# BoMingZhao/GaussianPrediction

Hardware: AMD Instinct MI355X
Metric: rendered views/s (full train step) @1M Gaussians 1352x1014 (higher is better)
Workload: dtype f32; 1 GPU; configs[2]: HyperNeRF-like 1M Gaussians, 1352x1014, stage-3 full train step (deform, raster, L1+SSIM loss, Adam: all HIP kernels); gaussians=1000000, width=1352, height=1014, keypoints=250, nearest_num=6, parallelism=view-parallel x1, ranks_seen_by_rccl=1, self_launched=False

## Files before the change

### gaussianprediction_amd/csrc/deform_kernels.h

```cpp
#pragma once
#include "gp_common.h"

struct MlpDev {
    long rows;
    int in_dim, in_pad, out_dim;
    int feature_dim, xyz_freq, time_freq;
    const float* w[5];
    const float* b[5];
    const float* feature;
    const float* xyz;
    const float* t;
    const float* pk;
};

struct MlpPackLayout {
    int q0;
    int tb0;
    long off_f[4], off_b[4], total;
};
static inline __host__ __device__ MlpPackLayout mlp_pack_layout(int in_dim) {
    MlpPackLayout L;
    L.q0 = (in_dim + 15) / 16;
    L.tb0 = 2 * ((in_dim + 31) / 32);
    long o = 0;
    L.off_f[0] = o; o += 16L * L.q0 * 64;
    for (int l = 1; l < 4; ++l) { L.off_f[l] = o; o += 16L * 16 * 64; }
    L.off_b[0] = o; o += (long)L.tb0 * 16 * 64;
    for (int l = 1; l < 4; ++l) { L.off_b[l] = o; o += 16L * 16 * 64; }
    L.total = o;
    return L;
}

struct MlpWeightJobs {
    const float* dZ[5];
    const float* H[5];
    float* dW[5];
    float* db[5];
    int n_out[5], n_in[5], ldh[5];
};

struct BlendDev {
    long N, K;
    int nn, out_dim, norm_rotation;
    const float* delta;
    const float* raw_w;
    const int64_t* knn;
    const float* xyz;
    const float* rot;
    const uint16_t* knn16;
};

__global__ __launch_bounds__(256) void gp_mlp_pack_kernel(MlpDev p, float4* __restrict__ out);
__global__ __launch_bounds__(512) void gp_mlp_fwd_kernel(MlpDev p, float* __restrict__ out, float* __restrict__ saved_x,
                                                         float* __restrict__ saved_h);
__global__ __launch_bounds__(512) void gp_mlp_bwd_data_kernel(MlpDev p, const float* __restrict__ saved_h,
                                                              const float* __restrict__ dL_dout, float* __restrict__ dz,
                                                              float* __restrict__ dfeature, float* __restrict__ dxyz);
__global__ __launch_bounds__(512) void gp_mlp_bwd_weight_kernel(const float* __restrict__ dZ, int n_out,
                                                                const float* __restrict__ H, int ldh, int n_in, long rows,
                                                                long rows_per_block, float* __restrict__ dW, int lddw,
                                                                float* __restrict__ db);
__global__ __launch_bounds__(256) void gp_blend_fwd_kernel(BlendDev a, float* __restrict__ xyz_t, float* __restrict__ q_t);
__global__ __launch_bounds__(256) void gp_blend_fwd6_kernel(BlendDev a, float* __restrict__ xyz_t, float* __restrict__ q_t);
__global__ __launch_bounds__(256) void gp_blend_fwd8_kernel(BlendDev a, float* __restrict__ xyz_t, float* __restrict__ q_t);
__global__ __launch_bounds__(256) void gp_blend_fwd6_i16_kernel(BlendDev a, float* __restrict__ xyz_t, float* __restrict__ q_t);
__global__ __launch_bounds__(256) void gp_blend_fwd8_i16_kernel(BlendDev a, float* __restrict__ xyz_t, float* __restrict__ q_t);
__global__ __launch_bounds__(256) void gp_blend_bwd_kernel(BlendDev a, const float* __restrict__ g_xyz_t,
                                                           const float* __restrict__ g_q_t, float* __restrict__ g_delta,
                                                           float* __restrict__ g_raw_w, float* __restrict__ g_xyz,
                                                           float* __restrict__ g_rot, float* __restrict__ partial);
__global__ __launch_bounds__(256) void gp_blend_bwd6_kernel(BlendDev a, const float* __restrict__ g_xyz_t,
                                                           const float* __restrict__ g_q_t, float* __restrict__ g_delta,
                                                           float* __restrict__ g_raw_w, float* __restrict__ g_xyz,
                                                           float* __restrict__ g_rot, float* __restrict__ partial);
__global__ __launch_bounds__(256) void gp_blend_bwd8_kernel(BlendDev a, const float* __restrict__ g_xyz_t,
                                                           const float* __restrict__ g_q_t, float* __restrict__ g_delta,
                                                           float* __restrict__ g_raw_w, float* __restrict__ g_xyz,
                                                           float* __restrict__ g_rot, float* __restrict__ partial);
__global__ __launch_bounds__(256) void gp_blend_bwd6_i16_kernel(BlendDev a, const float* __restrict__ g_xyz_t,
                                                           const float* __restrict__ g_q_t, float* __restrict__ g_delta,
                                                           float* __restrict__ g_raw_w, float* __restrict__ g_xyz,
                                                           float* __restrict__ g_rot, float* __restrict__ partial);
__global__ __launch_bounds__(256) void gp_blend_bwd8_i16_kernel(BlendDev a, const float* __restrict__ g_xyz_t,
                                                           const float* __restrict__ g_q_t, float* __restrict__ g_delta,
                                                           float* __restrict__ g_raw_w, float* __restrict__ g_xyz,
                                                           float* __restrict__ g_rot, float* __restrict__ partial);
__global__ __launch_bounds__(1024) void gp_blend_bwd_reduce_kernel(const float* __restrict__ partial, int nblocks, int KA,
                                                                  int od, float* __restrict__ g_delta);
__global__ __launch_bounds__(256) void gp_act_fwd_kernel(long n, const float* __restrict__ scaling_raw,
                                                         const float* __restrict__ opacity_raw,
                                                         const float* __restrict__ delta_o, int stride, float beta,
                                                         float* __restrict__ scale, float* __restrict__ opacity);
__global__ __launch_bounds__(256) void gp_act_bwd_kernel(long n, const float* __restrict__ scaling_raw,
                                                         const float* __restrict__ opacity_raw,
                                                         const float* __restrict__ delta_o, int stride, float beta,
                                                         const float* __restrict__ g_scale,
                                                         const float* __restrict__ g_opacity,
                                                         float* __restrict__ g_scaling_raw, float* __restrict__ g_opacity_raw,
                                                         float* __restrict__ g_delta_o);

__global__ __launch_bounds__(512) void gp_mlp_bwd_weight5_kernel(MlpWeightJobs t, long rows);
__global__ __launch_bounds__(512) void gp_mlp_fwd_small_kernel(MlpDev p, float* __restrict__ out, float* __restrict__ saved_x,
                                                               float* __restrict__ saved_h);
__global__ __launch_bounds__(512) void gp_mlp_bwd_data_small_kernel(MlpDev p, const float* __restrict__ saved_h,
                                                                    const float* __restrict__ dL_dout, float* __restrict__ dz,
                                                                    float* __restrict__ dfeature, float* __restrict__ dxyz);

__global__ __launch_bounds__(256) void gp_mlp_fwd_split_small_kernel(MlpDev p, float* __restrict__ out, float* __restrict__ saved_x, float* hx,
                                                                     uint32_t* flags, uint32_t* err);
__global__ __launch_bounds__(256) void gp_mlp_fwd_split_small_agent_kernel(MlpDev p, float* __restrict__ out, float* __restrict__ saved_x,
                                                                           float* hx, uint32_t* flags, uint32_t* err);
__global__ __launch_bounds__(256) void gp_mlp_bwd_data_split_small_kernel(MlpDev p, const float* __restrict__ saved_h, const float* __restrict__ dL_dout,
                                                                          float* dz, float* __restrict__ dfeature, float* __restrict__ dxyz, float* gx,
                                                                          uint32_t* flags, uint32_t* err, int form);
struct AdamTable;
__global__ __launch_bounds__(512) void gp_mlp_bwd_data_small_adam_kernel(MlpDev p, const float* __restrict__ saved_h,
                                                                         const float* __restrict__ dL_dout, float* __restrict__ dz,
                                                                         float* __restrict__ dfeature, float* __restrict__ dxyz,
                                                                         unsigned n_mlp, AdamTable t, float b1, float b2, float eps,
                                                                         int zero_grad, const uint32_t* __restrict__ skip_flag);

__global__ __launch_bounds__(256) void gp_mlp_bwd_weight64_kernel(const float* __restrict__ dZ, int n_out, const float* __restrict__ H,
                                                                 int ldh, int n_in, long rows, long rows_per_block,
                                                                 unsigned n_row_blocks, float* __restrict__ dW, int lddw,
                                                                 float* __restrict__ db);
__global__ __launch_bounds__(512) void gp_mlp_fwd2_kernel(MlpDev p, float* __restrict__ out, float* __restrict__ saved_x,
                                                          float* __restrict__ saved_h, uint32_t* __restrict__ masks);
__global__ __launch_bounds__(512) void gp_mlp_bwd_data2_kernel(MlpDev p, const uint32_t* __restrict__ masks,
                                                               const float* __restrict__ dL_dout, float* __restrict__ dz,
                                                               float* __restrict__ dfeature, float* __restrict__ dxyz);
```

### gaussianprediction_amd/csrc/deform_kernels.hip

```cpp
#include "gp_common.h"
#include "deform_kernels.h"

typedef float f32x16 __attribute__((ext_vector_type(16)));

#define MLP_ROWS 32
#define MLP_THREADS 512
#define MLP_W 256

__device__ __forceinline__ int act_idx(int f, int j) { return f * MLP_ROWS + (j ^ (f & 31)); }
__device__ __forceinline__ int cd_row(int r, int half) { return (r & 3) + 8 * (r >> 2) + 4 * half; }

__device__ __forceinline__ void build_input(float* buf, const MlpDev& p, long row0, int tid) {
    const int fd = p.feature_dim, xf = p.xyz_freq, tf = p.time_freq;
    for (int e = tid; e < fd * MLP_ROWS; e += MLP_THREADS) {
        const int jj = e / fd, f = e - jj * fd;
        const long row = row0 + jj;
        buf[act_idx(f, jj)] = row < p.rows ? p.feature[row * fd + f] : 0.f;
    }
    for (int e = tid; e < 3 * xf * MLP_ROWS; e += MLP_THREADS) {
        const int jj = e % MLP_ROWS, cf = e / MLP_ROWS;
        const int c = cf / xf, fr = cf - c * xf;
        const long row = row0 + jj;
        float sv = 0.f, cv = 0.f;
        if (row < p.rows) {
// ... 403 lines not shown
                    const long row = trow0 + jj;
                    if (row < p.rows) {
                        const float x = p.xyz[row * 3 + c];
                        float g = 0.f;
                        for (int fr = 0; fr < p.xyz_freq; ++fr) {
                            const float sc = (float)(1u << fr);
                            float sv, cv;
                            sincosf(x * sc, &sv, &cv);
                            const int f = p.feature_dim + 2 * (c * p.xyz_freq + fr);
                            g += sc * (cv * buf[act_idx(f, jj)] - sv * buf[act_idx(f + 1, jj)]);
                        }
                        dxyz[row * 3 + c] = g;
                    }
                }
            }
        }
    }
}

__device__ __forceinline__ void mlp_bwd_weight_body(const float* __restrict__ dZ, int n_out, const float* __restrict__ H, int ldh,
                                                    int n_in, long rows, long rows_per_block, float* __restrict__ dW, int lddw,
                                                    float* __restrict__ db, int row_block, int n_row_blocks, int bz, int by) {
    __shared__ float s_red[8][16][64];
    __shared__ float s_b[8][32];
    const int tid = threadIdx.x, lane = tid & 63, wave = tid >> 6, half = lane >> 5, j = lane & 31;
    const int o = 32 * bz + j;
    const int i = 32 * by + j;
    const long b_begin = (long)row_block * rows_per_block;
    long b_end = b_begin + rows_per_block;
    if (b_end > rows) b_end = rows;
    long per_wave = ((b_end - b_begin + 7) / 8 + 1) & ~1L;
    const long r_begin = b_begin + wave * per_wave;
    long r_end = r_begin + per_wave;
    if (r_end > b_end) r_end = b_end;
    f32x16 acc;
#pragma unroll
    for (int r = 0; r < 16; ++r) acc[r] = 0.f;
    float bsum = 0.f;
    const bool o_ok = o < n_out, i_ok = i < n_in;
    for (long rb = r_begin; rb < r_end; rb += 8) {
        float a[4], b[4];
#pragma unroll
        for (int u = 0; u < 4; ++u) {
            const long r = rb + 2 * u + half;
            a[u] = (r < r_end && o_ok) ? dZ[r * n_out + o] : 0.f;
            b[u] = (r < r_end && i_ok) ? H[r * (long)ldh + i] : 0.f;
            bsum += a[u];
        }
#pragma unroll
        for (int u = 0; u < 4; ++u) acc = __builtin_amdgcn_mfma_f32_32x32x2f32(a[u], b[u], acc, 0, 0, 0);
    }
#pragma unroll
    for (int r = 0; r < 16; ++r) s_red[wave][r][lane] = acc[r];
    bsum += __shfl_xor(bsum, 32);
    if (half == 0) s_b[wave][j] = bsum;
    __syncthreads();
    const bool single = n_row_blocks == 1;
    for (int e = tid; e < 16 * 64; e += MLP_THREADS) {
        const int r = e >> 6, l = e & 63;
        float v = 0.f;
#pragma unroll
        for (int w = 0; w < 8; ++w) v += s_red[w][r][l];
        const int oo = 32 * bz + cd_row(r, l >> 5), ii = 32 * by + (l & 31);
        if (oo < n_out && ii < n_in) {
            float* dst = &dW[(size_t)oo * lddw + ii];
            if (single) *dst += v; else atomicAdd(dst, v);
        }
    }
    if (db && by == 0 && tid < 32) {
        float v = 0.f;
#pragma unroll
        for (int w = 0; w < 8; ++w) v += s_b[w][tid];
        const int oo = 32 * bz + tid;
        if (oo < n_out) { if (single) db[oo] += v; else atomicAdd(&db[oo], v); }
    }
}

__global__ __launch_bounds__(MLP_THREADS) void gp_mlp_bwd_weight_kernel(const float* __restrict__ dZ, int n_out,
                                                                        const float* __restrict__ H, int ldh, int n_in,
                                                                        long rows, long rows_per_block,
                                                                        float* __restrict__ dW, int lddw,
                                                                        float* __restrict__ db) {
    mlp_bwd_weight_body(dZ, n_out, H, ldh, n_in, rows, rows_per_block, dW, lddw, db, blockIdx.x, gridDim.x, blockIdx.z, blockIdx.y);
}
__global__ __launch_bounds__(MLP_THREADS) void gp_mlp_bwd_weight5_kernel(MlpWeightJobs t, long rows) {
    const int l = blockIdx.x;
    if ((int)blockIdx.y * 32 >= t.n_in[l] || (int)blockIdx.z * 32 >= t.n_out[l]) return;
    mlp_bwd_weight_body(t.dZ[l], t.n_out[l], t.H[l], t.ldh[l], t.n_in[l], rows, rows, t.dW[l], t.n_in[l], t.db[l], 0, 1, blockIdx.z,
                        blockIdx.y);
}

__global__ __launch_bounds__(256) void gp_mlp_bwd_weight64_kernel(const float* __restrict__ dZ, int n_out, const float* __restrict__ H,
                                                                 int ldh, int n_in, long rows, long rows_per_block,
                                                                 unsigned n_row_blocks, float* __restrict__ dW, int lddw,
                                                                 float* __restrict__ db) {
    __shared__ float s_red[4][4][16][64];
    const int tid = threadIdx.x, lane = tid & 63, wave = tid >> 6, half = lane >> 5, j = lane & 31;
    const int n_ib = (n_in + 63) / 64;
    const int ntp = n_ib * ((n_out + 63) / 64);
    const unsigned flat = blockIdx.x, xcd = flat & 7u, seq = flat >> 3;
    const unsigned slab = (seq / ntp) * 8u + xcd, tp = seq % ntp;
    if (slab >= n_row_blocks) return;
    const int o0 = 64 * (tp / n_ib), i0 = 64 * (tp % n_ib);
    const long b_begin = (long)slab * rows_per_block;
    long b_end = b_begin + rows_per_block;
    if (b_end > rows) b_end = rows;
    const long per_wave = ((b_end - b_begin + 3) / 4 + 7) & ~7L;
    const long r_begin = b_begin + wave * per_wave;
    long r_end = r_begin + per_wave;
    if (r_end > b_end) r_end = b_end;
    f32x16 acc[2][2];
#pragma unroll
    for (int a = 0; a < 2; ++a)
#pragma unroll
        for (int b = 0; b < 2; ++b)
#pragma unroll
            for (int r = 0; r < 16; ++r) acc[a][b][r] = 0.f;
    float bsum[2] = {0.f, 0.f};
    const int oa = o0 + j, ob = o0 + 32 + j, ia = i0 + j, ib = i0 + 32 + j;
    const bool oka = oa < n_out, okb = ob < n_out, ika = ia < n_in, ikb = ib < n_in;
    for (long rb = r_begin; rb < r_end; rb += 8) {
        float a0[4], a1[4], b0[4], b1[4];
#pragma unroll
        for (int u = 0; u < 4; ++u) {
            const long r = rb + 2 * u + half;
            const bool rk = r < r_end;
            a0[u] = (rk && oka) ? dZ[r * n_out + oa] : 0.f;
            a1[u] = (rk && okb) ? dZ[r * n_out + ob] : 0.f;
            b0[u] = (rk && ika) ? H[r * (long)ldh + ia] : 0.f;
            b1[u] = (rk && ikb) ? H[r * (long)ldh + ib] : 0.f;
            bsum[0] += a0[u]; bsum[1] += a1[u];
        }
#pragma unroll
        for (int u = 0; u < 4; ++u) {
            acc[0][0] = __builtin_amdgcn_mfma_f32_32x32x2f32(a0[u], b0[u], acc[0][0], 0, 0, 0);
            acc[0][1] = __builtin_amdgcn_mfma_f32_32x32x2f32(a0[u], b1[u], acc[0][1], 0, 0, 0);
            acc[1][0] = __builtin_amdgcn_mfma_f32_32x32x2f32(a1[u], b0[u], acc[1][0], 0, 0, 0);
            acc[1][1] = __builtin_amdgcn_mfma_f32_32x32x2f32(a1[u], b1[u], acc[1][1], 0, 0, 0);
        }
    }
#pragma unroll
    for (int a = 0; a < 2; ++a)
#pragma unroll
        for (int b = 0; b < 2; ++b)
#pragma unroll
            for (int r = 0; r < 16; ++r) s_red[wave][2 * a + b][r][lane] = acc[a][b][r];
    __syncthreads();
    const bool single = n_row_blocks == 1;
    for (int e = tid; e < 4 * 16 * 64; e += 256) {
        const int tl = e >> 10, r = (e >> 6) & 15, l = e & 63;
        const float v = (s_red[0][tl][r][l] + s_red[1][tl][r][l]) + (s_red[2][tl][r][l] + s_red[3][tl][r][l]);
        const int oo = o0 + 32 * (tl >> 1) + cd_row(r, l >> 5), ii = i0 + 32 * (tl & 1) + (l & 31);
        if (oo < n_out && ii < n_in) {
            float* dst = &dW[(size_t)oo * lddw + ii];
            if (single) *dst += v; else atomicAdd(dst, v);
        }
    }
    if (db && i0 == 0) {
        __syncthreads();
        float* sb = &s_red[0][0][0][0];
#pragma unroll
        for (int u = 0; u < 2; ++u) {
            const float v = bsum[u] + __shfl_xor(bsum[u], 32);
            if (half == 0) sb[(wave * 2 + u) * 32 + j] = v;
        }
        __syncthreads();
        if (tid < 64) {
            const int u = tid >> 5, jj = tid & 31;
            const float v = (sb[(0 * 2 + u) * 32 + jj] + sb[(1 * 2 + u) * 32 + jj]) + (sb[(2 * 2 + u) * 32 + jj] + sb[(3 * 2 + u) * 32 + jj]);
            const int oo = o0 + 32 * u + jj;
            if (oo < n_out) { if (single) db[oo] += v; else atomicAdd(&db[oo], v); }
        }
    }
}

#define GP_MAX_NN 16

__device__ __forceinline__ void quat_mul(const float* q, const float* r, float* p) {
    p[0] = r[0] * q[0] - r[1] * q[1] - r[2] * q[2] - r[3] * q[3];
    p[1] = r[1] * q[0] + r[0] * q[1] + r[3] * q[2] - r[2] * q[3];
    p[2] = r[2] * q[0] - r[3] * q[1] + r[0] * q[2] + r[1] * q[3];
    p[3] = r[3] * q[0] + r[2] * q[1] - r[1] * q[2] + r[0] * q[3];
}
__device__ __forceinline__ float norm4(const float* v) {
    return fmaxf(sqrtf(v[0] * v[0] + v[1] * v[1] + v[2] * v[2] + v[3] * v[3]), 1e-12f);
}
__device__ __forceinline__ void softmax_n(const float* __restrict__ raw, int n, float* w) {
    float m = raw[0];
#pragma unroll
    for (int k = 1; k < n; ++k) m = fmaxf(m, raw[k]);
    float s = 0.f;
#pragma unroll
    for (int k = 0; k < n; ++k) { w[k] = expf(raw[k] - m); s += w[k]; }
    const float inv = 1.f / s;
#pragma unroll
    for (int k = 0; k < n; ++k) w[k] *= inv;
}

template <int NN, bool I16>
__device__ __forceinline__ void load_row_nn(const BlendDev& a, long i, float (&raw)[2 * NN], int (&kps)[NN]) {
    const float4* r4 = (const float4*)(a.raw_w + i * 2 * NN);
#pragma unroll
    for (int u = 0; u < 2 * NN / 4; ++u) { const float4 t = r4[u]; raw[4 * u] = t.x; raw[4 * u + 1] = t.y; raw[4 * u + 2] = t.z; raw[4 * u + 3] = t.w; }
    if (I16) {
        const uint32_t* k1 = (const uint32_t*)(a.knn16 + i * NN);
#pragma unroll
        for (int u = 0; u < NN / 2; ++u) { const uint32_t t = k1[u]; kps[2 * u] = (int)(t & 0xFFFFu); kps[2 * u + 1] = (int)(t >> 16); }
    } else {
        typedef long long ll2 __attribute__((ext_vector_type(2)));
        const ll2* k2 = (const ll2*)(a.knn + i * NN);
#pragma unroll
        for (int u = 0; u < NN / 2; ++u) { const ll2 t = k2[u]; kps[2 * u] = (int)t.x; kps[2 * u + 1] = (int)t.y; }
    }
}

template <int NN, bool I16 = false>
__device__ __forceinline__ void blend_fwd_body(BlendDev a, float* __restrict__ xyz_t, float* __restrict__ q_t) {
    const long i = (long)blockIdx.x * 256 + threadIdx.x;
    if (i >= a.N) return;
    float dxyz[3] = {0.f, 0.f, 0.f}, dq[4] = {0.f, 0.f, 0.f, 0.f};
    const int od = a.out_dim;
    const int nn = NN > 0 ? NN : a.nn;
    const float x0[3] = {a.xyz[3 * i], a.xyz[3 * i + 1], a.xyz[3 * i + 2]};
    const float r[4] = {a.rot[4 * i], a.rot[4 * i + 1], a.rot[4 * i + 2], a.rot[4 * i + 3]};
    if (nn > 0) {
        float wx[NN > 0 ? NN : GP_MAX_NN], wr[NN > 0 ? NN : GP_MAX_NN];
        int kpv[NN > 0 ? NN : 1];
        if constexpr (NN > 0) {
            float raw[2 * (NN > 0 ? NN : 1)];
            load_row_nn<NN, I16>(a, i, raw, kpv);
            softmax_n(raw, NN, wx);
            softmax_n(raw + NN, NN, wr);
        } else {
            softmax_n(a.raw_w + i * 2 * nn, nn, wx);
            softmax_n(a.raw_w + i * 2 * nn + nn, nn, wr);
        }
        if constexpr (NN > 0) {
            float dlr[NN > 0 ? NN : 1][7];
#pragma unroll
            for (int k = 0; k < NN; ++k) {
                const float* dl = a.delta + (long)kpv[k] * od;
#pragma unroll
                for (int c = 0; c < 7; ++c) dlr[k][c] = dl[c];
            }
#pragma unroll
            for (int k = 0; k < NN; ++k) {
                dxyz[0] = fmaf(wx[k], dlr[k][0], dxyz[0]);
                dxyz[1] = fmaf(wx[k], dlr[k][1], dxyz[1]);
                dxyz[2] = fmaf(wx[k], dlr[k][2], dxyz[2]);
                float v[4] = {dlr[k][3], dlr[k][4], dlr[k][5], dlr[k][6]};
                if (a.norm_rotation) { const float inv = 1.f / norm4(v); v[0] *= inv; v[1] *= inv; v[2] *= inv; v[3] *= inv; }
                dq[0] = fmaf(wr[k], v[0], dq[0]); dq[1] = fmaf(wr[k], v[1], dq[1]);
                dq[2] = fmaf(wr[k], v[2], dq[2]); dq[3] = fmaf(wr[k], v[3], dq[3]);
            }
        } else {
            for (int k = 0; k < nn; ++k) {
                const long kp = a.knn16 ? (long)a.knn16[i * nn + k] : a.knn[i * nn + k];
                const float* dl = a.delta + kp * od;
                dxyz[0] = fmaf(wx[k], dl[0], dxyz[0]);
                dxyz[1] = fmaf(wx[k], dl[1], dxyz[1]);
                dxyz[2] = fmaf(wx[k], dl[2], dxyz[2]);
                float v[4] = {dl[3], dl[4], dl[5], dl[6]};
                if (a.norm_rotation) { const float inv = 1.f / norm4(v); v[0] *= inv; v[1] *= inv; v[2] *= inv; v[3] *= inv; }
                dq[0] = fmaf(wr[k], v[0], dq[0]); dq[1] = fmaf(wr[k], v[1], dq[1]);
                dq[2] = fmaf(wr[k], v[2], dq[2]); dq[3] = fmaf(wr[k], v[3], dq[3]);
            }
        }
    } else {
        const float* dl = a.delta + i * od;
        dxyz[0] = dl[0]; dxyz[1] = dl[1]; dxyz[2] = dl[2];
        dq[0] = dl[3]; dq[1] = dl[4]; dq[2] = dl[5]; dq[3] = dl[6];
        if (a.norm_rotation) { const float inv = 1.f / norm4(dq); dq[0] *= inv; dq[1] *= inv; dq[2] *= inv; dq[3] *= inv; }
    }
    xyz_t[3 * i] = x0[0] + dxyz[0];
    xyz_t[3 * i + 1] = x0[1] + dxyz[1];
    xyz_t[3 * i + 2] = x0[2] + dxyz[2];
    const float invq = 1.f / norm4(dq);
    const float q[4] = {dq[0] * invq, dq[1] * invq, dq[2] * invq, dq[3] * invq};
    float pq[4];
    quat_mul(q, r, pq);
    const float invp = 1.f / norm4(pq);
    q_t[4 * i] = pq[0] * invp; q_t[4 * i + 1] = pq[1] * invp; q_t[4 * i + 2] = pq[2] * invp; q_t[4 * i + 3] = pq[3] * invp;
}
__global__ __launch_bounds__(256) void gp_blend_fwd_kernel(BlendDev a, float* __restrict__ xyz_t, float* __restrict__ q_t) { blend_fwd_body<0>(a, xyz_t, q_t); }
__global__ __launch_bounds__(256) void gp_blend_fwd6_kernel(BlendDev a, float* __restrict__ xyz_t, float* __restrict__ q_t) { blend_fwd_body<6>(a, xyz_t, q_t); }
__global__ __launch_bounds__(256) void gp_blend_fwd8_kernel(BlendDev a, float* __restrict__ xyz_t, float* __restrict__ q_t) { blend_fwd_body<8>(a, xyz_t, q_t); }
__global__ __launch_bounds__(256) void gp_blend_fwd6_i16_kernel(BlendDev a, float* __restrict__ xyz_t, float* __restrict__ q_t) { blend_fwd_body<6, true>(a, xyz_t, q_t); }
__global__ __launch_bounds__(256) void gp_blend_fwd8_i16_kernel(BlendDev a, float* __restrict__ xyz_t, float* __restrict__ q_t) { blend_fwd_body<8, true>(a, xyz_t, q_t); }

__device__ __forceinline__ void normalize_bwd(const float* v, const float* g, float* dv) {
    const float n = norm4(v), inv = 1.f / n;
    const float y[4] = {v[0] * inv, v[1] * inv, v[2] * inv, v[3] * inv};
    const float dot = y[0] * g[0] + y[1] * g[1] + y[2] * g[2] + y[3] * g[3];
#pragma unroll
    for (int k = 0; k < 4; ++k) dv[k] = (g[k] - y[k] * dot) * inv;
}

#define BB_LONG 20
#define BB_LONG_CAP 320
template <int NN, bool I16 = false>
__device__ __forceinline__ void blend_bwd_body(BlendDev a, const float* __restrict__ g_xyz_t,
                                               const float* __restrict__ g_q_t, float* __restrict__ g_delta,
                                               float* __restrict__ g_raw_w, float* __restrict__ g_xyz,
                                               float* __restrict__ g_rot, float* __restrict__ partial) {
    extern __shared__ float s_dyn[];
    const int od = a.out_dim;
    const int nn = NN > 0 ? NN : a.nn;
    const int K = (int)a.K;
    const int tid = threadIdx.x;
    float* s_acc = s_dyn;
    float* s_delta = s_acc + (nn > 0 ? K * 7 : 0);
    int* s_cnt = (int*)(s_delta + (nn > 0 ? K * od : 0));
    int* s_base = s_cnt + (nn > 0 ? K : 0);
    float* s_g = (float*)(s_base + (nn > 0 ? K + 1 : 0));
    float* s_inv = s_g + 256 * 7;
    float* s_w = s_inv + (nn > 0 ? K : 0);
    unsigned short* s_sorted = (unsigned short*)(s_w + 256 * 2 * nn);
    __shared__ int s_wsum[4];
    __shared__ int s_nlong, s_long[BB_LONG_CAP];
    if (nn > 0) {
        for (int e = tid; e < K * 7; e += 256) s_acc[e] = 0.f;
        for (int e = tid; e < K * od; e += 256) s_delta[e] = a.delta[e];
        if (a.norm_rotation) {
            __syncthreads();
            for (int kp = tid; kp < K; kp += 256) {
                float* dl = s_delta + kp * od;
                const float v[4] = {dl[3], dl[4], dl[5], dl[6]};
                const float inv = 1.f / norm4(v);
                s_inv[kp] = inv;
                dl[3] = v[0] * inv; dl[4] = v[1] * inv; dl[5] = v[2] * inv; dl[6] = v[3] * inv;
            }
        }
    }
    const long chunks = (a.N + 255) / 256;
    for (long c = blockIdx.x; c < chunks; c += gridDim.x) {
        const long i = c * 256 + tid;
        const bool live = i < a.N;
        if (nn > 0) {
            for (int e = tid; e < K; e += 256) s_cnt[e] = 0;
            if (tid == 0) s_nlong = 0;
            __syncthreads();
        }
        int kps[NN > 0 ? NN : GP_MAX_NN], rk[NN > 0 ? NN : GP_MAX_NN];
        if (live) {
            const float gx[3] = {g_xyz_t[3 * i], g_xyz_t[3 * i + 1], g_xyz_t[3 * i + 2]};
            const float gq[4] = {g_q_t[4 * i], g_q_t[4 * i + 1], g_q_t[4 * i + 2], g_q_t[4 * i + 3]};
            const float r[4] = {a.rot[4 * i], a.rot[4 * i + 1], a.rot[4 * i + 2], a.rot[4 * i + 3]};
            float wx[NN > 0 ? NN : GP_MAX_NN], wr[NN > 0 ? NN : GP_MAX_NN];
            float dq[4] = {0.f, 0.f, 0.f, 0.f};
            if (nn > 0) {
                if constexpr (NN > 0) {
                    float raw[2 * (NN > 0 ? NN : 1)];
                    load_row_nn<NN, I16>(a, i, raw, kps);
                    softmax_n(raw, NN, wx);
                    softmax_n(raw + NN, NN, wr);
                } else {
                    softmax_n(a.raw_w + i * 2 * nn, nn, wx);
                    softmax_n(a.raw_w + i * 2 * nn + nn, nn, wr);
                }
#pragma unroll
                for (int k = 0; k < nn; ++k) {
                    if (NN == 0) kps[k] = a.knn16 ? (int)a.knn16[i * nn + k] : (int)a.knn[i * nn + k];
                    const float* dl = s_delta + kps[k] * od;
                    const float v[4] = {dl[3], dl[4], dl[5], dl[6]};
                    dq[0] = fmaf(wr[k], v[0], dq[0]); dq[1] = fmaf(wr[k], v[1], dq[1]);
                    dq[2] = fmaf(wr[k], v[2], dq[2]); dq[3] = fmaf(wr[k], v[3], dq[3]);
                }
            } else {
                const float* dl = a.delta + i * od;
                dq[0] = dl[3]; dq[1] = dl[4]; dq[2] = dl[5]; dq[3] = dl[6];
                if (a.norm_rotation) { const float inv = 1.f / norm4(dq); dq[0] *= inv; dq[1] *= inv; dq[2] *= inv; dq[3] *= inv; }
            }
            const float invq = 1.f / norm4(dq);
            const float q[4] = {dq[0] * invq, dq[1] * invq, dq[2] * invq, dq[3] * invq};
            g_xyz[3 * i] = gx[0]; g_xyz[3 * i + 1] = gx[1]; g_xyz[3 * i + 2] = gx[2];
            float pq[4];
            quat_mul(q, r, pq);
            float gp[4];
            normalize_bwd(pq, gq, gp);
            const float gqn[4] = {gp[0] * r[0] + gp[1] * r[1] + gp[2] * r[2] + gp[3] * r[3],
                                  -gp[0] * r[1] + gp[1] * r[0] - gp[2] * r[3] + gp[3] * r[2],
                                  -gp[0] * r[2] + gp[1] * r[3] + gp[2] * r[0] - gp[3] * r[1],
                                  -gp[0] * r[3] - gp[1] * r[2] + gp[2] * r[1] + gp[3] * r[0]};
            g_rot[4 * i + 0] = gp[0] * q[0] + gp[1] * q[1] + gp[2] * q[2] + gp[3] * q[3];
            g_rot[4 * i + 1] = -gp[0] * q[1] + gp[1] * q[0] + gp[2] * q[3] - gp[3] * q[2];
            g_rot[4 * i + 2] = -gp[0] * q[2] - gp[1] * q[3] + gp[2] * q[0] + gp[3] * q[1];
            g_rot[4 * i + 3] = -gp[0] * q[3] + gp[1] * q[2] - gp[2] * q[1] + gp[3] * q[0];
            float gdq[4];
            normalize_bwd(dq, gqn, gdq);
            if (nn > 0) {
                float gwx[NN > 0 ? NN : GP_MAX_NN], gwr[NN > 0 ? NN : GP_MAX_NN];
                float sx = 0.f, sr = 0.f;
#pragma unroll
                for (int k = 0; k < nn; ++k) {
                    const float* dl = s_delta + kps[k] * od;
                    gwx[k] = dl[0] * gx[0] + dl[1] * gx[1] + dl[2] * gx[2];
                    const float vn[4] = {dl[3], dl[4], dl[5], dl[6]};
                    gwr[k] = vn[0] * gdq[0] + vn[1] * gdq[1] + vn[2] * gdq[2] + vn[3] * gdq[3];
                    sx += wx[k] * gwx[k];
                    sr += wr[k] * gwr[k];
                    s_w[k * 256 + tid] = wx[k];
                    s_w[(nn + k) * 256 + tid] = wr[k];
                    rk[k] = atomicAdd(&s_cnt[kps[k]], 1);
                }
                if (g_raw_w) {
                    if constexpr (NN > 0) {
                        float go[2 * (NN > 0 ? NN : 1)];
#pragma unroll
                        for (int k = 0; k < NN; ++k) { go[k] = wx[k] * (gwx[k] - sx); go[NN + k] = wr[k] * (gwr[k] - sr); }
                        float4* o4 = (float4*)(g_raw_w + i * 2 * NN);
#pragma unroll
                        for (int u = 0; u < 2 * NN / 4; ++u) o4[u] = make_float4(go[4 * u], go[4 * u + 1], go[4 * u + 2], go[4 * u + 3]);
                    } else {
                        for (int k = 0; k < nn; ++k) {
                            g_raw_w[i * 2 * nn + k] = wx[k] * (gwx[k] - sx);
                            g_raw_w[i * 2 * nn + nn + k] = wr[k] * (gwr[k] - sr);
                        }
                    }
                }
                s_g[0 * 256 + tid] = gx[0]; s_g[1 * 256 + tid] = gx[1]; s_g[2 * 256 + tid] = gx[2];
                s_g[3 * 256 + tid] = gdq[0]; s_g[4 * 256 + tid] = gdq[1]; s_g[5 * 256 + tid] = gdq[2]; s_g[6 * 256 + tid] = gdq[3];
            } else {
                const float* dl = a.delta + i * od;
                float gv[4] = {gdq[0], gdq[1], gdq[2], gdq[3]};
                if (a.norm_rotation) { const float v[4] = {dl[3], dl[4], dl[5], dl[6]}; normalize_bwd(v, gdq, gv); }
                float* gd = g_delta + i * od;
                gd[0] = gx[0]; gd[1] = gx[1]; gd[2] = gx[2];
                gd[3] = gv[0]; gd[4] = gv[1]; gd[5] = gv[2]; gd[6] = gv[3];
                for (int k = 7; k < od; ++k) gd[k] = 0.f;
            }
        }
        if (nn > 0) {
            __syncthreads();
            {
                const int per = (K + 255) / 256;
                const int b0 = tid * per;
                int loc = 0;
                for (int e = 0; e < per; ++e) if (b0 + e < K) loc += s_cnt[b0 + e];
                int inc = loc;
                inc = gp_wave_scan_add(inc);
                if ((tid & 63) == 63) s_wsum[tid >> 6] = inc;
                __syncthreads();
                int woff = 0;
                for (int w = 0; w < (tid >> 6); ++w) woff += s_wsum[w];
                int run = woff + inc - loc;
                for (int e = 0; e < per; ++e) if (b0 + e < K) { s_base[b0 + e] = run; run += s_cnt[b0 + e]; }
                if (tid == 255) s_base[K] = run;
            }
            __syncthreads();
            if (live) {
#pragma unroll
                for (int k = 0; k < nn; ++k) s_sorted[s_base[kps[k]] + rk[k]] = (unsigned short)((k << 8) | tid);
            }
            __syncthreads();
            for (int kp = tid; kp < K; kp += 256) {
                float sacc[7] = {0.f, 0.f, 0.f, 0.f, 0.f, 0.f, 0.f};
                const int pe = s_base[kp + 1];
                if (pe - s_base[kp] > BB_LONG) { s_long[atomicAdd(&s_nlong, 1)] = kp; continue; }
                for (int pp = s_base[kp]; pp < pe; pp += 2) {
                    const int e0 = s_sorted[pp], e1 = pp + 1 < pe ? s_sorted[pp + 1] : -1;
                    const int t0 = e0 & 255, k0 = e0 >> 8, t1 = e1 & 255, k1 = (e1 >> 8) & 15;
                    const float wx0 = s_w[k0 * 256 + t0], wr0 = s_w[(nn + k0) * 256 + t0];
                    const float wx1 = e1 >= 0 ? s_w[k1 * 256 + t1] : 0.f, wr1 = e1 >= 0 ? s_w[(nn + k1) * 256 + t1] : 0.f;
                    float g0[7], g1[7];
#pragma unroll
                    for (int cc = 0; cc < 7; ++cc) { g0[cc] = s_g[cc * 256 + t0]; g1[cc] = s_g[cc * 256 + t1]; }
                    sacc[0] = fmaf(wx0, g0[0], sacc[0]); sacc[1] = fmaf(wx0, g0[1], sacc[1]); sacc[2] = fmaf(wx0, g0[2], sacc[2]);
                    sacc[3] = fmaf(wr0, g0[3], sacc[3]); sacc[4] = fmaf(wr0, g0[4], sacc[4]);
                    sacc[5] = fmaf(wr0, g0[5], sacc[5]); sacc[6] = fmaf(wr0, g0[6], sacc[6]);
                    if (e1 >= 0) {
                        sacc[0] = fmaf(wx1, g1[0], sacc[0]); sacc[1] = fmaf(wx1, g1[1], sacc[1]); sacc[2] = fmaf(wx1, g1[2], sacc[2]);
                        sacc[3] = fmaf(wr1, g1[3], sacc[3]); sacc[4] = fmaf(wr1, g1[4], sacc[4]);
                        sacc[5] = fmaf(wr1, g1[5], sacc[5]); sacc[6] = fmaf(wr1, g1[6], sacc[6]);
                    }
                }
                float* acc = s_acc + kp * 7;
#pragma unroll
                for (int cc = 0; cc < 7; ++cc) acc[cc] += sacc[cc];
            }
            __syncthreads();
            const int nlong = s_nlong;
            for (int q = tid >> 6; q < nlong; q += 4) {
                const int kp = s_long[q], pe = s_base[kp + 1];
                float sacc[7] = {0.f, 0.f, 0.f, 0.f, 0.f, 0.f, 0.f};
                for (int pp = s_base[kp] + (tid & 63); pp < pe; pp += 64) {
                    const int e = s_sorted[pp], t = e & 255, k = e >> 8;
                    const float wxk = s_w[k * 256 + t], wrk = s_w[(nn + k) * 256 + t];
                    sacc[0] = fmaf(wxk, s_g[0 * 256 + t], sacc[0]); sacc[1] = fmaf(wxk, s_g[1 * 256 + t], sacc[1]);
                    sacc[2] = fmaf(wxk, s_g[2 * 256 + t], sacc[2]); sacc[3] = fmaf(wrk, s_g[3 * 256 + t], sacc[3]);
                    sacc[4] = fmaf(wrk, s_g[4 * 256 + t], sacc[4]); sacc[5] = fmaf(wrk, s_g[5 * 256 + t], sacc[5]);
                    sacc[6] = fmaf(wrk, s_g[6 * 256 + t], sacc[6]);
                }
#pragma unroll
                for (int off = 32; off > 0; off >>= 1)
#pragma unroll
                    for (int cc = 0; cc < 7; ++cc) sacc[cc] += __shfl_xor(sacc[cc], off);
                if ((tid & 63) == 0) {
                    float* acc = s_acc + kp * 7;
#pragma unroll
                    for (int cc = 0; cc < 7; ++cc) acc[cc] += sacc[cc];
                }
            }
            if (nlong > 0) __syncthreads();
        }
    }
    if (nn > 0) {
        const int KA = K * 7;
        for (int kp = tid; kp < K; kp += 256) {
            float* acc = s_acc + kp * 7;
            if (a.norm_rotation) {
                const float* y = s_delta + kp * od + 3;
                const float inv = s_inv[kp];
                const float cq[4] = {acc[3], acc[4], acc[5], acc[6]};
                const float dot = y[0] * cq[0] + y[1] * cq[1] + y[2] * cq[2] + y[3] * cq[3];
#pragma unroll
                for (int k = 0; k < 4; ++k) acc[3 + k] = (cq[k] - y[k] * dot) * inv;
            }
        }
        __syncthreads();
        for (int e = tid; e < KA; e += 256) partial[(size_t)blockIdx.x * KA + e] = s_acc[e];
    }
}

#define BB_ARGS BlendDev a, const float* __restrict__ g_xyz_t, const float* __restrict__ g_q_t, float* __restrict__ g_delta, \
    float* __restrict__ g_raw_w, float* __restrict__ g_xyz, float* __restrict__ g_rot, float* __restrict__ partial
__global__ __launch_bounds__(256) void gp_blend_bwd_kernel(BB_ARGS) { blend_bwd_body<0>(a, g_xyz_t, g_q_t, g_delta, g_raw_w, g_xyz, g_rot, partial); }
__global__ __launch_bounds__(256) void gp_blend_bwd6_kernel(BB_ARGS) { blend_bwd_body<6>(a, g_xyz_t, g_q_t, g_delta, g_raw_w, g_xyz, g_rot, partial); }
__global__ __launch_bounds__(256) void gp_blend_bwd8_kernel(BB_ARGS) { blend_bwd_body<8>(a, g_xyz_t, g_q_t, g_delta, g_raw_w, g_xyz, g_rot, partial); }
__global__ __launch_bounds__(256) void gp_blend_bwd6_i16_kernel(BB_ARGS) { blend_bwd_body<6, true>(a, g_xyz_t, g_q_t, g_delta, g_raw_w, g_xyz, g_rot, partial); }
__global__ __launch_bounds__(256) void gp_blend_bwd8_i16_kernel(BB_ARGS) { blend_bwd_body<8, true>(a, g_xyz_t, g_q_t, g_delta, g_raw_w, g_xyz, g_rot, partial); }

__global__ __launch_bounds__(1024) void gp_blend_bwd_reduce_kernel(const float* __restrict__ partial, int nblocks, int KA,
                                                                  int od, float* __restrict__ g_delta) {
    __shared__ float s_r[16][64];
    const int lane = threadIdx.x & 63, wave = threadIdx.x >> 6;
    const int e = blockIdx.x * 64 + lane;
    float v0 = 0.f, v1 = 0.f, v2 = 0.f, v3 = 0.f;
    if (e < KA) {
        int b = wave;
        for (; b + 240 < nblocks; b += 256) {
            float t[16];
#pragma unroll
            for (int u = 0; u < 16; ++u) t[u] = partial[(size_t)(b + 16 * u) * KA + e];
#pragma unroll
            for (int u = 0; u < 16; u += 4) { v0 += t[u]; v1 += t[u + 1]; v2 += t[u + 2]; v3 += t[u + 3]; }
        }
        for (; b + 48 < nblocks; b += 64) {
            v0 += partial[(size_t)b * KA + e]; v1 += partial[(size_t)(b + 16) * KA + e];
            v2 += partial[(size_t)(b + 32) * KA + e]; v3 += partial[(size_t)(b + 48) * KA + e];
        }
        for (; b < nblocks; b += 16) v0 += partial[(size_t)b * KA + e];
    }
    s_r[wave][lane] = (v0 + v1) + (v2 + v3);
    __syncthreads();
    if (wave == 0 && e < KA) {
        float t = 0.f;
#pragma unroll
        for (int w = 0; w < 16; ++w) t += s_r[w][lane];
        g_delta[(size_t)(e / 7) * od + (e % 7)] = t;
        if (e % 7 == 6) for (int c = 7; c < od; ++c) g_delta[(size_t)(e / 7) * od + c] = 0.f;
    }
}

__device__ __forceinline__ float sigmoidf(float x) { return 1.f / (1.f + expf(-x)); }

__global__ __launch_bounds__(256) void gp_act_fwd_kernel(long n, const float* __restrict__ scaling_raw,
                                                        const float* __restrict__ opacity_raw,
                                                        const float* __restrict__ delta_o, int stride, float beta,
                                                        float* __restrict__ scale, float* __restrict__ opacity) {
    const long i = (long)blockIdx.x * 256 + threadIdx.x;
    if (i >= n) return;
    const float s0 = scaling_raw[3 * i], s1 = scaling_raw[3 * i + 1], s2 = scaling_raw[3 * i + 2];
    const float op_raw = opacity_raw[i];
    const float dlt = delta_o ? delta_o[i * stride] : 0.f;
    scale[3 * i] = expf(s0);
    scale[3 * i + 1] = expf(s1);
    scale[3 * i + 2] = expf(s2);
    float o = sigmoidf(op_raw);
    if (delta_o) o *= 1.f / (1.f + expf(-dlt / beta));
    opacity[i] = o;
}
__global__ __launch_bounds__(256) void gp_act_bwd_kernel(long n, const float* __restrict__ scaling_raw,
                                                        const float* __restrict__ opacity_raw,
                                                        const float* __restrict__ delta_o, int stride, float beta,
                                                        const float* __restrict__ g_scale, const float* __restrict__ g_opacity,
                                                        float* __restrict__ g_scaling_raw, float* __restrict__ g_opacity_raw,
                                                        float* __restrict__ g_delta_o) {
    const long i = (long)blockIdx.x * 256 + threadIdx.x;
    if (i >= n) return;
    float gs[3] = {0.f, 0.f, 0.f}, sr[3] = {0.f, 0.f, 0.f};
    if (g_scaling_raw && g_scale) {
#pragma unroll
        for (int k = 0; k < 3; ++k) { gs[k] = g_scale[3 * i + k]; sr[k] = scaling_raw[3 * i + k]; }
    }
    const float op_raw = opacity_raw[i];
    const float go = g_opacity ? g_opacity[i] : 0.f;
    const float dlt = delta_o ? delta_o[i * stride] : 0.f;
    if (g_scaling_raw) {
#pragma unroll
        for (int k = 0; k < 3; ++k) g_scaling_raw[3 * i + k] = g_scale ? gs[k] * expf(sr[k]) : 0.f;
    }
    const float so = sigmoidf(op_raw);
    float life = 1.f;
    if (delta_o) life = 1.f / (1.f + expf(-dlt / beta));
    if (g_opacity_raw) g_opacity_raw[i] = go * life * so * (1.f - so);
    if (delta_o && g_delta_o) g_delta_o[i * stride] = go * so * life * (1.f - life) / beta;
}
```

### gaussianprediction_amd/csrc/gp_capi_deform.hip

```cpp
#include "gp_common.h"
#include "deform_kernels.h"
#include "loss_adam_kernels.h"
#include <stdlib.h>

static int make_mlp(const gp_mlp_params* p, const gp_mlp_input* x, MlpDev& m) {
    if (!p || !x) GP_FAIL("null mlp params/input");
    if (p->width != 256 || p->depth != 4) GP_FAIL("Deformable_Field: only d=4, w=256 is implemented (got d=%d w=%d)", p->depth, p->width);
    if (p->out_dim < 7 || p->out_dim > 8) GP_FAIL("out_dim must be 7 or 8 (got %d)", p->out_dim);
    if (x->feature_dim <= 0 || x->feature_dim % 4 || x->xyz_freq < 0 || x->xyz_freq > 16 || x->time_freq < 0 || x->time_freq > 16)
        GP_FAIL("bad input encoding dims");
    const int in_dim = x->feature_dim + 6 * x->xyz_freq + 2 * x->time_freq;
    if (in_dim != p->in_dim) GP_FAIL("in_dim %d != feature_dim + 6*xyz_freq + 2*time_freq = %d", p->in_dim, in_dim);
    if (in_dim % 4 || in_dim > 256) GP_FAIL("in_dim %d must be a multiple of 4 and <= 256", in_dim);
    if (x->rows < 0) GP_FAIL("negative rows");
    for (int l = 0; l < 5; ++l)
        if (!p->w[l] || !p->b[l]) GP_FAIL("null weight pointer (layer %d)", l);
    if (x->rows > 0 && (!x->feature || (x->xyz_freq > 0 && !x->xyz) || (x->time_freq > 0 && !x->t))) GP_FAIL("null input pointer");
    m.rows = x->rows; m.in_dim = in_dim; m.in_pad = (in_dim + 7) / 8 * 8; m.out_dim = p->out_dim;
    m.feature_dim = x->feature_dim; m.xyz_freq = x->xyz_freq; m.time_freq = x->time_freq;
    for (int l = 0; l < 5; ++l) { m.w[l] = p->w[l]; m.b[l] = p->b[l]; }
    m.feature = x->feature; m.xyz = x->xyz; m.t = x->t;
    m.pk = p->packed;
    if (m.pk && ((uintptr_t)m.pk & 15) != 0) GP_FAIL("gp_mlp_params.packed must be 16-byte aligned");
    if (p->scratch && ((uintptr_t)p->scratch & 15) != 0) GP_FAIL("gp_mlp_params.scratch must be 16-byte aligned");
    return 0;
}

extern "C" int64_t gp_mlp_packed_floats(int32_t in_dim) {
    if (in_dim <= 0 || in_dim > 256) return -1;
    return 4 * (int64_t)mlp_pack_layout(in_dim).total;
}

extern "C" int gp_mlp_pack(const gp_mlp_params* p, float* packed, gp_stream_t stream_) {
    if (!p || !packed) GP_FAIL("null argument");
    if (p->width != 256 || p->depth != 4) GP_FAIL("Deformable_Field: only d=4, w=256 is implemented");
    if (p->in_dim <= 0 || p->in_dim % 4 || p->in_dim > 256) GP_FAIL("in_dim %d must be a multiple of 4 and <= 256", p->in_dim);
    if (((uintptr_t)packed & 15) != 0) GP_FAIL("packed must be 16-byte aligned");
    MlpDev m;
    memset(&m, 0, sizeof(m));
    m.in_dim = p->in_dim;
    for (int l = 0; l < 4; ++l) { if (!p->w[l]) GP_FAIL("null weight pointer (layer %d)", l); m.w[l] = p->w[l]; }
    const long total = mlp_pack_layout(p->in_dim).total;
    GpProfScope _p("mlp_pack", (hipStream_t)stream_);
    hipLaunchKernelGGL(gp_mlp_pack_kernel, dim3(gp_blocks((size_t)total, 256)), dim3(256), 0, (hipStream_t)stream_, m, (float4*)packed);
    GP_LAUNCH_CHECK();
    return 0;
}

static inline size_t acts_x_floats(const MlpDev& m) { return (size_t)m.rows * m.in_pad; }

#define GP_MLP_SMALL_ROWS 2048
#define GP_MLP_LARGE_ROWS 32768
#define GP_MLP_SPLIT_ROWS 512
#define GP_MLP_SCRATCH_FLAG_BYTES 8192
#define GP_MLP_SCRATCH_ERR_WORD 1024

extern "C" int64_t gp_mlp_scratch_bytes(int64_t rows) {
    if (rows <= 0 || rows > GP_MLP_SPLIT_ROWS) return 0;
    return GP_MLP_SCRATCH_FLAG_BYTES + (int64_t)4 * rows * 256 * (int64_t)sizeof(float);
}

static unsigned mlp_split_grid(const MlpDev& m, const void* scratch, int& mode, int*& state_out) {
    mode = 0; state_out = nullptr;
    if (!scratch || m.rows > GP_MLP_SPLIT_ROWS || gp_debug_get(13) == 1) return 0;
    const unsigned rt = (unsigned)((m.rows + 15) / 16), grid = 8u * 16u * ((rt + 7u) / 8u);
    static int resident[32] = {0}, state[32] = {0};
    int dev = 0;
    if (hipGetDevice(&dev) != hipSuccess || dev < 0 || dev >= 32) return 0;
    if (__atomic_load_n(&resident[dev], __ATOMIC_RELAXED) == 0) {
        int per_cu = 0, r = -1;
        hipDeviceProp_t prop;
        if (hipOccupancyMaxActiveBlocksPerMultiprocessor(&per_cu, gp_mlp_fwd_split_small_kernel, 256, 0) == hipSuccess &&
            hipGetDeviceProperties(&prop, dev) == hipSuccess && per_cu * prop.multiProcessorCount > 0)
            r = per_cu * prop.multiProcessorCount;
        else (void)hipGetLastError();
        __atomic_store_n(&resident[dev], r, __ATOMIC_RELAXED);
    }
    if (__atomic_load_n(&resident[dev], __ATOMIC_RELAXED) < (int)grid) return 0;
    if (gp_debug_get(13) == 2) { mode = 3; return grid; }
    const int st = __atomic_load_n(&state[dev], __ATOMIC_ACQUIRE);
    if (st < 0) return 0;
    mode = st > 0 ? 1 : 2;
    state_out = &state[dev];
    return grid;
}

extern "C" int gp_mlp_forward(const gp_mlp_params* p, const gp_mlp_input* x, float* out, float* acts, gp_stream_t stream_) {
    MlpDev m;
    if (make_mlp(p, x, m)) return 1;
    if (m.rows == 0) return 0;
    if (!out) GP_FAIL("null output");
    float* sx = acts;
    float* sh = acts ? acts + gp_align_up(acts_x_floats(m), 64) : nullptr;
    { GpProfScope _p("mlp_fwd", (hipStream_t)stream_);
        int mode = 0;
        int* state = nullptr;
        const unsigned split = mlp_split_grid(m, p->scratch, mode, state);
        if (split) {
            float* hx = sh ? sh : (float*)((char*)p->scratch + GP_MLP_SCRATCH_FLAG_BYTES);
            uint32_t* flags = (uint32_t*)p->scratch;
            hipLaunchKernelGGL(mode == 3 ? gp_mlp_fwd_split_small_agent_kernel : gp_mlp_fwd_split_small_kernel, dim3(split), dim3(256), 0,
                               (hipStream_t)stream_, m, out, sx, hx, flags, flags + GP_MLP_SCRATCH_ERR_WORD);
            if (mode == 2) {
                uint32_t e = 1;
                if (hipGetLastError() != hipSuccess || hipStreamSynchronize((hipStream_t)stream_) != hipSuccess ||
                    hipMemcpy(&e, flags + GP_MLP_SCRATCH_ERR_WORD, sizeof(e), hipMemcpyDeviceToHost) != hipSuccess) e = 1;
                if (e != 0) {
                    (void)hipGetLastError();
                    __atomic_store_n(state, -1, __ATOMIC_RELEASE);
                    GP_HIP_CHECK(hipMemsetAsync(flags, 0, GP_MLP_SCRATCH_FLAG_BYTES, (hipStream_t)stream_));
                    hipLaunchKernelGGL(gp_mlp_fwd_small_kernel, dim3(gp_blocks((size_t)m.rows, 16)), dim3(512), 0, (hipStream_t)stream_, m, out, sx, sh);
                } else __atomic_store_n(state, 1, __ATOMIC_RELEASE);
            }
        }
        else if (m.rows <= GP_MLP_SMALL_ROWS)
            hipLaunchKernelGGL(gp_mlp_fwd_small_kernel, dim3(gp_blocks((size_t)m.rows, 16)), dim3(512), 0, (hipStream_t)stream_, m, out, sx, sh);
        else if (m.rows >= GP_MLP_LARGE_ROWS)
            hipLaunchKernelGGL(gp_mlp_fwd2_kernel, dim3(gp_blocks((size_t)m.rows, 64)), dim3(512), 0, (hipStream_t)stream_, m, out, sx, sh,
                               acts ? (uint32_t*)(sh + (size_t)4 * m.rows * 256) : (uint32_t*)nullptr);
        else
            hipLaunchKernelGGL(gp_mlp_fwd_kernel, dim3(gp_blocks((size_t)m.rows, 32)), dim3(512), 0, (hipStream_t)stream_, m, out, sx, sh);
    GP_LAUNCH_CHECK(); }
    return 0;
}

static thread_local int g_dfeature_accumulate = 0;
bool gp_mlp_backward_splits(const gp_mlp_params* p, int64_t rows) {
    if (!p) return false;
    MlpDev m;
    memset(&m, 0, sizeof(m));
    m.rows = rows;
    int mode = 0;
    int* st = nullptr;
    return mlp_split_grid(m, p->scratch, mode, st) != 0 && (mode == 1 || mode == 3);
}
void gp_mlp_backward_accumulate_dfeature_once() { g_dfeature_accumulate = 1; }

extern "C" int gp_mlp_backward(const gp_mlp_params* p, const gp_mlp_input* x, const float* acts, const float* dL_dout,
                               gp_mlp_grads* g, float* dL_dfeature, float* dL_dxyz, gp_alloc_fn alloc, void* alloc_ctx,
                               gp_stream_t stream_) {
    hipStream_t s = (hipStream_t)stream_;
    struct ClearAcc { ~ClearAcc() { g_dfeature_accumulate = 0; } } clear_acc;
    MlpDev m;
    if (make_mlp(p, x, m)) return 1;
    if (m.rows == 0) return 0;
    if (!acts || !dL_dout || !g || !alloc) GP_FAIL("null argument");
    for (int l = 0; l < 5; ++l)
        if (!g->dw[l] || !g->db[l]) GP_FAIL("null weight-grad pointer (layer %d)", l);
    const float* sx = acts;
    const float* sh = acts + gp_align_up(acts_x_floats(m), 64);
    const size_t dz_bytes = gp_align_up((size_t)4 * m.rows * 256 * sizeof(float), 256);
    float* dz = (float*)alloc(alloc_ctx, GP_BUF_TEMP, dz_bytes);
    if (!dz) GP_FAIL("allocator returned NULL for TEMP (%zu B)", dz_bytes);
    GpAdamRider* rider = gp_adam_rider_slot();
    int split_mode = 0;
    int* split_state = nullptr;
    const unsigned split = mlp_split_grid(m, p->scratch, split_mode, split_state);
    if (split && (split_mode == 1 || split_mode == 3)) {
        float* gx = (float*)((char*)p->scratch + GP_MLP_SCRATCH_FLAG_BYTES);
        uint32_t* flags = (uint32_t*)p->scratch;
        GpProfScope _p("mlp_bwd_data", s);
        const int acc = g_dfeature_accumulate;
        g_dfeature_accumulate = 0;
        hipLaunchKernelGGL(gp_mlp_bwd_data_split_small_kernel, dim3(split), dim3(256), 0, s, m, sh, dL_dout, dz, dL_dfeature, dL_dxyz, gx, flags,
                           flags + GP_MLP_SCRATCH_ERR_WORD, (split_mode == 3 ? 1 : 0) | (acc ? 2 : 0));
        GP_LAUNCH_CHECK();
    } else if (m.rows <= GP_MLP_SMALL_ROWS && rider->armed) {
        rider->armed = false;
        const unsigned n_mlp = gp_blocks((size_t)m.rows, 16);
        GpProfScope _p("adam", s);
        hipLaunchKernelGGL(gp_mlp_bwd_data_small_adam_kernel, dim3(n_mlp + rider->chunks), dim3(512), 0, s, m, sh, dL_dout, dz, dL_dfeature,
                           dL_dxyz, n_mlp, rider->t, rider->b1, rider->b2, rider->eps, rider->zero_grad, rider->skip_flag);
        GP_LAUNCH_CHECK();
    } else { GpProfScope _p("mlp_bwd_data", s);
        if (m.rows <= GP_MLP_SMALL_ROWS)
            hipLaunchKernelGGL(gp_mlp_bwd_data_small_kernel, dim3(gp_blocks((size_t)m.rows, 16)), dim3(512), 0, s, m, sh, dL_dout, dz,
                               dL_dfeature, dL_dxyz);
        else if (m.rows >= GP_MLP_LARGE_ROWS)
            hipLaunchKernelGGL(gp_mlp_bwd_data2_kernel, dim3(gp_blocks((size_t)m.rows, 64)), dim3(512), 0, s, m,
                               (const uint32_t*)(sh + (size_t)4 * m.rows * 256), dL_dout, dz,
                               dL_dfeature, dL_dxyz);
        else
            hipLaunchKernelGGL(gp_mlp_bwd_data_kernel, dim3(gp_blocks((size_t)m.rows, 32)), dim3(512), 0, s, m, sh, dL_dout, dz,
                       dL_dfeature, dL_dxyz);
    GP_LAUNCH_CHECK(); }
    long nrb_l = (m.rows + 4095) / 4096;
    if (nrb_l > 16) nrb_l = 16;
    if (nrb_l < 1) nrb_l = 1;
    long rpb = ((m.rows + nrb_l - 1) / nrb_l + 15) & ~15L;
    const unsigned nrb = (unsigned)((m.rows + rpb - 1) / rpb);
    GpProfScope _pw("mlp_bwd_weight", s);
    if (nrb == 1) {
        MlpWeightJobs jobs;
        for (int l = 0; l < 5; ++l) {
            jobs.dZ[l] = l < 4 ? dz + (size_t)l * m.rows * 256 : dL_dout;
            jobs.n_out[l] = l < 4 ? 256 : m.out_dim;
            jobs.H[l] = l == 0 ? sx : sh + (size_t)(l - 1) * m.rows * 256;
            jobs.ldh[l] = l == 0 ? m.in_pad : 256;
            jobs.n_in[l] = l == 0 ? m.in_dim : 256;
            jobs.dW[l] = g->dw[l]; jobs.db[l] = g->db[l];
        }
        hipLaunchKernelGGL(gp_mlp_bwd_weight5_kernel, dim3(5, 8, 8), dim3(512), 0, s, jobs, m.rows);
        GP_LAUNCH_CHECK();
        return 0;
    }
    if (m.rows >= 16384) {
        long nb = (m.rows + 4095) / 4096;
        if (nb < 64) nb = 64;
        const long brpb = ((m.rows + nb - 1) / nb + 7) & ~7L;
        const unsigned bnrb = (unsigned)((m.rows + brpb - 1) / brpb);
        for (int l = 0; l < 5; ++l) {
            const float* dZl = l < 4 ? dz + (size_t)l * m.rows * 256 : dL_dout;
            const int n_out = l < 4 ? 256 : m.out_dim;
            const float* H = l == 0 ? sx : sh + (size_t)(l - 1) * m.rows * 256;
            const int ldh = l == 0 ? m.in_pad : 256;
            const int n_in = l == 0 ? m.in_dim : 256;
            const unsigned ntp = (unsigned)((n_in + 63) / 64) * (unsigned)((n_out + 63) / 64);
            hipLaunchKernelGGL(gp_mlp_bwd_weight64_kernel, dim3(ntp * ((bnrb + 7u) & ~7u)), dim3(256), 0, s, dZl, n_out, H, ldh, n_in,
                               m.rows, brpb, bnrb, g->dw[l], n_in, g->db[l]);
            GP_LAUNCH_CHECK();
        }
        return 0;
    }
    for (int l = 0; l < 5; ++l) {
        const float* dZl = l < 4 ? dz + (size_t)l * m.rows * 256 : dL_dout;
        const int n_out = l < 4 ? 256 : m.out_dim;
        const float* H = l == 0 ? sx : sh + (size_t)(l - 1) * m.rows * 256;
        const int ldh = l == 0 ? m.in_pad : 256;
        const int n_in = l == 0 ? m.in_dim : 256;
        {
        hipLaunchKernelGGL(gp_mlp_bwd_weight_kernel, dim3(nrb, (unsigned)((n_in + 31) / 32), (unsigned)((n_out + 31) / 32)),
                           dim3(512), 0, s, dZl, n_out, H, ldh, n_in, m.rows, rpb, g->dw[l], n_in, g->db[l]);
        GP_LAUNCH_CHECK(); }
    }
    return 0;
}

static int make_blend(const gp_blend_args* a, BlendDev& b) {
    if (!a) GP_FAIL("null blend args");
    if (a->num_gaussians < 0) GP_FAIL("negative num_gaussians");
    if (a->out_dim < 7 || a->out_dim > 8) GP_FAIL("out_dim must be 7 or 8");
    if (a->nearest_num < 0 || a->nearest_num > 16) GP_FAIL("nearest_num %d unsupported (0..16)", a->nearest_num);
    if (a->nearest_num > 0 && (a->num_keypoints <= 0 || !a->raw_w || !a->knn_idx)) GP_FAIL("stage-2 blend needs keypoints, raw_w and knn_idx");
    if (a->nearest_num > 0 && a->num_keypoints * 7 * sizeof(float) > 60000) GP_FAIL("too many keypoints (%ld) for the LDS accumulator", (long)a->num_keypoints);
    if (a->num_gaussians > 0 && (!a->delta || !a->xyz || !a->rot)) GP_FAIL("null blend input");
    if (a->knn_idx16 && (a->num_keypoints > 65535 || ((uintptr_t)a->knn_idx16 & 3) != 0)) GP_FAIL("knn_idx16 needs K < 65536 and 4-byte alignment");
    b.N = a->num_gaussians; b.K = a->num_keypoints; b.nn = a->nearest_num; b.out_dim = a->out_dim;
    b.norm_rotation = a->norm_rotation; b.delta = a->delta; b.raw_w = a->raw_w; b.knn = a->knn_idx; b.xyz = a->xyz; b.rot = a->rot; b.knn16 = a->knn_idx16;
    return 0;
}

extern "C" int gp_blend_forward(const gp_blend_args* a, float* xyz_t, float* q_t, gp_stream_t stream_) {
    BlendDev b;
    if (make_blend(a, b)) return 1;
    if (b.N == 0) return 0;
    if (!xyz_t || !q_t) GP_FAIL("null output");
    { GpProfScope _p("blend_fwd", (hipStream_t)stream_);
        const bool al = (((uintptr_t)b.raw_w | (uintptr_t)b.knn) & 15) == 0;
        const bool i16 = b.knn16 != nullptr;
        hipLaunchKernelGGL(b.nn == 6 && al ? (i16 ? gp_blend_fwd6_i16_kernel : gp_blend_fwd6_kernel)
                           : b.nn == 8 && al ? (i16 ? gp_blend_fwd8_i16_kernel : gp_blend_fwd8_kernel) : gp_blend_fwd_kernel,
                       dim3(gp_blocks((size_t)b.N, 256)), dim3(256), 0, (hipStream_t)stream_, b, xyz_t, q_t);
    GP_LAUNCH_CHECK(); }
    return 0;
}

extern "C" int gp_blend_backward(const gp_blend_args* a, const float* dL_dxyz_t, const float* dL_dq_t, float* dL_ddelta,
                                 float* dL_draw_w, float* dL_dxyz, float* dL_drot, gp_alloc_fn alloc, void* alloc_ctx,
                                 gp_stream_t stream_) {
    BlendDev b;
    if (make_blend(a, b)) return 1;
    if (b.N == 0) return 0;
    if (!dL_dxyz_t || !dL_dq_t || !dL_ddelta || !dL_dxyz || !dL_drot) GP_FAIL("null argument");
    unsigned blocks = gp_blocks((size_t)b.N, 256);
    if (b.nn > 0 && blocks > 1024) blocks = 1024;
    const size_t lds = b.nn > 0 ? ((size_t)b.K * (7 + b.out_dim + 3) + 1 + 256 * 7 + 256 * 2 * (size_t)b.nn) * 4 + 256 * (size_t)b.nn * 2 + 16 : 256 * 8 * 4;
    if (lds > 64 * 1024) GP_FAIL("keypoint blend backward: K = %ld, nn = %d needs %zu B of LDS (> 64 KiB)", (long)b.K, b.nn, lds);
    float* partial = nullptr;
    const int KA = (int)b.K * 7;
    if (b.nn > 0) {
        if (!alloc) GP_FAIL("null allocator");
        partial = (float*)alloc(alloc_ctx, GP_BUF_TEMP, gp_align_up((size_t)blocks * KA * sizeof(float), 256));
        if (!partial) GP_FAIL("allocator returned NULL for TEMP");
    }
    { GpProfScope _p("blend_bwd", (hipStream_t)stream_);
    const bool al = (((uintptr_t)b.raw_w | (uintptr_t)b.knn | (uintptr_t)dL_draw_w) & 15) == 0;
    const bool i16 = b.knn16 != nullptr;
    hipLaunchKernelGGL(b.nn == 6 && al ? (i16 ? gp_blend_bwd6_i16_kernel : gp_blend_bwd6_kernel)
                       : b.nn == 8 && al ? (i16 ? gp_blend_bwd8_i16_kernel : gp_blend_bwd8_kernel) : gp_blend_bwd_kernel,
                       dim3(blocks), dim3(256), lds, (hipStream_t)stream_, b, dL_dxyz_t, dL_dq_t, dL_ddelta,
                       dL_draw_w, dL_dxyz, dL_drot, partial);
    GP_LAUNCH_CHECK();
    if (b.nn > 0) {
        hipLaunchKernelGGL(gp_blend_bwd_reduce_kernel, dim3(gp_blocks((size_t)KA, 64)), dim3(1024), 0, (hipStream_t)stream_, partial,
                           (int)blocks, KA, b.out_dim, dL_ddelta);
        GP_LAUNCH_CHECK();
    } }
    return 0;
}

extern "C" int gp_activations_forward(int64_t n, const float* scaling_raw, const float* opacity_raw, const float* delta_o,
                                      int32_t stride, float beta, float* scale, float* opacity, gp_stream_t stream_) {
    if (n < 0) GP_FAIL("negative n");
    if (n == 0) return 0;
    if (!scaling_raw || !opacity_raw || !scale || !opacity) GP_FAIL("null argument");
    if (delta_o && (stride <= 0 || !(beta > 0.f))) GP_FAIL("bad delta_o stride/beta");
    hipLaunchKernelGGL(gp_act_fwd_kernel, dim3(gp_blocks((size_t)n, 256)), dim3(256), 0, (hipStream_t)stream_, (long)n, scaling_raw,
                       opacity_raw, delta_o, stride, beta, scale, opacity);
    GP_LAUNCH_CHECK();
    return 0;
}

extern "C" int gp_activations_backward(int64_t n, const float* scaling_raw, const float* opacity_raw, const float* delta_o,
                                       int32_t stride, float beta, const float* dL_dscale, const float* dL_dopacity,
                                       float* dL_dscaling_raw, float* dL_dopacity_raw, float* dL_ddelta_o, gp_stream_t stream_) {
    if (n < 0) GP_FAIL("negative n");
    if (n == 0) return 0;
    if (!scaling_raw || !opacity_raw) GP_FAIL("null argument");
    hipLaunchKernelGGL(gp_act_bwd_kernel, dim3(gp_blocks((size_t)n, 256)), dim3(256), 0, (hipStream_t)stream_, (long)n, scaling_raw,
                       opacity_raw, delta_o, stride, beta, dL_dscale, dL_dopacity, dL_dscaling_raw, dL_dopacity_raw, dL_ddelta_o);
    GP_LAUNCH_CHECK();
    return 0;
}
```

### gaussianprediction_amd/csrc/gp_capi_raster.hip

```cpp
#include "gp_common.h"
#include "raster_kernels.h"
#include <stdlib.h>
#include <atomic>

thread_local char gp_err_buf[512] = "";
static std::atomic<uint32_t> g_key_tag{0};

extern "C" const char* gp_last_error(void) { return gp_err_buf; }
extern "C" const char* gp_version(void) { return "gaussianprediction_amd 0.4 (gfx950)"; }
extern "C" int gp_abi_version(void) { return GP_ABI_VERSION; }

static int tile_bits_for(int T) {
    int b = 1;
    while ((1 << b) < T) ++b;
    return b;
}

static int make_dims(const gp_raster_settings* st, const gp_raster_inputs* in, RasterDims& d) {
    if (!st || !in) GP_FAIL("null settings/inputs");
    if (st->image_width <= 0 || st->image_height <= 0) GP_FAIL("bad image size %dx%d", st->image_width, st->image_height);
    if (in->num_gaussians < 0 || in->num_gaussians > 0x7FFFFFF0LL) GP_FAIL("num_gaussians out of range");
    if (st->sh_degree < 0 || st->sh_degree > 3) GP_FAIL("sh_degree %d unsupported (0..3)", st->sh_degree);
    const bool has_sr = in->scales != nullptr || in->rotations != nullptr;
    if (in->num_gaussians > 0) {
        if ((in->shs == nullptr) == (in->colors_precomp == nullptr)) GP_FAIL("Please provide exactly one of either SHs or precomputed colors!");
        if (has_sr == (in->cov3D_precomp != nullptr) || (has_sr && (!in->scales || !in->rotations)))
            GP_FAIL("Please provide exactly one of either scale/rotation pair or precomputed 3D covariance!");
    }
    if (in->shs && st->sh_coeffs < (st->sh_degree + 1) * (st->sh_degree + 1)) GP_FAIL("shs has %d coeffs, degree %d needs more", st->sh_coeffs, st->sh_degree);
    if (in->shs && st->sh_coeffs > 16) GP_FAIL("sh_coeffs %d > 16 unsupported", st->sh_coeffs);
    if (in->shs_rest && (!in->shs || st->sh_coeffs != 16)) GP_FAIL("shs_rest needs shs (= features_dc) and sh_coeffs == 16");
    if (!st->bg || !st->viewmatrix || !st->projmatrix || !st->campos) GP_FAIL("null camera pointers");
    if (in->num_gaussians > 0 && (!in->means3D || !in->opacities)) GP_FAIL("null means3D/opacities");
    d.N = (int)in->num_gaussians;
    d.M = in->shs ? st->sh_coeffs : 0;
    d.D = st->sh_degree;
    d.W = st->image_width;
    d.H = st->image_height;
    d.gx = (d.W + GP_TILE - 1) / GP_TILE;
    d.gy = (d.H + GP_TILE - 1) / GP_TILE;
    d.tanfovx = st->tanfovx;
    d.tanfovy = st->tanfovy;
    d.fx = (float)d.W / (2.f * st->tanfovx);
    d.fy = (float)d.H / (2.f * st->tanfovy);
    d.scale_mod = st->scale_modifier;
    d.late_color = (st->sh_ready_event && in->shs) ? 1 : 0;
    d.visible = nullptr; d.zero_words = nullptr; d.n_zero = 0;
    d.key_hi = 0u; d.key_base = 0u; d.key_culled = 0xFFFFFFFFu; d.key_flag = nullptr; d.key_tag = 0u;
    d.sb_side = nullptr;
    d.raw_opacity = nullptr;
    if (st->raw_activations) {
        if (in->cov3D_precomp || !in->scales) GP_FAIL("raw_activations needs scales + rotations (not cov3D_precomp)");
        d.raw_opacity = in->opacities;
    }
    if (st->depth_key_bits != 0 && st->depth_key_bits != 32) {
        if (st->depth_key_bits < 8 || st->depth_key_bits > 31) GP_FAIL("depth_key_bits must be 0, 32 or 8 .. 31 (got %d)", st->depth_key_bits);
        if (!st->binning_status) GP_FAIL("depth_key_bits needs binning_status (the word a broken promise raises)");
        const uint32_t low = (1u << st->depth_key_bits) - 1u;
        d.key_hi = ~low;
        d.key_base = st->depth_key_base;
        d.key_culled = low;
        d.key_flag = st->binning_status + 2;
        do { d.key_tag = ++g_key_tag; } while (d.key_tag == 0u);
    }
    return 0;
}

struct GeomLayout {
    float4* rec;
    uint8_t* clamped;
    float2* sb_side;
    size_t bytes;
    GeomLayout(void* base, size_t N) {
        GpCarver c(base);
        rec = c.take<float4>(3 * N + 1);
        clamped = c.take<uint8_t>(N + 1);
        sb_side = c.take<float2>(GP_SB_HOIST == 1 ? N + 1 : 0);
        bytes = c.bytes();
    }
};
struct ImageLayout {
    int2* ranges;
    float* final_T;
    int32_t* n_contrib;
    int32_t* tile_work;
    uint32_t* order;
    size_t bytes;
    uint32_t* total;
    ImageLayout(void* base, size_t T, size_t P) {
        GpCarver c(base);
        ranges = c.take<int2>(T + GP_TOTAL_SLOTS / 2);
        total = (uint32_t*)(ranges + T);
        final_T = c.take<float>(P);
        n_contrib = c.take<int32_t>(P);
        tile_work = c.take<int32_t>(T);
        order = c.take<uint32_t>(T);
        bytes = c.bytes();
    }
};

extern "C" int gp_raster_forward(const gp_raster_settings* st, const gp_raster_inputs* in, gp_raster_outputs* out,
                                 gp_raster_saved* saved, gp_alloc_fn alloc, void* alloc_ctx, gp_stream_t stream_) {
    hipStream_t s = (hipStream_t)stream_;
    RasterDims d;
    if (make_dims(st, in, d)) return 1;
    if (!out || !out->color || !out->depth || !out->tidx || (d.N > 0 && !out->radii)) GP_FAIL("null output pointers");
    if (!saved || !alloc) GP_FAIL("null saved/alloc");
    const size_t N = (size_t)d.N, T = (size_t)d.gx * d.gy, P = (size_t)d.W * d.H;

    ImageLayout il0(nullptr, T, P);
    void* img = alloc(alloc_ctx, GP_BUF_IMAGE, il0.bytes);
    if (!img) GP_FAIL("allocator returned NULL for IMAGE (%zu B)", il0.bytes);
    ImageLayout il(img, T, P);
    GeomLayout gl0(nullptr, N);
    void* geom = alloc(alloc_ctx, GP_BUF_GEOM, gl0.bytes);
    if (!geom) GP_FAIL("allocator returned NULL for GEOM (%zu B)", gl0.bytes);
    GeomLayout gl(geom, N);
    d.sb_side = gl.sb_side;
    saved->geom = geom; saved->geom_bytes = gl.bytes;
    saved->image = img; saved->image_bytes = il.bytes;
    saved->binning = nullptr; saved->binning_bytes = 0; saved->num_rendered = 0;

    {
        const size_t words = (T + GP_TOTAL_SLOTS / 2) * 2;
        if ((size_t)N >= words) { d.zero_words = (uint32_t*)il.ranges; d.n_zero = (int)words; }
        else GP_HIP_CHECK(hipMemsetAsync(il.ranges, 0, words * sizeof(uint32_t), s));
    }
    d.visible = out->visible;
    uint32_t R = 0;
    uint32_t* point_list = nullptr;
    bool order_done = false;
    if (N > 0) {
        GpCarver tc0(nullptr);
        const size_t hist_elems = gp_sort_hist_elems(N);
        const size_t scan_elems = gp_scan_tmp_elems(256 * ((N + 4095) / 4096) > N + 1 ? 256 * ((N + 4095) / 4096) : N + 1) + (N + GP_SCAN_TILE - 1) / GP_SCAN_TILE + 64;
        const bool counting = gp_bin_supported(N, T);
        GpBinPlan bp = {0, 0, 0};
        if (counting) bp = gp_bin_plan(N, T);
        const bool dsort3 = gp_dsort_supported(N);
        auto carve_tmp = [&](GpCarver& c, uint32_t*& k0, uint32_t*& k1, uint32_t*& v0, uint32_t*& v1, uint2*& tiles,
                             uint2*& rects, uint32_t*& tt, uint32_t*& hist, uint32_t*& scan_tmp, uint32_t*& binhist, uint32_t*& dshist) {
            k0 = c.take<uint32_t>(N); k1 = c.take<uint32_t>(N); v0 = c.take<uint32_t>(N); v1 = c.take<uint32_t>(N);
            tiles = c.take<uint2>(N); rects = c.take<uint2>(N); tt = c.take<uint32_t>(N + 1);
            hist = c.take<uint32_t>(hist_elems); scan_tmp = c.take<uint32_t>(scan_elems);
            binhist = c.take<uint32_t>(bp.hist_elems);
            dshist = c.take<uint32_t>(dsort3 ? gp_dsort_hist_elems(N) : 0);
        };
        uint32_t *k0, *k1, *v0, *v1, *tt, *hist, *scan_tmp, *binhist, *dshist;
        uint2 *tiles, *rects;
        carve_tmp(tc0, k0, k1, v0, v1, tiles, rects, tt, hist, scan_tmp, binhist, dshist);
        void* tmp = alloc(alloc_ctx, GP_BUF_TEMP, tc0.bytes());
        if (!tmp) GP_FAIL("allocator returned NULL for TEMP (%zu B)", tc0.bytes());
        GpCarver tc(tmp);
        carve_tmp(tc, k0, k1, v0, v1, tiles, rects, tt, hist, scan_tmp, binhist, dshist);

        {
            GpProfScope _p("preprocess_fwd", s);
            const bool al16 = (((uintptr_t)in->shs | (uintptr_t)in->shs_rest) & 15) == 0;
            auto kern = gp_preprocess_fwd_kernel;
            if (in->shs && in->shs_rest) {
                if (!al16) GP_FAIL("shs/shs_rest must be 16-byte aligned");
                kern = gp_preprocess_fwd_split_kernel;
            } else if (in->shs && d.M == 16 && al16) {
                kern = gp_preprocess_fwd_sh16_kernel;
            }
            hipLaunchKernelGGL(kern, dim3(gp_blocks(N, 256)), dim3(256), 0, s, d, in->means3D, in->scales, in->rotations,
                               in->opacities, in->shs, in->shs_rest, in->colors_precomp, in->cov3D_precomp, st->viewmatrix,
                               st->projmatrix, st->campos, out->radii, gl.rec, k0, tiles, gl.clamped);
            GP_LAUNCH_CHECK();
        }
        GpSortBufs sb;
        sb.k[0] = k0; sb.k[1] = k1; sb.v[0] = v0; sb.v[1] = v1; sb.hist = hist; sb.scan_tmp = scan_tmp; sb.scan_tmp_elems = scan_elems;
        int r1;
        const GpSortEpilogue ep = {tiles, rects, tt};
        const int key_bits = d.key_hi ? st->depth_key_bits : 32;
        if (st->depth_key_range) {
            GP_HIP_CHECK(hipMemsetAsync(st->depth_key_range, 0xFF, 4, s));
            GP_HIP_CHECK(hipMemsetAsync(st->depth_key_range + 1, 0, 4, s));
            hipLaunchKernelGGL(gp_key_range_kernel, dim3(gp_blocks(N, 1024)), dim3(256), 0, s, (const uint32_t*)k0, (const int32_t*)out->radii, (int)N,
                               d.key_base, st->depth_key_range);
            GP_LAUNCH_CHECK();
        }
        { GpProfScope _p("depth_sort", s); r1 = (dsort3 && key_bits == 32) ? gp_depth_sort3(sb, N, dshist, s, &ep) : gp_radix_sort_pairs(sb, N, key_bits, s, true, &ep); }
        if (r1 < 0) return 1;
        const uint32_t* sorted_ids = sb.v[r1];
        uint32_t* block_sums = scan_tmp;
        if (counting) {
            GpProfScope _p("bin_count", s);
            if (gp_bin_count(bp, N, d.gx, T, rects, binhist, il.total, s)) return 1;
        } else if (gp_scan_blocks_u32(tt, N, block_sums, il.total, s)) return 1;
        const bool capacity_mode = st->binning_capacity > 0;
        if (capacity_mode) {
            if (!st->binning_status) GP_FAIL("binning_capacity needs binning_status (device, 2 words)");
            if (st->binning_capacity > 0x7FFFFF00ll) GP_FAIL("binning_capacity too large");
            R = (uint32_t)st->binning_capacity;
        } else {
            uint32_t slots[GP_TOTAL_SLOTS];
            GP_HIP_CHECK(hipMemcpyAsync(slots, il.total, sizeof(slots), hipMemcpyDeviceToHost, s));
            GP_HIP_CHECK(hipStreamSynchronize(s));
            uint64_t Rsum = 0;
            for (int k = 0; k < GP_TOTAL_SLOTS; ++k) Rsum += slots[k];
            if (Rsum > 0x7FFFFF00ull) GP_FAIL("too many tile-splat instances (%llu)", (unsigned long long)Rsum);
            R = (uint32_t)Rsum;
            if (R > 0x7FFFFF00u) GP_FAIL("too many tile-splat instances (%u)", R);
            if (st->binning_status && (!counting || R == 0)) {
                hipLaunchKernelGGL(gp_binning_status_kernel, dim3(1), dim3(1), 0, s, il.total, 0xFFFFFFFFu, st->binning_status, d.key_tag);
                GP_LAUNCH_CHECK();
            }
        }

        if (R > 0 && counting) {
            const size_t bin_bytes = gp_align_up((size_t)R * 4, 256) + gp_align_up(2 * (size_t)R + 8, 256);
            void* bin = alloc(alloc_ctx, GP_BUF_BINNING, bin_bytes);
            if (!bin) GP_FAIL("allocator returned NULL for BINNING");
            point_list = (uint32_t*)bin;
            saved->binning = bin; saved->binning_bytes = bin_bytes;
            if (gp_bin_scatter(bp, N, d.gx, T, sorted_ids, rects, binhist, point_list, R, il.ranges, st->binning_status, il.order, d.key_tag, s)) return 1;
            order_done = true;
        } else if (R > 0) {
            const int tbits = tile_bits_for((int)T + (capacity_mode ? 1 : 0));
            const int passes = (tbits + 7) / 8;
            const int res = passes & 1;
            const size_t bin_bytes = gp_align_up((size_t)R * 4, 256) + gp_align_up(2 * (size_t)R + 8, 256);
            void* bin = alloc(alloc_ctx, GP_BUF_BINNING, bin_bytes);
            if (!bin) GP_FAIL("allocator returned NULL for BINNING");
            point_list = (uint32_t*)bin;
            saved->binning = bin; saved->binning_bytes = bin_bytes;
            const size_t bh = gp_sort_hist_elems(R), bs = gp_scan_tmp_elems(256 * (((size_t)R + 4095) / 4096));
            auto carve_bin = [&](GpCarver& c, uint32_t*& bk0, uint32_t*& bk1, uint32_t*& bvo, uint32_t*& bhist, uint32_t*& bscan) {
                bk0 = c.take<uint32_t>(R); bk1 = c.take<uint32_t>(R); bvo = c.take<uint32_t>(R);
                bhist = c.take<uint32_t>(bh); bscan = c.take<uint32_t>(bs);
            };
            uint32_t *bk0, *bk1, *bvo, *bhist, *bscan;
            GpCarver bc0(nullptr);
            carve_bin(bc0, bk0, bk1, bvo, bhist, bscan);
            void* btmp = alloc(alloc_ctx, GP_BUF_TEMP, bc0.bytes());
            if (!btmp) GP_FAIL("allocator returned NULL for TEMP (%zu B)", bc0.bytes());
            GpCarver bc(btmp);
            carve_bin(bc, bk0, bk1, bvo, bhist, bscan);
            GpSortBufs tb;
            tb.k[0] = bk0; tb.k[1] = bk1;
            tb.v[res] = point_list; tb.v[res ^ 1] = bvo;
            tb.hist = bhist; tb.scan_tmp = bscan; tb.scan_tmp_elems = bs;
            { GpProfScope _p("duplicate", s);
            const unsigned ndup = gp_blocks(N, 256);
            hipLaunchKernelGGL(gp_duplicate_kernel, dim3(ndup + (capacity_mode ? gp_blocks(R, 4096) : 0u)), dim3(256), 0, s, d, sorted_ids, tt,
                               (const uint32_t*)block_sums, (const uint32_t*)il.total, rects, tb.k[0], tb.v[0], R, st->binning_status, ndup, d.key_tag);
            GP_LAUNCH_CHECK(); }
            int r2;
            { GpProfScope _p("tile_sort", s); r2 = gp_radix_sort_pairs(tb, R, tbits, s); }
            if (r2 < 0) return 1;
            if (r2 != res) GP_FAIL("internal: sort parity mismatch");
            { GpProfScope _p("tile_ranges", s);
        hipLaunchKernelGGL(gp_tile_ranges_kernel, dim3(gp_blocks(R, 256)), dim3(256), 0, s, tb.k[r2], R, (uint32_t)T, il.ranges);
            GP_LAUNCH_CHECK(); }
        }
    }
    if (N == 0 && st->binning_status)
        GP_HIP_CHECK(hipMemsetAsync(st->binning_status, 0, 2 * sizeof(uint32_t), s));
    saved->num_rendered = (int64_t)R;
    if (!order_done) {
        hipLaunchKernelGGL(gp_tile_order_kernel, dim3(1), dim3(1024), 0, s, il.ranges, (const int32_t*)nullptr, (int)T, il.order);
        GP_LAUNCH_CHECK();
    }
    if (d.late_color && N > 0) {
        GP_HIP_CHECK(hipStreamWaitEvent(s, (hipEvent_t)st->sh_ready_event, 0));
        GpProfScope _p("sh_color", s);
        const bool al16 = (((uintptr_t)in->shs | (uintptr_t)in->shs_rest) & 15) == 0;
        auto kern = gp_sh_color_kernel;
        if (in->shs_rest) kern = gp_sh_color_split_kernel;
        else if (d.M == 16 && al16) kern = gp_sh_color_sh16_kernel;
        GeomLayout glc(saved->geom, N);
        hipLaunchKernelGGL(kern, dim3(gp_blocks(N, 256)), dim3(256), 0, s, d, in->means3D, in->shs, in->shs_rest, st->campos,
                           (const int32_t*)out->radii, glc.rec, glc.clamped);
        GP_LAUNCH_CHECK();
    }
    { GpProfScope _p("composite_fwd", s, 1);
        hipLaunchKernelGGL((gp_debug_get(0) == 3 ? gp_composite_fwd_count_kernel : gp_debug_get(0) == 2 ? gp_composite_fwd_sbc_kernel : gp_composite_fwd_sb_kernel), dim3((unsigned)T), dim3(256), 0, s, d, il.ranges, point_list, gl.rec, st->bg,
                       out->color, out->depth, out->tidx, il.final_T, il.n_contrib, il.order, il.tile_work,
                       point_list ? (uint16_t*)((uint8_t*)point_list + gp_align_up((size_t)R * 4, 256)) : (uint16_t*)nullptr);
    GP_LAUNCH_CHECK(); }
    return 0;
}

extern "C" int gp_raster_backward(const gp_raster_settings* st, const gp_raster_inputs* in, const gp_raster_outputs* fwd,
                                  const gp_raster_saved* saved, const float* dL_dcolor, const float* dL_ddepth,
                                  gp_raster_grads* g, gp_alloc_fn alloc, void* alloc_ctx, gp_stream_t stream_) {
    hipStream_t s = (hipStream_t)stream_;
    RasterDims d;
    if (make_dims(st, in, d)) return 1;
    if (!fwd || !saved || !g || !alloc || !dL_dcolor) GP_FAIL("null argument");
    const size_t N = (size_t)d.N, T = (size_t)d.gx * d.gy, P = (size_t)d.W * d.H;
    if (N == 0) return 0;
    if (!g->dL_dmeans3D || !g->dL_dmeans2D || !g->dL_dopacities) GP_FAIL("null gradient outputs");
    if (in->shs ? (!g->dL_dshs && !g->adam_shs) : !g->dL_dcolors_precomp) GP_FAIL("missing colour gradient output");
    if (in->cov3D_precomp ? !g->dL_dcov3D_precomp : (!g->dL_dscales || !g->dL_drotations)) GP_FAIL("missing covariance gradient output");
    if (!saved->geom || !saved->image) GP_FAIL("saved state missing");
    AdamFuseDev af;
    memset(&af, 0, sizeof(af));
    if (g->adam_shs) {
        const gp_adam_fuse* a = g->adam_shs;
        if (!(in->shs && in->shs_rest) || d.M != 16) GP_FAIL("adam_shs needs the split SH layout (shs [N,1,3] + shs_rest [N,15,3])");
        if (!a->exp_avg_dc || !a->exp_avg_sq_dc || !a->exp_avg_rest || !a->exp_avg_sq_rest) GP_FAIL("adam_shs: null moment pointer");
        if ((((uintptr_t)in->shs_rest | (uintptr_t)a->exp_avg_rest | (uintptr_t)a->exp_avg_sq_rest) & 15) != 0)
            GP_FAIL("adam_shs: shs_rest and its moments must be 16-byte aligned");
        if (a->step < 1) GP_FAIL("adam_shs: bad step");
        const float bc1 = 1.f - powf(a->beta1, (float)a->step);
        af.p_dc = (float*)in->shs; af.m_dc = a->exp_avg_dc; af.v_dc = a->exp_avg_sq_dc;
        af.p_rest = (float*)in->shs_rest; af.m_rest = a->exp_avg_rest; af.v_rest = a->exp_avg_sq_rest;
        af.step_dc = a->lr_dc / bc1; af.step_rest = a->lr_rest / bc1;
        af.b1 = a->beta1; af.b2 = a->beta2; af.eps = a->eps;
        af.bc2_sqrt = sqrtf(1.f - powf(a->beta2, (float)a->step));
        af.skip = a->skip_flag; af.on = 1;
    }
    GeomLayout gl(saved->geom, N);
    ImageLayout il(saved->image, T, P);
    const uint32_t R = (uint32_t)saved->num_rendered;
    const uint32_t* point_list = (const uint32_t*)saved->binning;
    if (R > 0 && !point_list) GP_FAIL("saved binning state missing");

    const size_t acc_floats = (size_t)GP_ACC_STRIDE * N;
    float* acc = (float*)alloc(alloc_ctx, GP_BUF_TEMP, gp_align_up(acc_floats * 4, 256) + gp_align_up(T * 4, 256));
    if (!acc) GP_FAIL("allocator returned NULL for TEMP");
    uint32_t* order_bwd = (uint32_t*)((char*)acc + gp_align_up(acc_floats * 4, 256));
    if (R > 0) {
        const unsigned zb = (unsigned)std::min<size_t>(2048, std::max<size_t>(1, (acc_floats / 4 + 1023) / 1024));
        hipLaunchKernelGGL(gp_bwd_prologue_kernel, dim3(1 + zb), dim3(1024), 0, s, il.ranges, il.tile_work, (int)T, order_bwd, acc, acc_floats);
        GP_LAUNCH_CHECK();
    } else {
        GP_HIP_CHECK(hipMemsetAsync(acc, 0, acc_floats * 4, s));
    }
    float* g_mean2D = acc;
    float* g_conic = acc + 2;
    float* g_opacity = acc + 5;
    float* g_color = acc + 6;
    float* g_depth = acc + 9;
    if (R > 0) {
        static thread_local int ablate_set = 0;
        if (gp_debug_get(1) != ablate_set) { ablate_set = gp_debug_get(1); if (gp_bwd_set_ablate(ablate_set)) GP_FAIL("bwd ablate flag"); }
        GpProfScope _p("composite_bwd", s);
        const int variant = gp_debug_get(7);
        auto kern = dL_ddepth ? gp_composite_bwd_depth_kernel : gp_composite_bwd_kernel;
        if (variant == 3 && N < (size_t)GP_BWD_SB_MAX_N) kern = dL_ddepth ? gp_composite_bwd_sb_depth_kernel : gp_composite_bwd_sb_kernel;
        else if (variant == 2 && !dL_ddepth && N < (size_t)GP_BWD_SB_MAX_N) kern = gp_composite_bwd_sb_count_kernel;
        hipLaunchKernelGGL(kern, dim3((unsigned)((T + 7) / 8 * 8) * GP_BWD_PARTS),
                           dim3(64), 0, s, d, il.ranges, point_list, (const uint16_t*)((const uint8_t*)point_list + gp_align_up((size_t)R * 4, 256)), gl.rec,
                           st->bg, (const float*)fwd->color, (const float*)fwd->depth, (const float*)il.final_T,
                           (const int32_t*)il.n_contrib, dL_dcolor, dL_ddepth, g_mean2D, g_conic, g_opacity, g_color, g_depth, order_bwd);
        GP_LAUNCH_CHECK();
    }
    {
        GpProfScope _p("preprocess_bwd", s);
        const bool al16 = (((uintptr_t)in->shs | (uintptr_t)in->shs_rest | (uintptr_t)g->dL_dshs | (uintptr_t)g->dL_dshs_rest) & 15) == 0;
        auto kern = gp_preprocess_bwd_kernel;
        if (in->shs && in->shs_rest) {
            if (!al16 || (!g->dL_dshs_rest && !af.on)) GP_FAIL("split SH mode needs 16-byte aligned tensors and dL_dshs_rest");
            kern = gp_preprocess_bwd_split_kernel;
        } else if (in->shs && d.M == 16 && al16) {
            kern = gp_preprocess_bwd_sh16_kernel;
        }
        if (g->accumulate_shs && kern == gp_preprocess_bwd_kernel)
            GP_FAIL("accumulate_shs needs the staged SH kernels (16 coeffs, 16-byte aligned)");
        hipLaunchKernelGGL(kern, dim3(gp_blocks(N, 256)), dim3(256), 0, s, d, in->means3D, in->scales, in->rotations, in->shs,
                           in->shs_rest, in->cov3D_precomp, st->viewmatrix, st->projmatrix, st->campos, fwd->radii, gl.clamped,
                           g_mean2D, g_conic, g_opacity, g_color, g_depth, g->dL_dmeans3D, g->dL_dmeans2D, g->dL_dshs,
                           g->dL_dshs_rest, in->shs ? nullptr : g->dL_dcolors_precomp, g->dL_dopacities, g->dL_dscales,
                           g->dL_drotations, g->dL_dcov3D_precomp, (kern != gp_preprocess_bwd_kernel) ? g->accumulate_shs : 0, af);
        GP_LAUNCH_CHECK();
    }
    return 0;
}

extern "C" int gp_debug_counters(uint64_t* out4) {
    if (!out4) GP_FAIL("null argument");
    unsigned long long v[4];
    if (gp_pair_counters_read(v)) GP_FAIL("gp_debug_counters: device read failed");
    for (int k = 0; k < 4; ++k) out4[k] = v[k];
    return 0;
}

extern "C" int gp_raster_mark_visible(int64_t n, const float* means3D, const float* viewmatrix, uint8_t* present,
                                      gp_stream_t stream_) {
    if (n < 0 || n > 0x7FFFFFF0LL) GP_FAIL("n out of range");
    if (n == 0) return 0;
    if (!means3D || !viewmatrix || !present) GP_FAIL("null argument");
    hipLaunchKernelGGL(gp_mark_visible_kernel, dim3(gp_blocks((size_t)n, 256)), dim3(256), 0, (hipStream_t)stream_, (int)n,
                       means3D, viewmatrix, present);
    GP_LAUNCH_CHECK();
    return 0;
}

extern "C" int gp_raster_debug_binning(const gp_raster_settings* st, const gp_raster_saved* saved, uint32_t* point_list,
                                       int32_t* ranges, gp_stream_t stream_) {
    hipStream_t s = (hipStream_t)stream_;
    if (!st || !saved || !ranges) GP_FAIL("null argument");
    const int gx = (st->image_width + GP_TILE - 1) / GP_TILE, gy = (st->image_height + GP_TILE - 1) / GP_TILE;
    const size_t T = (size_t)gx * gy, P = (size_t)st->image_width * st->image_height;
    ImageLayout il(saved->image, T, P);
    GP_HIP_CHECK(hipMemcpyAsync(ranges, il.ranges, T * sizeof(int2), hipMemcpyDeviceToDevice, s));
    if (saved->num_rendered > 0) {
        if (!point_list) GP_FAIL("null point_list");
        GP_HIP_CHECK(hipMemcpyAsync(point_list, saved->binning, (size_t)saved->num_rendered * 4, hipMemcpyDeviceToDevice, s));
    }
    return 0;
}
```

### gaussianprediction_amd/csrc/gp_train_step.hip

```cpp
#include "gp_common.h"
#include "loss_adam_kernels.h"

bool gp_mlp_backward_splits(const gp_mlp_params* p, int64_t rows);
void gp_mlp_backward_accumulate_dfeature_once();

__global__ __launch_bounds__(256) void gp_step_accumulate_kernel(float* __restrict__ dst, const float* __restrict__ src, int64_t n) {
    const int64_t i = (int64_t)blockIdx.x * 256 + threadIdx.x;
    if (i < n) dst[i] += src[i];
}

static int step_adam(const gp_step_update* u, uint32_t sel, gp_stream_t stream, bool ride = false) {
    float *P[32], *G[32], *M[32], *V[32];
    int64_t NUM[32], ST[32];
    float LR[32];
    int n = 0;
    uint32_t keep = 0;
    for (int k = 0; k < u->adam_count && k < 32; ++k) {
        if (!((sel >> k) & 1u)) continue;
        P[n] = u->adam_params[k]; G[n] = u->adam_grads[k]; M[n] = u->adam_exp_avgs[k]; V[n] = u->adam_exp_avg_sqs[k];
        NUM[n] = u->adam_numels[k]; LR[n] = u->adam_lrs[k];
        ST[n] = u->adam_steps ? u->adam_steps[k] : u->step;
        if ((u->keep_grad_mask >> k) & 1u) keep |= 1u << n;
        ++n;
    }
    if (n == 0) return 0;
    if (ride) return gp_adam_rider_arm(n, P, G, M, V, NUM, LR, ST, u->beta1, u->beta2, u->eps, 1, keep, u->skip_flag);
    return gp_adam_step_multi_steps(n, P, G, M, V, NUM, LR, ST, u->beta1, u->beta2, u->eps, 1, keep, u->skip_flag, stream);
}

extern "C" int gp_train_step_run(const gp_step_plan* p, const gp_step_view* v, const gp_step_update* u, gp_alloc_fn alloc,
                                 void* alloc_ctx, gp_stream_t stream) {
    if (!p || !v || !u || !alloc) GP_FAIL("gp_train_step_run: null argument");
    const int64_t N = p->num_gaussians, K = p->num_keypoints;
    if (N <= 0 || K <= 0 || p->nearest_num <= 0) GP_FAIL("gp_train_step_run: needs Gaussians, keypoints and neighbours (the stage-3 form)");
    if (u->binning_capacity <= 0 || !u->binning_status) GP_FAIL("gp_train_step_run: capacity mode only (binning_capacity > 0 with a status word)");
    if (!p->xyz || !p->scaling || !p->rotation || !p->opacity || !p->features_dc || !p->features_rest || !p->keypoints ||
        !p->keypoint_features || !p->raw_w || !p->knn_idx)
        GP_FAIL("gp_train_step_run: null parameter pointer");
    if (!p->g_xyz || !p->g_scaling || !p->g_rotation || !p->g_opacity || !p->g_keypoints || !p->g_keypoint_features)
        GP_FAIL("gp_train_step_run: null gradient pointer");
    if (!u->adam_shs && (!p->g_features_dc || !p->g_features_rest)) GP_FAIL("gp_train_step_run: SH gradient buffers or adam_shs needed");
    if (!p->delta || !p->acts || !p->xyz_t || !p->q_t || !p->scale || !p->opacity_t || !p->loss_sums || !p->loss || !p->g_xyz_t || !p->g_q_t || !p->g_scale || !p->g_opacity_t || !p->g_means2D || !p->g_delta || !p->g_feature_tmp)
        GP_FAIL("gp_train_step_run: null intermediate buffer");
    if (!v->bg || !v->viewmatrix || !v->projmatrix || !v->campos || !v->gt_image || !v->time) GP_FAIL("gp_train_step_run: null view pointer");
    if (u->adam_count < 0 || u->adam_count > 32) GP_FAIL("gp_train_step_run: 0..32 optimizer tensors (got %d)", u->adam_count);
    if (u->adam_count > 0 && (!u->adam_params || !u->adam_grads || !u->adam_exp_avgs || !u->adam_exp_avg_sqs || !u->adam_numels || !u->adam_lrs))
        GP_FAIL("gp_train_step_run: null optimizer table");
    const int H = p->image_height, W = p->image_width, od = p->mlp.out_dim;
    const bool reg = p->reg_scale != 0.f;
    const int64_t nfeat = K * (int64_t)p->feature_dim;
    if (reg && nfeat > 65536) GP_FAIL("gp_train_step_run: the folded regulariser takes at most 65536 feature elements");

    gp_mlp_input mi;
    mi.rows = K; mi.feature_dim = p->feature_dim; mi.xyz_freq = p->xyz_freq; mi.time_freq = p->time_freq;
    mi.feature = p->keypoint_features; mi.xyz = p->keypoints; mi.t = v->time;
    if (gp_mlp_forward(&p->mlp, &mi, p->delta, p->acts, stream)) return 1;
    gp_blend_args ba;
    ba.num_gaussians = N; ba.num_keypoints = K; ba.nearest_num = p->nearest_num; ba.out_dim = od; ba.norm_rotation = p->norm_rotation;
    ba.delta = p->delta; ba.raw_w = p->raw_w; ba.knn_idx = p->knn_idx; ba.xyz = p->xyz; ba.rot = p->rotation; ba.knn_idx16 = p->knn_idx16;
    if (gp_blend_forward(&ba, p->xyz_t, p->q_t, stream)) return 1;
    const bool raw_act = gp_debug_get(14) == 0;
    if (!raw_act && gp_activations_forward(N, p->scaling, p->opacity, nullptr, 0, 1.f, p->scale, p->opacity_t, stream)) return 1;

    gp_raster_settings st;
    memset(&st, 0, sizeof(st));
    st.image_height = H; st.image_width = W; st.tanfovx = v->tanfovx; st.tanfovy = v->tanfovy; st.scale_modifier = 1.f;
    st.sh_degree = p->sh_degree; st.sh_coeffs = 16;
    st.bg = v->bg; st.viewmatrix = v->viewmatrix; st.projmatrix = v->projmatrix; st.campos = v->campos;
    st.binning_capacity = u->binning_capacity; st.binning_status = u->binning_status; st.sh_ready_event = u->sh_ready_event;
    st.depth_key_bits = u->depth_key_bits; st.depth_key_base = u->depth_key_base;
    st.raw_activations = raw_act ? 1 : 0;
    gp_raster_inputs in;
    memset(&in, 0, sizeof(in));
    in.num_gaussians = N; in.means3D = p->xyz_t; in.shs = p->features_dc; in.shs_rest = p->features_rest;
    in.opacities = raw_act ? p->opacity : p->opacity_t;
    in.scales = raw_act ? p->scaling : p->scale; in.rotations = p->q_t;
    gp_raster_outputs out = p->out;
    gp_raster_saved saved;
    memset(&saved, 0, sizeof(saved));
    if (gp_raster_forward(&st, &in, &out, &saved, alloc, alloc_ctx, stream)) return 1;
    alloc(alloc_ctx, GP_BUF_TEMP_DONE, 0);
    if (u->hook) u->hook(u->hook_ctx, GP_STEP_AFTER_FORWARD);

    float* dimg = p->dL_dimage;
    if (!dimg) GP_FAIL("gp_train_step_run: null intermediate buffer");
    if (gp_debug_get(11) == 0) {
        if (gp_loss_l1_ssim_fused(out.color, v->gt_image, 3, H, W, p->lambda_dssim, nullptr, p->loss_sums, dimg, reg ? p->keypoint_features : nullptr,
                                  nfeat, p->reg_scale, reg ? p->g_keypoint_features : nullptr, stream)) return 1;
        if (reg) { if (gp_loss_l1_ssim_finalize_reg(p->loss_sums, 3, H, W, p->lambda_dssim, p->keypoint_features, nfeat, p->reg_scale, p->loss, stream)) return 1; }
        else if (gp_loss_l1_ssim_finalize(p->loss_sums, 3, H, W, p->lambda_dssim, p->loss, stream)) return 1;
    } else {
        float* dmaps = p->dmaps;
        if (!dmaps) {
            dmaps = (float*)alloc(alloc_ctx, GP_BUF_TEMP, gp_align_up((size_t)9 * H * W * 4, 256));
            if (!dmaps) GP_FAIL("gp_train_step_run: allocator returned NULL for the SSIM derivative maps");
        }
        if (gp_loss_l1_ssim_forward(out.color, v->gt_image, 3, H, W, p->loss_sums, dmaps, stream)) return 1;
        if (reg) {
            if (gp_loss_l1_ssim_finalize_reg(p->loss_sums, 3, H, W, p->lambda_dssim, p->keypoint_features, nfeat, p->reg_scale, p->loss, stream)) return 1;
            if (gp_loss_l1_ssim_backward_reg(out.color, v->gt_image, dmaps, 3, H, W, p->lambda_dssim, nullptr, dimg,
                                             p->keypoint_features, nfeat, p->reg_scale, p->g_keypoint_features, stream)) return 1;
        } else {
            if (gp_loss_l1_ssim_finalize(p->loss_sums, 3, H, W, p->lambda_dssim, p->loss, stream)) return 1;
            if (gp_loss_l1_ssim_backward(out.color, v->gt_image, dmaps, 3, H, W, p->lambda_dssim, nullptr, dimg, stream)) return 1;
        }
        if (!p->dmaps) alloc(alloc_ctx, GP_BUF_TEMP_DONE, 0);
    }

    gp_raster_grads g;
    memset(&g, 0, sizeof(g));
    g.dL_dmeans3D = p->g_xyz_t; g.dL_dmeans2D = p->g_means2D; g.dL_dshs = p->g_features_dc; g.dL_dshs_rest = p->g_features_rest;
    g.dL_dopacities = raw_act ? p->g_opacity : p->g_opacity_t; g.dL_dscales = raw_act ? p->g_scaling : p->g_scale; g.dL_drotations = p->g_q_t; g.accumulate_shs = 0; g.adam_shs = u->adam_shs;
    if (gp_raster_backward(&st, &in, &out, &saved, dimg, nullptr, &g, alloc, alloc_ctx, stream)) return 1;
    alloc(alloc_ctx, GP_BUF_TEMP_DONE, 0);
    if (u->hook) u->hook(u->hook_ctx, GP_STEP_AFTER_RASTER_BACKWARD);
    if (!raw_act && gp_activations_backward(N, p->scaling, p->opacity, nullptr, 0, 1.f, p->g_scale, p->g_opacity_t, p->g_scaling, p->g_opacity, nullptr, stream))
        return 1;
    if (gp_blend_backward(&ba, p->g_xyz_t, p->g_q_t, p->g_delta, nullptr, p->g_xyz, p->g_rotation, alloc, alloc_ctx, stream)) return 1;
    alloc(alloc_ctx, GP_BUF_TEMP_DONE, 0);
    const uint32_t all = u->adam_count >= 32 ? 0xFFFFFFFFu : ((1u << u->adam_count) - 1u);
    const uint32_t early = (u->hook || u->adam_count <= 0) ? 0u : (u->adam_early_mask & all);
    if (early && step_adam(u, early, stream, true)) return 1;
    gp_mlp_grads mg = p->g_mlp;
    const bool add_in_place = reg && gp_mlp_backward_splits(&p->mlp, K);
    if (add_in_place) gp_mlp_backward_accumulate_dfeature_once();
    const int rc_mlp = gp_mlp_backward(&p->mlp, &mi, p->acts, p->g_delta, &mg, (reg && !add_in_place) ? p->g_feature_tmp : p->g_keypoint_features,
                                       p->g_keypoints, alloc, alloc_ctx, stream);
    if (rc_mlp) { gp_adam_rider_slot()->armed = false; return 1; }
    if (gp_adam_rider_flush((hipStream_t)stream)) return 1;
    if (reg && !add_in_place) {
        hipLaunchKernelGGL(gp_step_accumulate_kernel, dim3(gp_blocks((size_t)nfeat, 256)), dim3(256), 0, (hipStream_t)stream,
                           p->g_keypoint_features, (const float*)p->g_feature_tmp, nfeat);
        GP_LAUNCH_CHECK();
    }
    if (u->hook) u->hook(u->hook_ctx, GP_STEP_AFTER_BACKWARD);

    if (u->adam_count > 0 && step_adam(u, all & ~early, stream)) return 1;
    return 0;
}
```

### gaussianprediction_amd/csrc/loss_adam_kernels.h

```cpp
#pragma once
#include "gp_common.h"

#define ADAM_MAX_TENSORS 32
#define ADAM_CHUNK 16384
struct AdamTable {
    float* p[ADAM_MAX_TENSORS];
    float* g[ADAM_MAX_TENSORS];
    float* m[ADAM_MAX_TENSORS];
    float* v[ADAM_MAX_TENSORS];
    unsigned long long n[ADAM_MAX_TENSORS];
    float step_size[ADAM_MAX_TENSORS];
    float bc2_sqrt[ADAM_MAX_TENSORS];
    unsigned keep_grad_mask;
    unsigned chunk_begin[ADAM_MAX_TENSORS + 1];
    int count;
};

template <int THREADS>
__device__ __forceinline__ void adam_chunk_body(const AdamTable& t, unsigned chunk, int tid, float b1, float b2, float eps, int zero_grad,
                                                const uint32_t* __restrict__ skip_flag) {
    const bool skip = skip_flag && *skip_flag != 0;
    int k = 0;
    while (k + 1 < t.count && chunk >= t.chunk_begin[k + 1]) ++k;
    const size_t base = (size_t)(chunk - t.chunk_begin[k]) * ADAM_CHUNK;
    const size_t n = t.n[k];
    float* __restrict__ p = t.p[k]; float* __restrict__ g = t.g[k]; float* __restrict__ m = t.m[k]; float* __restrict__ v = t.v[k];
    const float step_size = t.step_size[k], bc2_sqrt = t.bc2_sqrt[k];
    if ((t.keep_grad_mask >> k) & 1u) zero_grad = 0;
    const size_t end = base + ADAM_CHUNK < n ? base + ADAM_CHUNK : n;
    auto upd = [&](float4& pv, const float4& gv, float4& mv, float4& vv) {
        float* pp = (float*)&pv; const float* gg = (const float*)&gv; float* mm = (float*)&mv; float* vq = (float*)&vv;
#pragma unroll
        for (int u = 0; u < 4; ++u) gp_adam_update(pp[u], gg[u], mm[u], vq[u], b1, b2, eps, step_size, bc2_sqrt);
    };
    const float4 zero4 = make_float4(0.f, 0.f, 0.f, 0.f);
    size_t i = base + (size_t)tid * 4;
    if (skip) {
        if (zero_grad)
            for (size_t j = base + tid; j < end; j += THREADS) g[j] = 0.f;
        return;
    }
    constexpr size_t S = (size_t)THREADS * 4;
    for (; i + S + 3 < end; i += 2 * S) {
        const size_t j = i + S;
        float4 pa = *(float4*)(p + i), ga = *(float4*)(g + i), ma = *(float4*)(m + i), va = *(float4*)(v + i);
        float4 pb = *(float4*)(p + j), gb = *(float4*)(g + j), mb = *(float4*)(m + j), vb = *(float4*)(v + j);
        upd(pa, ga, ma, va);
        upd(pb, gb, mb, vb);
        *(float4*)(p + i) = pa; *(float4*)(m + i) = ma; *(float4*)(v + i) = va;
        *(float4*)(p + j) = pb; *(float4*)(m + j) = mb; *(float4*)(v + j) = vb;
        if (zero_grad) { *(float4*)(g + i) = zero4; *(float4*)(g + j) = zero4; }
    }
    for (; i < end; i += S) {
        if (i + 3 < n) {
            float4 pv = *(float4*)(p + i), gv = *(float4*)(g + i), mv = *(float4*)(m + i), vv = *(float4*)(v + i);
            upd(pv, gv, mv, vv);
            *(float4*)(p + i) = pv; *(float4*)(m + i) = mv; *(float4*)(v + i) = vv;
            if (zero_grad) *(float4*)(g + i) = zero4;
        } else {
            for (size_t j = i; j < n; ++j) {
                gp_adam_update(p[j], g[j], m[j], v[j], b1, b2, eps, step_size, bc2_sqrt);
                if (zero_grad) g[j] = 0.f;
            }
        }
    }
}

struct GpAdamRider {
    AdamTable t;
    float b1, b2, eps;
    int zero_grad;
    const uint32_t* skip_flag;
    unsigned chunks;
    bool armed;
};
GpAdamRider* gp_adam_rider_slot();
int gp_adam_rider_arm(int count, float* const* params, float* const* grads, float* const* exp_avgs, float* const* exp_avg_sqs,
                      const int64_t* numels, const float* lrs, const int64_t* steps, float beta1, float beta2, float eps, int zero_grad,
                      uint32_t keep_grad_mask, const uint32_t* skip_flag);
int gp_adam_rider_flush(hipStream_t s);
```

### gaussianprediction_amd/csrc/loss_adam_kernels.hip

```cpp
#include "gp_common.h"
#include "loss_adam_kernels.h"

#define LT 32
#define LH 5
#define LE (LT + 2 * LH)
#define LP (LE + 1)
#define LHP (LT + 1)

struct Win11 { float w[11]; };

__device__ __forceinline__ float block_sum_256(float v, float* s_red) {
#pragma unroll
    for (int d = 32; d >= 1; d >>= 1) v += __shfl_xor(v, d);
    const int lane = threadIdx.x & 63, wave = threadIdx.x >> 6;
    if (lane == 0) s_red[wave] = v;
    __syncthreads();
    return s_red[0] + s_red[1] + s_red[2] + s_red[3];
}

__global__ __launch_bounds__(256) void gp_l1_ssim_fwd_kernel(const float* __restrict__ img, const float* __restrict__ gt,
                                                            int H, int W, Win11 win, double* __restrict__ sums,
                                                            float* __restrict__ dmap) {
    __shared__ float s_a[LE][LP], s_b[LE][LP];
    __shared__ float s_h[4][LE][LHP];
    __shared__ float s_red[4];
    const int tid = threadIdx.x;
    const int tx0 = blockIdx.x * LT, ty0 = blockIdx.y * LT, ch = blockIdx.z;
    const size_t HW = (size_t)H * W;
    const float* a_img = img + ch * HW;
    const float* b_img = gt + ch * HW;
    {
        constexpr int NST = (LE * LE + 255) / 256;
        float va[NST], vb[NST];
#pragma unroll
        for (int u = 0; u < NST; ++u) {
            const int i = tid + 256 * u, y = i / LE, x = i - y * LE;
            const int gy = ty0 - LH + y, gx = tx0 - LH + x;
            const bool in = i < LE * LE && gy >= 0 && gy < H && gx >= 0 && gx < W;
            const size_t o = in ? (size_t)gy * W + gx : 0;
            va[u] = a_img[o]; vb[u] = b_img[o];
        }
#pragma unroll
        for (int u = 0; u < NST; ++u) {
            const int i = tid + 256 * u, y = i / LE, x = i - y * LE;
            const int gy = ty0 - LH + y, gx = tx0 - LH + x;
            const bool in = gy >= 0 && gy < H && gx >= 0 && gx < W;
            if (i < LE * LE) { s_a[y][x] = in ? va[u] : 0.f; s_b[y][x] = in ? vb[u] : 0.f; }
        }
    }
    __syncthreads();
    if (tid < LE * 4) {
        const int y = tid >> 2, x0 = (tid & 3) * 8;
        float a[18], b[18], s2[18], ab[18];
#pragma unroll
        for (int j = 0; j < 18; ++j) {
            a[j] = s_a[y][x0 + j]; b[j] = s_b[y][x0 + j];
            s2[j] = a[j] * a[j] + b[j] * b[j]; ab[j] = a[j] * b[j];
        }
#pragma unroll
        for (int e = 0; e < 8; ++e) {
            float m1 = 0.f, m2 = 0.f, ss2 = 0.f, sab = 0.f;
#pragma unroll
            for (int k = 0; k < 11; ++k) {
                const float w = win.w[k];
                m1 = fmaf(w, a[e + k], m1); m2 = fmaf(w, b[e + k], m2);
                ss2 = fmaf(w, s2[e + k], ss2); sab = fmaf(w, ab[e + k], sab);
            }
            s_h[0][y][x0 + e] = m1; s_h[1][y][x0 + e] = m2; s_h[2][y][x0 + e] = ss2; s_h[3][y][x0 + e] = sab;
        }
    }
    __syncthreads();
    float l1 = 0.f, ss = 0.f;
    const float C1 = 0.01f * 0.01f, C2 = 0.03f * 0.03f;
    {
        const int x = tid & 31, y0 = (tid >> 5) * 4;
        float o[4][4];
#pragma unroll
        for (int q = 0; q < 4; ++q) {
            float v[14];
#pragma unroll
            for (int j = 0; j < 14; ++j) v[j] = s_h[q][y0 + j][x];
#pragma unroll
            for (int e = 0; e < 4; ++e) {
                float acc = 0.f;
#pragma unroll
                for (int k = 0; k < 11; ++k) acc = fmaf(win.w[k], v[e + k], acc);
                o[q][e] = acc;
            }
        }
        const int gx = tx0 + x;
#pragma unroll
        for (int e = 0; e < 4; ++e) {
            const int y = y0 + e, gy = ty0 + y;
            if (gy >= H || gx >= W) continue;
            const float mu1 = o[0][e], mu2 = o[1][e], s2f = o[2][e], ab = o[3][e];
            const float mu1s = mu1 * mu1, mu2s = mu2 * mu2, mu12 = mu1 * mu2;
            const float s12 = ab - mu12;
            const float N1 = 2.f * mu12 + C1, N2 = 2.f * s12 + C2, D1 = mu1s + mu2s + C1, D2 = ((s2f - mu1s) - mu2s) + C2;
            const float inv = 1.f / (D1 * D2);
            const float ssim = N1 * N2 * inv;
            ss += ssim;
            l1 += fabsf(s_a[y + LH][x + LH] - s_b[y + LH][x + LH]);
            if (dmap) {
                const size_t oo = ch * HW + (size_t)gy * W + gx;
                const float dmu1 = (2.f * mu2 * N2 - 2.f * mu2 * N1) * inv - ssim * (2.f * mu1 * D2 - 2.f * mu1 * D1) * inv;
                dmap[oo] = dmu1;
                dmap[3 * HW + oo] = -ssim / D2;
                dmap[6 * HW + oo] = 2.f * N1 * inv;
            }
        }
    }
    const float l1_tot = block_sum_256(l1, s_red);
    __syncthreads();
    const float ss_tot = block_sum_256(ss, s_red);
    if (tid == 0) {
        const unsigned slot = blockIdx.x + gridDim.x * (blockIdx.y + gridDim.y * blockIdx.z);
        sums[2 * slot] = (double)l1_tot;
        sums[2 * slot + 1] = (double)ss_tot;
    }
}

__global__ __launch_bounds__(256) void gp_l1_ssim_bwd_kernel(const float* __restrict__ img, const float* __restrict__ gt,
                                                            const float* __restrict__ dmap, int H, int W, Win11 win,
                                                            float lambda, const float* __restrict__ upstream,
                                                            float* __restrict__ dimg, const float* __restrict__ reg_x, long reg_n,
                                                            float reg_scale_over_n, float* __restrict__ reg_g) {
    __shared__ float s_m[3][LE][LP];
    __shared__ float s_h[3][LE][LHP];
    const int tid = threadIdx.x;
    const int tx0 = blockIdx.x * LT, ty0 = blockIdx.y * LT, ch = blockIdx.z;
    if (reg_g && blockIdx.x == 0 && blockIdx.y == 0 && blockIdx.z == 0) {
        const float c = (upstream ? upstream[0] : 1.f) * reg_scale_over_n;
        for (long i = tid; i < reg_n; i += 256) { const float v = reg_x[i]; reg_g[i] = v > 0.f ? c : (v < 0.f ? -c : 0.f); }
    }
    const size_t HW = (size_t)H * W;
    float pa[4], pb[4];
    {
        const int x = tid & 31, y0 = (tid >> 5) * 4, gx = min(tx0 + x, W - 1);
#pragma unroll
        for (int e = 0; e < 4; ++e) {
            const size_t oo = ch * HW + (size_t)min(ty0 + y0 + e, H - 1) * W + gx;
            pa[e] = img[oo]; pb[e] = gt[oo];
        }
    }
    {
        constexpr int NST = (LE * LE + 255) / 256;
        float v0[NST], v1[NST], v2[NST];
#pragma unroll
        for (int u = 0; u < NST; ++u) {
            const int i = tid + 256 * u, y = i / LE, x = i - y * LE;
            const int gy = ty0 - LH + y, gx = tx0 - LH + x;
            const bool in = i < LE * LE && gy >= 0 && gy < H && gx >= 0 && gx < W;
            const size_t o = ch * HW + (in ? (size_t)gy * W + gx : 0);
            v0[u] = dmap[o]; v1[u] = dmap[3 * HW + o]; v2[u] = dmap[6 * HW + o];
        }
#pragma unroll
        for (int u = 0; u < NST; ++u) {
            const int i = tid + 256 * u, y = i / LE, x = i - y * LE;
            const int gy = ty0 - LH + y, gx = tx0 - LH + x;
            const bool in = gy >= 0 && gy < H && gx >= 0 && gx < W;
            if (i < LE * LE) { s_m[0][y][x] = in ? v0[u] : 0.f; s_m[1][y][x] = in ? v1[u] : 0.f; s_m[2][y][x] = in ? v2[u] : 0.f; }
        }
    }
    __syncthreads();
    if (tid < LE * 4) {
        const int y = tid >> 2, x0 = (tid & 3) * 8;
#pragma unroll
        for (int q = 0; q < 3; ++q) {
            float v[18];
#pragma unroll
            for (int j = 0; j < 18; ++j) v[j] = s_m[q][y][x0 + j];
#pragma unroll
            for (int e = 0; e < 8; ++e) {
                float acc = 0.f;
#pragma unroll
                for (int k = 0; k < 11; ++k) acc = fmaf(win.w[k], v[e + k], acc);
                s_h[q][y][x0 + e] = acc;
            }
        }
    }
    __syncthreads();
    const float g = upstream ? upstream[0] : 1.f;
    const float inv_n = 1.f / (3.f * (float)HW);
    {
        const int x = tid & 31, y0 = (tid >> 5) * 4;
        float o[3][4];
#pragma unroll
        for (int q = 0; q < 3; ++q) {
            float v[14];
#pragma unroll
            for (int j = 0; j < 14; ++j) v[j] = s_h[q][y0 + j][x];
#pragma unroll
            for (int e = 0; e < 4; ++e) {
                float acc = 0.f;
#pragma unroll
                for (int k = 0; k < 11; ++k) acc = fmaf(win.w[k], v[e + k], acc);
                o[q][e] = acc;
            }
        }
        const int gx = tx0 + x;
#pragma unroll
        for (int e = 0; e < 4; ++e) {
            const int gy = ty0 + y0 + e;
            if (gy >= H || gx >= W) continue;
            const size_t oo = ch * HW + (size_t)gy * W + gx;
            const float a = pa[e], b = pb[e];
            const float d = a - b;
            const float sgn = (d > 0.f) ? 1.f : ((d < 0.f) ? -1.f : 0.f);
            dimg[oo] = g * inv_n * ((1.f - lambda) * sgn - lambda * (o[0][e] + 2.f * a * o[1][e] + b * o[2][e]));
        }
    }
}

#define LF (LT + 4 * LH)
#define LFP (LF + 1)
__global__ __launch_bounds__(256) void gp_l1_ssim_fused_kernel(const float* __restrict__ img, const float* __restrict__ gt, int H, int W,
                                                              Win11 win, float lambda, const float* __restrict__ upstream,
                                                              double* __restrict__ sums, float* __restrict__ dimg,
                                                              const float* __restrict__ reg_x, long reg_n, float reg_scale_over_n,
                                                              float* __restrict__ reg_g) {
    typedef float f2 __attribute__((ext_vector_type(2)));
    __shared__ f2 s_ab[LF][LFP];
    __shared__ f2 s_h[LF][LP];
    __shared__ float s_red[4];
    f2 (*s_m01)[LP] = (f2 (*)[LP]) & s_ab[0][0];
    float (*s_m2)[LP] = (float (*)[LP])((float*)&s_ab[0][0] + 2 * LE * LP);
    f2 (*s_g01)[LHP] = (f2 (*)[LHP]) & s_h[0][0];
    float (*s_g2)[LHP] = (float (*)[LHP])((float*)&s_h[0][0] + 2 * LE * LHP);
    static_assert(3 * LE * LP <= 2 * LF * LFP && 3 * LE * LHP <= 2 * LF * LP, "aliased planes must fit");
    const int tid = threadIdx.x;
    const int tx0 = blockIdx.x * LT, ty0 = blockIdx.y * LT, ch = blockIdx.z;
    if (reg_g && blockIdx.x == 0 && blockIdx.y == 0 && blockIdx.z == 0) {
        const float c = (upstream ? upstream[0] : 1.f) * reg_scale_over_n;
        for (long i = tid; i < reg_n; i += 256) { const float v = reg_x[i]; reg_g[i] = v > 0.f ? c : (v < 0.f ? -c : 0.f); }
    }
    const size_t HW = (size_t)H * W;
    const float* a_img = img + ch * HW;
    const float* b_img = gt + ch * HW;
    {
        constexpr int NST = (LF * LF + 255) / 256;
        float va[NST], vb[NST];
#pragma unroll
        for (int u = 0; u < NST; ++u) {
            const int i = tid + 256 * u, y = i / LF, x = i - y * LF;
            const int gy = ty0 - 2 * LH + y, gx = tx0 - 2 * LH + x;
            const bool in = i < LF * LF && gy >= 0 && gy < H && gx >= 0 && gx < W;
            const size_t o = in ? (size_t)gy * W + gx : 0;
            va[u] = a_img[o]; vb[u] = b_img[o];
        }
#pragma unroll
        for (int u = 0; u < NST; ++u) {
            const int i = tid + 256 * u, y = i / LF, x = i - y * LF;
            const int gy = ty0 - 2 * LH + y, gx = tx0 - 2 * LH + x;
            const bool in = gy >= 0 && gy < H && gx >= 0 && gx < W;
            if (i < LF * LF) s_ab[y][x] = in ? f2{va[u], vb[u]} : f2{0.f, 0.f};
        }
    }
    __syncthreads();
    const int ox = tid & 31, oy0 = (tid >> 5) * 4;
    f2 pab[4];
#pragma unroll
    for (int e = 0; e < 4; ++e) pab[e] = s_ab[oy0 + e + 2 * LH][ox + 2 * LH];
    const int vx = tid % LE, vy0 = (tid / LE) * 7;
    const bool vert = tid < LE * 6;
    float st[4][7];
#pragma unroll
    for (int round = 0; round < 2; ++round) {
        if (tid < LF * 4) {
            const int y = tid >> 2, x0 = (tid & 3) * 11;
            f2 v[21];
#pragma unroll
            for (int j = 0; j < 21; ++j) v[j] = s_ab[y][x0 + j];
            if (round == 1) {
#pragma unroll
                for (int j = 0; j < 21; ++j) {
                    const f2 sq = v[j] * v[j];
                    v[j] = f2{sq[0] + sq[1], v[j][0] * v[j][1]};
                }
            }
#pragma unroll
            for (int e = 0; e < 11; ++e) {
                f2 m = {0.f, 0.f};
#pragma unroll
                for (int k = 0; k < 11; ++k) m = __builtin_elementwise_fma(f2{win.w[k], win.w[k]}, v[e + k], m);
                if (x0 + e < LE) s_h[y][x0 + e] = m;
            }
        }
        __syncthreads();
        if (vert) {
            f2 v[17];
#pragma unroll
            for (int j = 0; j < 17; ++j) v[j] = s_h[vy0 + j][vx];
#pragma unroll
            for (int e = 0; e < 7; ++e) {
                f2 acc = {0.f, 0.f};
#pragma unroll
                for (int k = 0; k < 11; ++k) acc = __builtin_elementwise_fma(f2{win.w[k], win.w[k]}, v[e + k], acc);
                st[2 * round][e] = acc[0];
                st[2 * round + 1][e] = acc[1];
            }
        }
        if (round < 1) __syncthreads();
    }
    float l1 = 0.f, ss = 0.f;
    const float C1 = 0.01f * 0.01f, C2 = 0.03f * 0.03f;
    if (vert) {
        const int gx = tx0 - LH + vx;
#pragma unroll
        for (int e = 0; e < 7; ++e) {
            const int y = vy0 + e, gy = ty0 - LH + y;
            float d0 = 0.f, d1 = 0.f, d2 = 0.f;
            if (gy >= 0 && gy < H && gx >= 0 && gx < W) {
                const float mu1 = st[0][e], mu2 = st[1][e], s2f = st[2][e], ab = st[3][e];
                const float mu1s = mu1 * mu1, mu2s = mu2 * mu2, mu12 = mu1 * mu2;
                const float s12 = ab - mu12;
                const float N1 = 2.f * mu12 + C1, N2 = 2.f * s12 + C2, D1 = mu1s + mu2s + C1, D2 = ((s2f - mu1s) - mu2s) + C2;
                const float inv = 1.f / (D1 * D2);
                const float ssim = N1 * N2 * inv;
                if (vx >= LH && vx < LH + LT && y >= LH && y < LH + LT) ss += ssim;
                d0 = (2.f * mu2 * N2 - 2.f * mu2 * N1) * inv - ssim * (2.f * mu1 * D2 - 2.f * mu1 * D1) * inv;
                d1 = -ssim / D2;
                d2 = 2.f * N1 * inv;
            }
            s_m01[y][vx] = f2{d0, d1};
            s_m2[y][vx] = d2;
        }
    }
    __syncthreads();
    if (tid < LE * 4) {
        const int y = tid >> 2, x0 = (tid & 3) * 8;
        f2 v[18];
        float v2[18];
#pragma unroll
        for (int j = 0; j < 18; ++j) { v[j] = s_m01[y][x0 + j]; v2[j] = s_m2[y][x0 + j]; }
#pragma unroll
        for (int e = 0; e < 8; ++e) {
            f2 acc = {0.f, 0.f};
            float acc2 = 0.f;
#pragma unroll
            for (int k = 0; k < 11; ++k) { acc = __builtin_elementwise_fma(f2{win.w[k], win.w[k]}, v[e + k], acc); acc2 = fmaf(win.w[k], v2[e + k], acc2); }
            s_g01[y][x0 + e] = acc;
            s_g2[y][x0 + e] = acc2;
        }
    }
    __syncthreads();
    const float g = upstream ? upstream[0] : 1.f;
    const float inv_n = 1.f / (3.f * (float)HW);
    {
        float o[3][4];
        {
            f2 v[14];
            float v2[14];
#pragma unroll
            for (int j = 0; j < 14; ++j) { v[j] = s_g01[oy0 + j][ox]; v2[j] = s_g2[oy0 + j][ox]; }
#pragma unroll
            for (int e = 0; e < 4; ++e) {
                f2 acc = {0.f, 0.f};
                float acc2 = 0.f;
#pragma unroll
                for (int k = 0; k < 11; ++k) { acc = __builtin_elementwise_fma(f2{win.w[k], win.w[k]}, v[e + k], acc); acc2 = fmaf(win.w[k], v2[e + k], acc2); }
                o[0][e] = acc[0]; o[1][e] = acc[1]; o[2][e] = acc2;
            }
        }
        const int gx = tx0 + ox;
#pragma unroll
        for (int e = 0; e < 4; ++e) {
            const int gy = ty0 + oy0 + e;
            if (gy >= H || gx >= W) continue;
            const float a = pab[e][0], b = pab[e][1];
            const float d = a - b;
            l1 += fabsf(d);
            const float sgn = (d > 0.f) ? 1.f : ((d < 0.f) ? -1.f : 0.f);
            dimg[ch * HW + (size_t)gy * W + gx] = g * inv_n * ((1.f - lambda) * sgn - lambda * (o[0][e] + 2.f * a * o[1][e] + b * o[2][e]));
        }
    }
    const float l1_tot = block_sum_256(l1, s_red);
    __syncthreads();
    const float ss_tot = block_sum_256(ss, s_red);
    if (tid == 0) {
        const unsigned slot = blockIdx.x + gridDim.x * (blockIdx.y + gridDim.y * blockIdx.z);
        sums[2 * slot] = (double)l1_tot;
        sums[2 * slot + 1] = (double)ss_tot;
    }
}

__global__ __launch_bounds__(256) void gp_adam_kernel(float* __restrict__ p, float* __restrict__ g, float* __restrict__ m,
                                                     float* __restrict__ v, size_t n, float lr, float b1, float b2, float eps,
                                                     float bc1, float bc2_sqrt, int zero_grad) {
    size_t i = ((size_t)blockIdx.x * 256 + threadIdx.x) * 4;
    if (i + 3 < n) {
        float4 pv = *(float4*)(p + i), gv = *(float4*)(g + i), mv = *(float4*)(m + i), vv = *(float4*)(v + i);
        float* pp = (float*)&pv; float* gg = (float*)&gv; float* mm = (float*)&mv; float* vq = (float*)&vv;
#pragma unroll
        for (int k = 0; k < 4; ++k) {
            mm[k] = b1 * mm[k] + (1.f - b1) * gg[k];
            vq[k] = b2 * vq[k] + (1.f - b2) * gg[k] * gg[k];
            const float denom = sqrtf(vq[k]) / bc2_sqrt + eps;
            pp[k] -= (lr / bc1) * (mm[k] / denom);
        }
        *(float4*)(p + i) = pv; *(float4*)(m + i) = mv; *(float4*)(v + i) = vv;
        if (zero_grad) *(float4*)(g + i) = make_float4(0.f, 0.f, 0.f, 0.f);
    } else {
        for (; i < n; ++i) {
            const float gk = g[i];
            const float mk = b1 * m[i] + (1.f - b1) * gk;
            const float vk = b2 * v[i] + (1.f - b2) * gk * gk;
            const float denom = sqrtf(vk) / bc2_sqrt + eps;
            p[i] -= (lr / bc1) * (mk / denom);
            m[i] = mk; v[i] = vk;
            if (zero_grad) g[i] = 0.f;
        }
    }
}

__global__ __launch_bounds__(256) void gp_adam_multi_kernel(AdamTable t, float b1, float b2, float eps, int zero_grad,
                                                           const uint32_t* __restrict__ skip_flag) {
    adam_chunk_body<256>(t, blockIdx.x, threadIdx.x, b1, b2, eps, zero_grad, skip_flag);
}

__device__ __forceinline__ void loss_slot_totals(const double* __restrict__ sums, int nslots, double* s_red , double& s0, double& s1) {
    const int tid = threadIdx.x;
    double a = 0.0, b = 0.0;
    const double2* s2 = reinterpret_cast<const double2*>(sums);
    for (int k0 = tid; k0 < nslots; k0 += 256 * 8) {
        double2 v[8];
#pragma unroll
        for (int u = 0; u < 8; ++u) { const int k = k0 + 256 * u; v[u] = s2[k < nslots ? k : nslots - 1]; }
#pragma unroll
        for (int u = 0; u < 8; ++u) if (k0 + 256 * u < nslots) { a += v[u].x; b += v[u].y; }
    }
#pragma unroll
    for (int d = 32; d >= 1; d >>= 1) {
        a += __shfl_xor(a, d);
        b += __shfl_xor(b, d);
    }
    if ((tid & 63) == 0) { s_red[2 * (tid >> 6)] = a; s_red[2 * (tid >> 6) + 1] = b; }
    __syncthreads();
    s0 = (s_red[0] + s_red[2]) + (s_red[4] + s_red[6]);
    s1 = (s_red[1] + s_red[3]) + (s_red[5] + s_red[7]);
}

__global__ __launch_bounds__(256) void gp_loss_finalize_kernel(const double* __restrict__ sums, int nslots, double n, float lambda, float* __restrict__ loss) {
    __shared__ double s_tot[8];
    double s0, s1;
    loss_slot_totals(sums, nslots, s_tot, s0, s1);
    if (threadIdx.x == 0) loss[0] = (float)((1.0 - (double)lambda) * s0 / n + (double)lambda * (1.0 - s1 / n));
}

__global__ __launch_bounds__(256) void gp_loss_finalize_reg_kernel(const double* __restrict__ sums, int nslots, double n, float lambda,
                                                                  const float* __restrict__ x, long nx, float scale_over_n,
                                                                  float* __restrict__ loss) {
    __shared__ float s_red[4];
    __shared__ double s_tot[8];
    float acc = 0.f;
    if ((nx & 3) == 0 && (((uintptr_t)x) & 15) == 0) {
        const float4* x4 = (const float4*)x;
        const long n4 = nx >> 2;
        for (long i0 = threadIdx.x; i0 < n4; i0 += 256 * 8) {
            float4 v[8];
#pragma unroll
            for (int u = 0; u < 8; ++u) { const long i = i0 + 256 * u; v[u] = x4[i < n4 ? i : n4 - 1]; }
#pragma unroll
            for (int u = 0; u < 8; ++u)
                if (i0 + 256 * u < n4) acc += (fabsf(v[u].x) + fabsf(v[u].y)) + (fabsf(v[u].z) + fabsf(v[u].w));
        }
    } else {
        for (long i = threadIdx.x; i < nx; i += 256) acc += fabsf(x[i]);
    }
    const float tot = block_sum_256(acc, s_red);
    double s0, s1;
    loss_slot_totals(sums, nslots, s_tot, s0, s1);
    if (threadIdx.x == 0)
        loss[0] = (float)((1.0 - (double)lambda) * s0 / n + (double)lambda * (1.0 - s1 / n)) + tot * scale_over_n;
}

__global__ __launch_bounds__(256) void gp_l1_mean_fwd_kernel(const float* __restrict__ x, long n, float scale_over_n,
                                                            const float* __restrict__ base, float* __restrict__ out) {
    __shared__ float s_red[4];
    float acc = 0.f;
    for (long i = (long)blockIdx.x * 256 + threadIdx.x; i < n; i += (long)gridDim.x * 256) acc += fabsf(x[i]);
    const float tot = block_sum_256(acc, s_red);
    if (threadIdx.x == 0) atomicAdd(out, tot * scale_over_n + (blockIdx.x == 0 ? base[0] : 0.f));
}
__global__ __launch_bounds__(256) void gp_l1_mean_bwd_kernel(const float* __restrict__ x, long n, float scale_over_n,
                                                            const float* __restrict__ upstream, float* __restrict__ g) {
    const float c = upstream[0] * scale_over_n;
    for (long i = (long)blockIdx.x * 256 + threadIdx.x; i < n; i += (long)gridDim.x * 256) {
        const float v = x[i];
        g[i] = v > 0.f ? c : (v < 0.f ? -c : 0.f);
    }
}

static Win11 make_window() {
    Win11 w;
    double s = 0.0, t[11];
    for (int x = 0; x < 11; ++x) { t[x] = exp(-(double)((x - 5) * (x - 5)) / (2.0 * 1.5 * 1.5)); s += (float)t[x]; }
    for (int x = 0; x < 11; ++x) w.w[x] = (float)((float)t[x] / (float)s);
    return w;
}

extern "C" int gp_loss_l1_ssim_forward(const float* img, const float* gt, int32_t channels, int32_t H, int32_t W, double* sums,
                                       float* dmaps, gp_stream_t stream_) {
    hipStream_t s = (hipStream_t)stream_;
    if (!img || !gt || !sums) GP_FAIL("null argument");
    if (channels != 3 || H <= 0 || W <= 0) GP_FAIL("expects a [3,H,W] image (got C=%d H=%d W=%d)", channels, H, W);
    GpProfScope _p("l1_ssim_fwd", s);
    hipLaunchKernelGGL(gp_l1_ssim_fwd_kernel, dim3((W + LT - 1) / LT, (H + LT - 1) / LT, 3), dim3(256), 0, s, img, gt, H, W,
                       make_window(), sums, dmaps);
    GP_LAUNCH_CHECK();
    return 0;
}

extern "C" int gp_loss_l1_ssim_finalize(const double* sums, int32_t channels, int32_t H, int32_t W, float lambda_dssim, float* loss,
                                        gp_stream_t stream_) {
    if (!sums || !loss) GP_FAIL("null argument");
    if (((uintptr_t)sums & 15) != 0) GP_FAIL("sums must be 16-byte aligned");
    hipLaunchKernelGGL(gp_loss_finalize_kernel, dim3(1), dim3(256), 0, (hipStream_t)stream_, sums, (int)GP_LOSS_SUM_SLOTS(H, W), (double)channels * H * W, lambda_dssim, loss);
    GP_LAUNCH_CHECK();
    return 0;
}

extern "C" int gp_loss_l1_ssim_backward(const float* img, const float* gt, const float* dmaps, int32_t channels, int32_t H,
                                        int32_t W, float lambda_dssim, const float* upstream, float* dimg, gp_stream_t stream_) {
    hipStream_t s = (hipStream_t)stream_;
    if (!img || !gt || !dmaps || !dimg) GP_FAIL("null argument");
    if (channels != 3 || H <= 0 || W <= 0) GP_FAIL("expects a [3,H,W] image");
    GpProfScope _p("l1_ssim_bwd", s);
    hipLaunchKernelGGL(gp_l1_ssim_bwd_kernel, dim3((W + LT - 1) / LT, (H + LT - 1) / LT, 3), dim3(256), 0, s, img, gt, dmaps, H, W,
                       make_window(), lambda_dssim, upstream, dimg, (const float*)nullptr, 0L, 0.f, (float*)nullptr);
    GP_LAUNCH_CHECK();
    return 0;
}

extern "C" int gp_loss_l1_ssim_fused(const float* img, const float* gt, int32_t channels, int32_t H, int32_t W, float lambda_dssim,
                                     const float* upstream, double* sums, float* dimg, const float* x, int64_t n, float scale, float* gx,
                                     gp_stream_t stream_) {
    hipStream_t s = (hipStream_t)stream_;
    if (!img || !gt || !sums || !dimg) GP_FAIL("null argument");
    if (channels != 3 || H <= 0 || W <= 0) GP_FAIL("expects a [3,H,W] image (got C=%d H=%d W=%d)", channels, H, W);
    if ((x != nullptr) != (gx != nullptr)) GP_FAIL("regulariser input and gradient must be given together");
    if (x && (n <= 0 || n > 65536)) GP_FAIL("regulariser input must have 1..65536 elements");
    GpProfScope _p("l1_ssim_fused", s);
    hipLaunchKernelGGL(gp_l1_ssim_fused_kernel, dim3((W + LT - 1) / LT, (H + LT - 1) / LT, 3), dim3(256), 0, s, img, gt, H, W, make_window(),
                       lambda_dssim, upstream, sums, dimg, x, x ? (long)n : 0L, x ? scale / (float)n : 0.f, gx);
    GP_LAUNCH_CHECK();
    return 0;
}

#define GP_LOSS_REG_MAX 65536
extern "C" int gp_loss_l1_ssim_finalize_reg(const double* sums, int32_t channels, int32_t H, int32_t W, float lambda_dssim,
                                            const float* x, int64_t n, float scale, float* loss, gp_stream_t stream_) {
    if (!sums || !loss || !x) GP_FAIL("null argument");
    if (((uintptr_t)sums & 15) != 0) GP_FAIL("sums must be 16-byte aligned");
    if (n <= 0 || n > GP_LOSS_REG_MAX) GP_FAIL("regulariser input must have 1..%d elements (use gp_l1_mean_forward beyond)", GP_LOSS_REG_MAX);
    hipLaunchKernelGGL(gp_loss_finalize_reg_kernel, dim3(1), dim3(256), 0, (hipStream_t)stream_, sums, (int)GP_LOSS_SUM_SLOTS(H, W), (double)channels * H * W, lambda_dssim,
                       x, (long)n, scale / (float)n, loss);
    GP_LAUNCH_CHECK();
    return 0;
}
extern "C" int gp_loss_l1_ssim_backward_reg(const float* img, const float* gt, const float* dmaps, int32_t channels, int32_t H, int32_t W,
                                            float lambda_dssim, const float* upstream, float* dimg, const float* x, int64_t n,
                                            float scale, float* gx, gp_stream_t stream_) {
    hipStream_t s = (hipStream_t)stream_;
    if (!img || !gt || !dmaps || !dimg || !x || !gx) GP_FAIL("null argument");
    if (channels != 3 || H <= 0 || W <= 0) GP_FAIL("expects a [3,H,W] image");
    if (n <= 0 || n > GP_LOSS_REG_MAX) GP_FAIL("regulariser input must have 1..%d elements", GP_LOSS_REG_MAX);
    GpProfScope _p("l1_ssim_bwd", s);
    hipLaunchKernelGGL(gp_l1_ssim_bwd_kernel, dim3((W + LT - 1) / LT, (H + LT - 1) / LT, 3), dim3(256), 0, s, img, gt, dmaps, H, W,
                       make_window(), lambda_dssim, upstream, dimg, x, (long)n, scale / (float)n, gx);
    GP_LAUNCH_CHECK();
    return 0;
}

extern "C" int gp_adam_step(float* param, float* grad, float* exp_avg, float* exp_avg_sq, int64_t n, float lr, float beta1,
                            float beta2, float eps, int64_t step, int32_t zero_grad, gp_stream_t stream_) {
    hipStream_t s = (hipStream_t)stream_;
    if (n < 0 || step < 1) GP_FAIL("bad n/step");
    if (n == 0) return 0;
    if (!param || !grad || !exp_avg || !exp_avg_sq) GP_FAIL("null argument");
    if ((((uintptr_t)param | (uintptr_t)grad | (uintptr_t)exp_avg | (uintptr_t)exp_avg_sq) & 15) != 0) GP_FAIL("adam: pointers must be 16-byte aligned");
    const float bc1 = 1.f - powf(beta1, (float)step);
    const float bc2_sqrt = sqrtf(1.f - powf(beta2, (float)step));
    GpProfScope _p("adam", s);
    hipLaunchKernelGGL(gp_adam_kernel, dim3(gp_blocks(((size_t)n + 3) / 4, 256)), dim3(256), 0, s, param, grad, exp_avg, exp_avg_sq,
                       (size_t)n, lr, beta1, beta2, eps, bc1, bc2_sqrt, zero_grad);
    GP_LAUNCH_CHECK();
    return 0;
}

static int adam_build_table(AdamTable& t, long& n_chunks, int32_t count, float* const* params, float* const* grads, float* const* exp_avgs,
                            float* const* exp_avg_sqs, const int64_t* numels, const float* lrs, const int64_t* steps, float beta1,
                            float beta2, uint32_t keep_grad_mask) {
    n_chunks = 0;
    if (count < 0 || count > ADAM_MAX_TENSORS) GP_FAIL("adam: at most %d tensors per call (got %d)", ADAM_MAX_TENSORS, count);
    if (count == 0) return 0;
    if (!params || !grads || !exp_avgs || !exp_avg_sqs || !numels || !lrs || !steps) GP_FAIL("null argument");
    t.count = 0;
    t.keep_grad_mask = 0;
    unsigned chunks = 0;
    for (int k = 0; k < count; ++k) {
        if (numels[k] <= 0) continue;
        if (steps[k] < 1) GP_FAIL("adam: bad step %lld (tensor %d)", (long long)steps[k], k);
        if ((((uintptr_t)params[k] | (uintptr_t)grads[k] | (uintptr_t)exp_avgs[k] | (uintptr_t)exp_avg_sqs[k]) & 15) != 0)
            GP_FAIL("adam: pointers must be 16-byte aligned (tensor %d)", k);
        const int j = t.count++;
        if ((keep_grad_mask >> k) & 1u) t.keep_grad_mask |= 1u << j;
        t.p[j] = params[k]; t.g[j] = grads[k]; t.m[j] = exp_avgs[k]; t.v[j] = exp_avg_sqs[k];
        t.n[j] = (unsigned long long)numels[k];
        t.step_size[j] = lrs[k] / (1.f - powf(beta1, (float)steps[k]));
        t.bc2_sqrt[j] = sqrtf(1.f - powf(beta2, (float)steps[k]));
        t.chunk_begin[j] = chunks;
        chunks += (unsigned)((numels[k] + ADAM_CHUNK - 1) / ADAM_CHUNK);
    }
    t.chunk_begin[t.count] = chunks;
    n_chunks = (long)chunks;
    return 0;
}

extern "C" int gp_adam_step_multi_steps(int32_t count, float* const* params, float* const* grads, float* const* exp_avgs,
                                        float* const* exp_avg_sqs, const int64_t* numels, const float* lrs, const int64_t* steps,
                                        float beta1, float beta2, float eps, int32_t zero_grad, uint32_t keep_grad_mask,
                                        const uint32_t* skip_flag, gp_stream_t stream_) {
    hipStream_t s = (hipStream_t)stream_;
    AdamTable t;
    long chunks = 0;
    if (adam_build_table(t, chunks, count, params, grads, exp_avgs, exp_avg_sqs, numels, lrs, steps, beta1, beta2, keep_grad_mask)) return 1;
    if (chunks == 0) return 0;
    GpProfScope _p("adam", s);
    hipLaunchKernelGGL(gp_adam_multi_kernel, dim3((unsigned)chunks), dim3(256), 0, s, t, beta1, beta2, eps, zero_grad, skip_flag);
    GP_LAUNCH_CHECK();
    return 0;
}

GpAdamRider* gp_adam_rider_slot() {
    static thread_local GpAdamRider slot = {};
    return &slot;
}
int gp_adam_rider_arm(int count, float* const* params, float* const* grads, float* const* exp_avgs, float* const* exp_avg_sqs,
                      const int64_t* numels, const float* lrs, const int64_t* steps, float beta1, float beta2, float eps, int zero_grad,
                      uint32_t keep_grad_mask, const uint32_t* skip_flag) {
    GpAdamRider* r = gp_adam_rider_slot();
    r->armed = false;
    long chunks = 0;
    if (adam_build_table(r->t, chunks, count, params, grads, exp_avgs, exp_avg_sqs, numels, lrs, steps, beta1, beta2, keep_grad_mask)) return 1;
    r->b1 = beta1; r->b2 = beta2; r->eps = eps; r->zero_grad = zero_grad; r->skip_flag = skip_flag; r->chunks = (unsigned)chunks;
    r->armed = chunks > 0;
    return 0;
}
int gp_adam_rider_flush(hipStream_t s) {
    GpAdamRider* r = gp_adam_rider_slot();
    if (!r->armed) return 0;
    r->armed = false;
    GpProfScope _p("adam", s);
    hipLaunchKernelGGL(gp_adam_multi_kernel, dim3(r->chunks), dim3(256), 0, s, r->t, r->b1, r->b2, r->eps, r->zero_grad, r->skip_flag);
    GP_LAUNCH_CHECK();
    return 0;
}

extern "C" int gp_adam_step_multi(int32_t count, float* const* params, float* const* grads, float* const* exp_avgs,
                                  float* const* exp_avg_sqs, const int64_t* numels, const float* lrs, float beta1, float beta2,
                                  float eps, int64_t step, int32_t zero_grad, uint32_t keep_grad_mask, const uint32_t* skip_flag,
                                  gp_stream_t stream_) {
    if (count < 0 || count > ADAM_MAX_TENSORS) GP_FAIL("adam: at most %d tensors per call (got %d)", ADAM_MAX_TENSORS, count);
    if (step < 1) GP_FAIL("bad step");
    int64_t steps[ADAM_MAX_TENSORS];
    for (int k = 0; k < count; ++k) steps[k] = step;
    return gp_adam_step_multi_steps(count, params, grads, exp_avgs, exp_avg_sqs, numels, lrs, steps, beta1, beta2, eps, zero_grad,
                                    keep_grad_mask, skip_flag, stream_);
}

extern "C" int gp_l1_mean_forward(const float* x, int64_t n, float scale, const float* base, float* out, gp_stream_t stream_) {
    if (n <= 0) GP_FAIL("l1 mean: empty input");
    if (!x || !base || !out) GP_FAIL("null argument");
    hipStream_t s = (hipStream_t)stream_;
    GP_HIP_CHECK(hipMemsetAsync(out, 0, sizeof(float), s));
    unsigned blocks = gp_blocks((size_t)n, 4096);
    if (blocks > 256) blocks = 256;
    hipLaunchKernelGGL(gp_l1_mean_fwd_kernel, dim3(blocks), dim3(256), 0, s, x, (long)n, scale / (float)n, base, out);
    GP_LAUNCH_CHECK();
    return 0;
}

extern "C" int gp_l1_mean_backward(const float* x, int64_t n, float scale, const float* upstream, float* g, gp_stream_t stream_) {
    if (n <= 0) GP_FAIL("l1 mean: empty input");
    if (!x || !upstream || !g) GP_FAIL("null argument");
    unsigned blocks = gp_blocks((size_t)n, 1024);
    if (blocks > 2048) blocks = 2048;
    hipLaunchKernelGGL(gp_l1_mean_bwd_kernel, dim3(blocks), dim3(256), 0, (hipStream_t)stream_, x, (long)n, scale / (float)n, upstream, g);
    GP_LAUNCH_CHECK();
    return 0;
}
```

### gaussianprediction_amd/csrc/raster_kernels.h

```cpp
#pragma once
#include "gp_common.h"

#define GP_ACC_STRIDE 16
#ifndef GP_BWD_ROWS
#define GP_BWD_ROWS 8
#define GP_BWD_COLS 8
#endif
#define GP_BWD_PARTS ((16 / GP_BWD_ROWS) * (16 / GP_BWD_COLS))
#define GP_BWD_PAIRS (GP_BWD_ROWS * GP_BWD_COLS / 2)

#ifndef GP_SB_HOIST
#define GP_SB_HOIST 0
#endif
struct RasterDims {
    int N, M, D;
    int W, H, gx, gy;
    float tanfovx, tanfovy, fx, fy, scale_mod;
    int late_color;
    uint8_t* visible;
    uint32_t* zero_words;
    int n_zero;
    uint32_t key_hi, key_base, key_culled, key_tag;
    uint32_t* key_flag;
    float2* sb_side;
    const float* raw_opacity;
};
__global__ __launch_bounds__(256) void gp_key_range_kernel(const uint32_t* __restrict__ keys, const int32_t* __restrict__ radii, int n,
                                                          uint32_t base, uint32_t* __restrict__ out2);

__global__ __launch_bounds__(256) void gp_preprocess_fwd_kernel(RasterDims d, const float* __restrict__ means3D, const float* __restrict__ scales,      const float* __restrict__ rotations, const float* __restrict__ opacities, const float* __restrict__ shs,      const float* __restrict__ shs_rest, const float* __restrict__ colors_precomp, const float* __restrict__ cov3D_precomp,      const float* __restrict__ view, const float* __restrict__ proj, const float* __restrict__ campos,      int32_t* __restrict__ radii, float4* __restrict__ rec, uint32_t* __restrict__ depth_key,      uint2* __restrict__ tiles_touched, uint8_t* __restrict__ clamped);

__global__ __launch_bounds__(256) void gp_preprocess_fwd_sh16_kernel(RasterDims d, const float* __restrict__ means3D, const float* __restrict__ scales,      const float* __restrict__ rotations, const float* __restrict__ opacities, const float* __restrict__ shs,      const float* __restrict__ shs_rest, const float* __restrict__ colors_precomp, const float* __restrict__ cov3D_precomp,      const float* __restrict__ view, const float* __restrict__ proj, const float* __restrict__ campos,      int32_t* __restrict__ radii, float4* __restrict__ rec, uint32_t* __restrict__ depth_key,      uint2* __restrict__ tiles_touched, uint8_t* __restrict__ clamped);

__global__ __launch_bounds__(256) void gp_preprocess_fwd_split_kernel(RasterDims d, const float* __restrict__ means3D, const float* __restrict__ scales,      const float* __restrict__ rotations, const float* __restrict__ opacities, const float* __restrict__ shs,      const float* __restrict__ shs_rest, const float* __restrict__ colors_precomp, const float* __restrict__ cov3D_precomp,      const float* __restrict__ view, const float* __restrict__ proj, const float* __restrict__ campos,      int32_t* __restrict__ radii, float4* __restrict__ rec, uint32_t* __restrict__ depth_key,      uint2* __restrict__ tiles_touched, uint8_t* __restrict__ clamped);

#define GP_SC_ARGS RasterDims d, const float* __restrict__ means3D, const float* __restrict__ shs, const float* __restrict__ shs_rest, \
    const float* __restrict__ campos, const int32_t* __restrict__ radii, float4* __restrict__ rec, uint8_t* __restrict__ clamped
__global__ __launch_bounds__(256) void gp_sh_color_kernel(GP_SC_ARGS);
__global__ __launch_bounds__(256) void gp_sh_color_sh16_kernel(GP_SC_ARGS);
__global__ __launch_bounds__(256) void gp_sh_color_split_kernel(GP_SC_ARGS);

__global__ __launch_bounds__(256) void gp_mark_visible_kernel(int n, const float* __restrict__ means3D,
                                                             const float* __restrict__ view, uint8_t* __restrict__ present);


__global__ __launch_bounds__(256) void gp_duplicate_kernel(RasterDims d, const uint32_t* __restrict__ sorted_ids,
                                                          const uint32_t* __restrict__ offsets,
                                                          const uint32_t* __restrict__ block_sums, const uint32_t* __restrict__ total,
                                                          const uint2* __restrict__ rect_sorted,
                                                          uint32_t* __restrict__ keys, uint32_t* __restrict__ vals, uint32_t capacity,
                                                          uint32_t* __restrict__ status, uint32_t n_dup_blocks, uint32_t key_tag);

__global__ __launch_bounds__(256) void gp_tile_ranges_kernel(const uint32_t* __restrict__ keys, uint32_t R, uint32_t n_tiles,
                                                            int2* __restrict__ ranges);
__global__ void gp_binning_status_kernel(const uint32_t* __restrict__ total, uint32_t capacity, uint32_t* __restrict__ status, uint32_t key_tag);

__global__ __launch_bounds__(1024) void gp_tile_order_kernel(const int2* __restrict__ ranges, const int32_t* __restrict__ work_hint, int T, uint32_t* __restrict__ order);
__global__ __launch_bounds__(1024) void gp_bwd_prologue_kernel(const int2* __restrict__ ranges, const int32_t* __restrict__ work_hint, int T,
                                                               uint32_t* __restrict__ order, float* __restrict__ acc, size_t acc_floats);



__global__ __launch_bounds__(256) void gp_preprocess_bwd_kernel(RasterDims d, const float* __restrict__ means3D, const float* __restrict__ scales,      const float* __restrict__ rotations, const float* __restrict__ shs, const float* __restrict__ shs_rest,      const float* __restrict__ cov3D_precomp, const float* __restrict__ view, const float* __restrict__ proj,      const float* __restrict__ campos, const int32_t* __restrict__ radii, const uint8_t* __restrict__ clamped,      const float* __restrict__ g_mean2D, const float* __restrict__ g_conic, const float* __restrict__ g_opacity,      const float* __restrict__ g_color, const float* __restrict__ g_depth, float* __restrict__ dL_dmeans3D,      float* __restrict__ dL_dmeans2D, float* __restrict__ dL_dshs, float* __restrict__ dL_dshs_rest,      float* __restrict__ dL_dcolors, float* __restrict__ dL_dopacities, float* __restrict__ dL_dscales,      float* __restrict__ dL_drots, float* __restrict__ dL_dcov3D, int accumulate_shs, AdamFuseDev af);

__global__ __launch_bounds__(256) void gp_preprocess_bwd_sh16_kernel(RasterDims d, const float* __restrict__ means3D, const float* __restrict__ scales,      const float* __restrict__ rotations, const float* __restrict__ shs, const float* __restrict__ shs_rest,      const float* __restrict__ cov3D_precomp, const float* __restrict__ view, const float* __restrict__ proj,      const float* __restrict__ campos, const int32_t* __restrict__ radii, const uint8_t* __restrict__ clamped,      const float* __restrict__ g_mean2D, const float* __restrict__ g_conic, const float* __restrict__ g_opacity,      const float* __restrict__ g_color, const float* __restrict__ g_depth, float* __restrict__ dL_dmeans3D,      float* __restrict__ dL_dmeans2D, float* __restrict__ dL_dshs, float* __restrict__ dL_dshs_rest,      float* __restrict__ dL_dcolors, float* __restrict__ dL_dopacities, float* __restrict__ dL_dscales,      float* __restrict__ dL_drots, float* __restrict__ dL_dcov3D, int accumulate_shs, AdamFuseDev af);

__global__ __launch_bounds__(256) void gp_preprocess_bwd_split_kernel(RasterDims d, const float* __restrict__ means3D, const float* __restrict__ scales,      const float* __restrict__ rotations, const float* __restrict__ shs, const float* __restrict__ shs_rest,      const float* __restrict__ cov3D_precomp, const float* __restrict__ view, const float* __restrict__ proj,      const float* __restrict__ campos, const int32_t* __restrict__ radii, const uint8_t* __restrict__ clamped,      const float* __restrict__ g_mean2D, const float* __restrict__ g_conic, const float* __restrict__ g_opacity,      const float* __restrict__ g_color, const float* __restrict__ g_depth, float* __restrict__ dL_dmeans3D,      float* __restrict__ dL_dmeans2D, float* __restrict__ dL_dshs, float* __restrict__ dL_dshs_rest,      float* __restrict__ dL_dcolors, float* __restrict__ dL_dopacities, float* __restrict__ dL_dscales,      float* __restrict__ dL_drots, float* __restrict__ dL_dcov3D, int accumulate_shs, AdamFuseDev af);


__global__ __launch_bounds__(256) void gp_composite_fwd_sb_kernel(RasterDims d, const int2* __restrict__ ranges,
                                                                  const uint32_t* __restrict__ point_list,
                                                                  const float4* __restrict__ rec,
                                                                  const float* __restrict__ bg,
                                                                  float* __restrict__ out_color,
                                                                  float* __restrict__ out_depth,
                                                                  int32_t* __restrict__ out_tidx,
                                                                  float* __restrict__ final_T,
                                                                  int32_t* __restrict__ n_contrib, const uint32_t* __restrict__ order, int32_t* __restrict__ tile_work, uint16_t* __restrict__ smask);

__device__ __forceinline__ int gp_tile_bucket(int w) {
    if (w <= 0) return 127;
    const int lg = 31 - __clz(w);
    const int sub = lg >= 2 ? ((w >> (lg - 2)) & 3) : 0;
    const int v = lg * 4 + sub;
    return 126 - (v < 126 ? v : 126);
}
int gp_pair_counters_read(unsigned long long* out4);
int gp_bwd_set_ablate(int v);
__global__ __launch_bounds__(256) void gp_composite_fwd_count_kernel(RasterDims d, const int2* __restrict__ ranges,
                                                                  const uint32_t* __restrict__ point_list,
                                                                  const float4* __restrict__ rec,
                                                                  const float* __restrict__ bg,
                                                                  float* __restrict__ out_color,
                                                                  float* __restrict__ out_depth,
                                                                  int32_t* __restrict__ out_tidx,
                                                                  float* __restrict__ final_T,
                                                                  int32_t* __restrict__ n_contrib, const uint32_t* __restrict__ order, int32_t* __restrict__ tile_work, uint16_t* __restrict__ smask);

__global__ __launch_bounds__(256) void gp_composite_fwd_sbc_kernel(RasterDims d, const int2* __restrict__ ranges,
                                                                  const uint32_t* __restrict__ point_list,
                                                                  const float4* __restrict__ rec,
                                                                  const float* __restrict__ bg,
                                                                  float* __restrict__ out_color,
                                                                  float* __restrict__ out_depth,
                                                                  int32_t* __restrict__ out_tidx,
                                                                  float* __restrict__ final_T,
                                                                  int32_t* __restrict__ n_contrib, const uint32_t* __restrict__ order, int32_t* __restrict__ tile_work, uint16_t* __restrict__ smask);

#define GP_CB_ARGS RasterDims d, const int2* __restrict__ ranges, const uint32_t* __restrict__ point_list, \
    const uint16_t* __restrict__ smask, const float4* __restrict__ rec, const float* __restrict__ bg, const float* __restrict__ out_color, \
    const float* __restrict__ out_depth, const float* __restrict__ final_T, const int32_t* __restrict__ n_contrib, \
    const float* __restrict__ dL_dpix, const float* __restrict__ dL_dpixdepth, float* __restrict__ g_mean2D, float* __restrict__ g_conic, \
    float* __restrict__ g_opacity, float* __restrict__ g_color, float* __restrict__ g_depth, const uint32_t* __restrict__ order
__global__ __launch_bounds__(64) void gp_composite_bwd_kernel(GP_CB_ARGS);
__global__ __launch_bounds__(64) void gp_composite_bwd_depth_kernel(GP_CB_ARGS);
__global__ __launch_bounds__(64) void gp_composite_bwd_sb_kernel(GP_CB_ARGS);
__global__ __launch_bounds__(64) void gp_composite_bwd_sb_depth_kernel(GP_CB_ARGS);
__global__ __launch_bounds__(64) void gp_composite_bwd_sb_count_kernel(GP_CB_ARGS);
#define GP_BWD_SB_MAX_N (1 << 28)
```

Measured before the change: 880.0 views/s.

## Piggyback loss finalize, Adam and raster-bwd prologue onto existing kernels

Adds rider blocks to the keypoint blend-backward kernel so the loss-finalize and the Adam optimizer chunks run as extra blocks of the same launch, and moves the raster-backward prologue (tile ordering and accumulator zeroing) into an extra block of the fused L1+SSIM loss kernel. The aim is to remove several small kernel launches and their serialization gaps in the train step. In exchange, the blend grid is capped lower when Adam rides, state is passed through thread-local slots with arm/disarm logic, and error paths must clean up the armed state.

New measurement: 896.8 views/s (median of 6 runs). 1.02x the previous value.

```diff
diff --git a/gaussianprediction_amd/csrc/deform_kernels.h b/gaussianprediction_amd/csrc/deform_kernels.h
--- a/gaussianprediction_amd/csrc/deform_kernels.h
+++ b/gaussianprediction_amd/csrc/deform_kernels.h
@@ -1,5 +1,6 @@
 #pragma once
 #include "gp_common.h"
+#include "loss_adam_kernels.h"
 
 struct MlpDev {
     long rows;
@@ -85,6 +86,12 @@
                                                            const float* __restrict__ g_q_t, float* __restrict__ g_delta,
                                                            float* __restrict__ g_raw_w, float* __restrict__ g_xyz,
                                                            float* __restrict__ g_rot, float* __restrict__ partial);
+#define GP_BB_RIDE_ARGS BlendRideDev r, BlendDev a, const float* __restrict__ g_xyz_t, const float* __restrict__ g_q_t, \
+    float* __restrict__ g_delta, float* __restrict__ g_raw_w, float* __restrict__ g_xyz, float* __restrict__ g_rot, float* __restrict__ partial
+__global__ __launch_bounds__(256) void gp_blend_bwd6_ride_kernel(GP_BB_RIDE_ARGS);
+__global__ __launch_bounds__(256) void gp_blend_bwd8_ride_kernel(GP_BB_RIDE_ARGS);
+__global__ __launch_bounds__(256) void gp_blend_bwd6_i16_ride_kernel(GP_BB_RIDE_ARGS);
+__global__ __launch_bounds__(256) void gp_blend_bwd8_i16_ride_kernel(GP_BB_RIDE_ARGS);
 __global__ __launch_bounds__(1024) void gp_blend_bwd_reduce_kernel(const float* __restrict__ partial, int nblocks, int KA,
                                                                   int od, float* __restrict__ g_delta);
 __global__ __launch_bounds__(256) void gp_act_fwd_kernel(long n, const float* __restrict__ scaling_raw,
diff --git a/gaussianprediction_amd/csrc/deform_kernels.hip b/gaussianprediction_amd/csrc/deform_kernels.hip
--- a/gaussianprediction_amd/csrc/deform_kernels.hip
+++ b/gaussianprediction_amd/csrc/deform_kernels.hip
@@ -729,7 +729,8 @@
 __device__ __forceinline__ void blend_bwd_body(BlendDev a, const float* __restrict__ g_xyz_t,
                                                const float* __restrict__ g_q_t, float* __restrict__ g_delta,
                                                float* __restrict__ g_raw_w, float* __restrict__ g_xyz,
-                                               float* __restrict__ g_rot, float* __restrict__ partial) {
+                                               float* __restrict__ g_rot, float* __restrict__ partial, const unsigned bid,
+                                               const unsigned nblk) {
     extern __shared__ float s_dyn[];
     const int od = a.out_dim;
     const int nn = NN > 0 ? NN : a.nn;
@@ -760,7 +761,7 @@
         }
     }
     const long chunks = (a.N + 255) / 256;
-    for (long c = blockIdx.x; c < chunks; c += gridDim.x) {
+    for (long c = bid; c < chunks; c += nblk) {
         const long i = c * 256 + tid;
         const bool live = i < a.N;
         if (nn > 0) {
@@ -945,17 +946,37 @@
             }
         }
         __syncthreads();
-        for (int e = tid; e < KA; e += 256) partial[(size_t)blockIdx.x * KA + e] = s_acc[e];
+        for (int e = tid; e < KA; e += 256) partial[(size_t)bid * KA + e] = s_acc[e];
     }
 }
 
 #define BB_ARGS BlendDev a, const float* __restrict__ g_xyz_t, const float* __restrict__ g_q_t, float* __restrict__ g_delta, \
     float* __restrict__ g_raw_w, float* __restrict__ g_xyz, float* __restrict__ g_rot, float* __restrict__ partial
-__global__ __launch_bounds__(256) void gp_blend_bwd_kernel(BB_ARGS) { blend_bwd_body<0>(a, g_xyz_t, g_q_t, g_delta, g_raw_w, g_xyz, g_rot, partial); }
-__global__ __launch_bounds__(256) void gp_blend_bwd6_kernel(BB_ARGS) { blend_bwd_body<6>(a, g_xyz_t, g_q_t, g_delta, g_raw_w, g_xyz, g_rot, partial); }
-__global__ __launch_bounds__(256) void gp_blend_bwd8_kernel(BB_ARGS) { blend_bwd_body<8>(a, g_xyz_t, g_q_t, g_delta, g_raw_w, g_xyz, g_rot, partial); }
-__global__ __launch_bounds__(256) void gp_blend_bwd6_i16_kernel(BB_ARGS) { blend_bwd_body<6, true>(a, g_xyz_t, g_q_t, g_delta, g_raw_w, g_xyz, g_rot, partial); }
-__global__ __launch_bounds__(256) void gp_blend_bwd8_i16_kernel(BB_ARGS) { blend_bwd_body<8, true>(a, g_xyz_t, g_q_t, g_delta, g_raw_w, g_xyz, g_rot, partial); }
+__global__ __launch_bounds__(256) void gp_blend_bwd_kernel(BB_ARGS) { blend_bwd_body<0>(a, g_xyz_t, g_q_t, g_delta, g_raw_w, g_xyz, g_rot, partial, blockIdx.x, gridDim.x); }
+__global__ __launch_bounds__(256) void gp_blend_bwd6_kernel(BB_ARGS) { blend_bwd_body<6>(a, g_xyz_t, g_q_t, g_delta, g_raw_w, g_xyz, g_rot, partial, blockIdx.x, gridDim.x); }
+__global__ __launch_bounds__(256) void gp_blend_bwd8_kernel(BB_ARGS) { blend_bwd_body<8>(a, g_xyz_t, g_q_t, g_delta, g_raw_w, g_xyz, g_rot, partial, blockIdx.x, gridDim.x); }
+__global__ __launch_bounds__(256) void gp_blend_bwd6_i16_kernel(BB_ARGS) { blend_bwd_body<6, true>(a, g_xyz_t, g_q_t, g_delta, g_raw_w, g_xyz, g_rot, partial, blockIdx.x, gridDim.x); }
+__global__ __launch_bounds__(256) void gp_blend_bwd8_i16_kernel(BB_ARGS) { blend_bwd_body<8, true>(a, g_xyz_t, g_q_t, g_delta, g_raw_w, g_xyz, g_rot, partial, blockIdx.x, gridDim.x); }
+
+template <int NN, bool I16>
+__device__ __forceinline__ void blend_bwd_ride_body(const BlendRideDev& r, BB_ARGS) {
+    const unsigned riders = r.fin_blocks + r.adam_chunks;
+    if (blockIdx.x < riders) {
+        if (blockIdx.x < r.fin_blocks) {
+            extern __shared__ float s_dyn[];
+            double* s_tot = (double*)(((uintptr_t)s_dyn + 7) & ~(uintptr_t)7);
+            loss_finalize_body(r.fin, (float*)(s_tot + 8), s_tot);
+        } else {
+            adam_chunk_body<256>(r.t, blockIdx.x - r.fin_blocks, threadIdx.x, r.b1, r.b2, r.eps, r.zero_grad, r.skip_flag);
+        }
+        return;
+    }
+    blend_bwd_body<NN, I16>(a, g_xyz_t, g_q_t, g_delta, g_raw_w, g_xyz, g_rot, partial, blockIdx.x - riders, gridDim.x - riders);
+}
+__global__ __launch_bounds__(256) void gp_blend_bwd6_ride_kernel(BlendRideDev r, BB_ARGS) { blend_bwd_ride_body<6, false>(r, a, g_xyz_t, g_q_t, g_delta, g_raw_w, g_xyz, g_rot, partial); }
+__global__ __launch_bounds__(256) void gp_blend_bwd8_ride_kernel(BlendRideDev r, BB_ARGS) { blend_bwd_ride_body<8, false>(r, a, g_xyz_t, g_q_t, g_delta, g_raw_w, g_xyz, g_rot, partial); }
+__global__ __launch_bounds__(256) void gp_blend_bwd6_i16_ride_kernel(BlendRideDev r, BB_ARGS) { blend_bwd_ride_body<6, true>(r, a, g_xyz_t, g_q_t, g_delta, g_raw_w, g_xyz, g_rot, partial); }
+__global__ __launch_bounds__(256) void gp_blend_bwd8_i16_ride_kernel(BlendRideDev r, BB_ARGS) { blend_bwd_ride_body<8, true>(r, a, g_xyz_t, g_q_t, g_delta, g_raw_w, g_xyz, g_rot, partial); }
 
 __global__ __launch_bounds__(1024) void gp_blend_bwd_reduce_kernel(const float* __restrict__ partial, int nblocks, int KA,
                                                                   int od, float* __restrict__ g_delta) {
diff --git a/gaussianprediction_amd/csrc/gp_capi_deform.hip b/gaussianprediction_amd/csrc/gp_capi_deform.hip
--- a/gaussianprediction_amd/csrc/gp_capi_deform.hip
+++ b/gaussianprediction_amd/csrc/gp_capi_deform.hip
@@ -272,8 +272,14 @@
     if (make_blend(a, b)) return 1;
     if (b.N == 0) return 0;
     if (!dL_dxyz_t || !dL_dq_t || !dL_ddelta || !dL_dxyz || !dL_drot) GP_FAIL("null argument");
+    const bool al = (((uintptr_t)b.raw_w | (uintptr_t)b.knn | (uintptr_t)dL_draw_w) & 15) == 0;
+    const bool i16 = b.knn16 != nullptr;
+    GpBlendRider* rider = gp_blend_rider_slot();
+    const bool ride = (rider->fin_armed || rider->adam.armed) && al && (b.nn == 6 || b.nn == 8);
+    const unsigned adam_chunks = ride && rider->adam.armed ? rider->adam.chunks : 0u;
     unsigned blocks = gp_blocks((size_t)b.N, 256);
-    if (b.nn > 0 && blocks > 1024) blocks = 1024;
+    const unsigned cap = adam_chunks > 0 ? 768u : 1024u;
+    if (b.nn > 0 && blocks > cap) blocks = cap;
     const size_t lds = b.nn > 0 ? ((size_t)b.K * (7 + b.out_dim + 3) + 1 + 256 * 7 + 256 * 2 * (size_t)b.nn) * 4 + 256 * (size_t)b.nn * 2 + 16 : 256 * 8 * 4;
     if (lds > 64 * 1024) GP_FAIL("keypoint blend backward: K = %ld, nn = %d needs %zu B of LDS (> 64 KiB)", (long)b.K, b.nn, lds);
     float* partial = nullptr;
@@ -284,12 +290,25 @@
         if (!partial) GP_FAIL("allocator returned NULL for TEMP");
     }
     { GpProfScope _p("blend_bwd", (hipStream_t)stream_);
-    const bool al = (((uintptr_t)b.raw_w | (uintptr_t)b.knn | (uintptr_t)dL_draw_w) & 15) == 0;
-    const bool i16 = b.knn16 != nullptr;
-    hipLaunchKernelGGL(b.nn == 6 && al ? (i16 ? gp_blend_bwd6_i16_kernel : gp_blend_bwd6_kernel)
-                       : b.nn == 8 && al ? (i16 ? gp_blend_bwd8_i16_kernel : gp_blend_bwd8_kernel) : gp_blend_bwd_kernel,
-                       dim3(blocks), dim3(256), lds, (hipStream_t)stream_, b, dL_dxyz_t, dL_dq_t, dL_ddelta,
-                       dL_draw_w, dL_dxyz, dL_drot, partial);
+    if (ride) {
+        BlendRideDev r;
+        memset(&r, 0, sizeof(r));
+        if (adam_chunks) {
+            r.t = rider->adam.t; r.b1 = rider->adam.b1; r.b2 = rider->adam.b2; r.eps = rider->adam.eps; r.zero_grad = rider->adam.zero_grad;
+            r.skip_flag = rider->adam.skip_flag; r.adam_chunks = adam_chunks;
+        }
+        if (rider->fin_armed) { r.fin = rider->fin; r.fin_blocks = 1; }
+        gp_blend_rider_disarm();
+        hipLaunchKernelGGL(b.nn == 6 ? (i16 ? gp_blend_bwd6_i16_ride_kernel : gp_blend_bwd6_ride_kernel)
+                                     : (i16 ? gp_blend_bwd8_i16_ride_kernel : gp_blend_bwd8_ride_kernel),
+                           dim3(r.fin_blocks + r.adam_chunks + blocks), dim3(256), lds, (hipStream_t)stream_, r, b, dL_dxyz_t, dL_dq_t, dL_ddelta,
+                           dL_draw_w, dL_dxyz, dL_drot, partial);
+    } else {
+        hipLaunchKernelGGL(b.nn == 6 && al ? (i16 ? gp_blend_bwd6_i16_kernel : gp_blend_bwd6_kernel)
+                           : b.nn == 8 && al ? (i16 ? gp_blend_bwd8_i16_kernel : gp_blend_bwd8_kernel) : gp_blend_bwd_kernel,
+                           dim3(blocks), dim3(256), lds, (hipStream_t)stream_, b, dL_dxyz_t, dL_dq_t, dL_ddelta,
+                           dL_draw_w, dL_dxyz, dL_drot, partial);
+    }
     GP_LAUNCH_CHECK();
     if (b.nn > 0) {
         hipLaunchKernelGGL(gp_blend_bwd_reduce_kernel, dim3(gp_blocks((size_t)KA, 64)), dim3(1024), 0, (hipStream_t)stream_, partial,
diff --git a/gaussianprediction_amd/csrc/gp_capi_raster.hip b/gaussianprediction_amd/csrc/gp_capi_raster.hip
--- a/gaussianprediction_amd/csrc/gp_capi_raster.hip
+++ b/gaussianprediction_amd/csrc/gp_capi_raster.hip
@@ -1,5 +1,6 @@
 #include "gp_common.h"
 #include "raster_kernels.h"
+#include "loss_adam_kernels.h"
 #include <stdlib.h>
 #include <atomic>
 
@@ -283,6 +284,36 @@
     return 0;
 }
 
+struct GpBwdPrepared {
+    const void* image;
+    float* acc;
+    size_t acc_floats;
+    bool armed;
+};
+static GpBwdPrepared* bwd_prepared_slot() {
+    static thread_local GpBwdPrepared slot = {};
+    return &slot;
+}
+void gp_raster_backward_unprepare() { bwd_prepared_slot()->armed = false; }
+int gp_raster_backward_prepare(const gp_raster_settings* st, const gp_raster_inputs* in, const gp_raster_saved* saved, gp_alloc_fn alloc,
+                               void* alloc_ctx, GpLossPrologue* pro) {
+    bwd_prepared_slot()->armed = false;
+    pro->armed = false;
+    RasterDims d;
+    if (make_dims(st, in, d)) return 1;
+    const size_t N = (size_t)d.N, T = (size_t)d.gx * d.gy, P = (size_t)d.W * d.H;
+    if (N == 0 || !saved || !saved->image || saved->num_rendered <= 0 || !alloc) return 0;
+    ImageLayout il(saved->image, T, P);
+    const size_t acc_floats = (size_t)GP_ACC_STRIDE * N;
+    float* acc = (float*)alloc(alloc_ctx, GP_BUF_TEMP, gp_align_up(acc_floats * 4, 256) + gp_align_up(T * 4, 256));
+    if (!acc) GP_FAIL("allocator returned NULL for TEMP");
+    pro->ranges = il.ranges; pro->tile_work = il.tile_work; pro->T = (int)T;
+    pro->order = (uint32_t*)((char*)acc + gp_align_up(acc_floats * 4, 256));
+    pro->acc = acc; pro->acc_floats = acc_floats; pro->armed = true;
+    *bwd_prepared_slot() = GpBwdPrepared{saved->image, acc, acc_floats, true};
+    return 0;
+}
+
 extern "C" int gp_raster_backward(const gp_raster_settings* st, const gp_raster_inputs* in, const gp_raster_outputs* fwd,
                                   const gp_raster_saved* saved, const float* dL_dcolor, const float* dL_ddepth,
                                   gp_raster_grads* g, gp_alloc_fn alloc, void* alloc_ctx, gp_stream_t stream_) {
@@ -320,10 +351,14 @@
     if (R > 0 && !point_list) GP_FAIL("saved binning state missing");
 
     const size_t acc_floats = (size_t)GP_ACC_STRIDE * N;
-    float* acc = (float*)alloc(alloc_ctx, GP_BUF_TEMP, gp_align_up(acc_floats * 4, 256) + gp_align_up(T * 4, 256));
+    GpBwdPrepared* pre = bwd_prepared_slot();
+    const bool prepared = pre->armed && pre->image == saved->image && pre->acc_floats == acc_floats && R > 0;
+    pre->armed = false;
+    float* acc = prepared ? pre->acc : (float*)alloc(alloc_ctx, GP_BUF_TEMP, gp_align_up(acc_floats * 4, 256) + gp_align_up(T * 4, 256));
     if (!acc) GP_FAIL("allocator returned NULL for TEMP");
     uint32_t* order_bwd = (uint32_t*)((char*)acc + gp_align_up(acc_floats * 4, 256));
-    if (R > 0) {
+    if (prepared) {
+    } else if (R > 0) {
         const unsigned zb = (unsigned)std::min<size_t>(2048, std::max<size_t>(1, (acc_floats / 4 + 1023) / 1024));
         hipLaunchKernelGGL(gp_bwd_prologue_kernel, dim3(1 + zb), dim3(1024), 0, s, il.ranges, il.tile_work, (int)T, order_bwd, acc, acc_floats);
         GP_LAUNCH_CHECK();
diff --git a/gaussianprediction_amd/csrc/gp_train_step.hip b/gaussianprediction_amd/csrc/gp_train_step.hip
--- a/gaussianprediction_amd/csrc/gp_train_step.hip
+++ b/gaussianprediction_amd/csrc/gp_train_step.hip
@@ -3,13 +3,16 @@
 
 bool gp_mlp_backward_splits(const gp_mlp_params* p, int64_t rows);
 void gp_mlp_backward_accumulate_dfeature_once();
+int gp_raster_backward_prepare(const gp_raster_settings* st, const gp_raster_inputs* in, const gp_raster_saved* saved, gp_alloc_fn alloc,
+                               void* alloc_ctx, GpLossPrologue* pro);
+void gp_raster_backward_unprepare();
 
 __global__ __launch_bounds__(256) void gp_step_accumulate_kernel(float* __restrict__ dst, const float* __restrict__ src, int64_t n) {
     const int64_t i = (int64_t)blockIdx.x * 256 + threadIdx.x;
     if (i < n) dst[i] += src[i];
 }
 
-static int step_adam(const gp_step_update* u, uint32_t sel, gp_stream_t stream, bool ride = false) {
+static int step_adam(const gp_step_update* u, uint32_t sel, gp_stream_t stream, int ride = 0) {
     float *P[32], *G[32], *M[32], *V[32];
     int64_t NUM[32], ST[32];
     float LR[32];
@@ -24,12 +27,28 @@
         ++n;
     }
     if (n == 0) return 0;
+    if (ride == 2) return gp_blend_rider_arm_adam(n, P, G, M, V, NUM, LR, ST, u->beta1, u->beta2, u->eps, 1, keep, u->skip_flag);
     if (ride) return gp_adam_rider_arm(n, P, G, M, V, NUM, LR, ST, u->beta1, u->beta2, u->eps, 1, keep, u->skip_flag);
     return gp_adam_step_multi_steps(n, P, G, M, V, NUM, LR, ST, u->beta1, u->beta2, u->eps, 1, keep, u->skip_flag, stream);
 }
 
+static int train_step_run(const gp_step_plan* p, const gp_step_view* v, const gp_step_update* u, gp_alloc_fn alloc, void* alloc_ctx,
+                          gp_stream_t stream, bool& temp_open);
 extern "C" int gp_train_step_run(const gp_step_plan* p, const gp_step_view* v, const gp_step_update* u, gp_alloc_fn alloc,
                                  void* alloc_ctx, gp_stream_t stream) {
+    bool temp_open = false;
+    const int rc = train_step_run(p, v, u, alloc, alloc_ctx, stream, temp_open);
+    if (rc) {
+        gp_adam_rider_slot()->armed = false;
+        gp_blend_rider_disarm();
+        gp_loss_prologue_slot()->armed = false;
+        gp_raster_backward_unprepare();
+        if (temp_open) alloc(alloc_ctx, GP_BUF_TEMP_DONE, 0);
+    }
+    return rc;
+}
+static int train_step_run(const gp_step_plan* p, const gp_step_view* v, const gp_step_update* u, gp_alloc_fn alloc, void* alloc_ctx,
+                          gp_stream_t stream, bool& temp_open) {
     if (!p || !v || !u || !alloc) GP_FAIL("gp_train_step_run: null argument");
     const int64_t N = p->num_gaussians, K = p->num_keypoints;
     if (N <= 0 || K <= 0 || p->nearest_num <= 0) GP_FAIL("gp_train_step_run: needs Gaussians, keypoints and neighbours (the stage-3 form)");
@@ -84,10 +103,20 @@
 
     float* dimg = p->dL_dimage;
     if (!dimg) GP_FAIL("gp_train_step_run: null intermediate buffer");
+    const int riders_off = gp_debug_get(15);
+    bool finalize_rides = false;
     if (gp_debug_get(11) == 0) {
+        if (!(riders_off & 1)) {
+            GpLossPrologue pro;
+            if (gp_raster_backward_prepare(&st, &in, &saved, alloc, alloc_ctx, &pro)) return 1;
+            if (pro.armed) { temp_open = true; *gp_loss_prologue_slot() = pro; }
+        }
         if (gp_loss_l1_ssim_fused(out.color, v->gt_image, 3, H, W, p->lambda_dssim, nullptr, p->loss_sums, dimg, reg ? p->keypoint_features : nullptr,
                                   nfeat, p->reg_scale, reg ? p->g_keypoint_features : nullptr, stream)) return 1;
-        if (reg) { if (gp_loss_l1_ssim_finalize_reg(p->loss_sums, 3, H, W, p->lambda_dssim, p->keypoint_features, nfeat, p->reg_scale, p->loss, stream)) return 1; }
+        if (!(riders_off & 2)) {
+            if (gp_blend_rider_arm_finalize(p->loss_sums, 3, H, W, p->lambda_dssim, reg ? p->keypoint_features : nullptr, nfeat, p->reg_scale, p->loss)) return 1;
+            finalize_rides = true;
+        } else if (reg) { if (gp_loss_l1_ssim_finalize_reg(p->loss_sums, 3, H, W, p->lambda_dssim, p->keypoint_features, nfeat, p->reg_scale, p->loss, stream)) return 1; }
         else if (gp_loss_l1_ssim_finalize(p->loss_sums, 3, H, W, p->lambda_dssim, p->loss, stream)) return 1;
     } else {
         float* dmaps = p->dmaps;
@@ -112,21 +141,29 @@
     g.dL_dmeans3D = p->g_xyz_t; g.dL_dmeans2D = p->g_means2D; g.dL_dshs = p->g_features_dc; g.dL_dshs_rest = p->g_features_rest;
     g.dL_dopacities = raw_act ? p->g_opacity : p->g_opacity_t; g.dL_dscales = raw_act ? p->g_scaling : p->g_scale; g.dL_drotations = p->g_q_t; g.accumulate_shs = 0; g.adam_shs = u->adam_shs;
     if (gp_raster_backward(&st, &in, &out, &saved, dimg, nullptr, &g, alloc, alloc_ctx, stream)) return 1;
+    gp_raster_backward_unprepare();
     alloc(alloc_ctx, GP_BUF_TEMP_DONE, 0);
+    temp_open = false;
     if (u->hook) u->hook(u->hook_ctx, GP_STEP_AFTER_RASTER_BACKWARD);
     if (!raw_act && gp_activations_backward(N, p->scaling, p->opacity, nullptr, 0, 1.f, p->g_scale, p->g_opacity_t, p->g_scaling, p->g_opacity, nullptr, stream))
         return 1;
+    const uint32_t all = u->adam_count >= 32 ? 0xFFFFFFFFu : ((1u << u->adam_count) - 1u);
+    uint32_t rode = 0;
+    if (!(riders_off & 4) && raw_act && !u->hook)
+        for (int k = 0; k < u->adam_count; ++k)
+            if (u->adam_params[k] == p->scaling || u->adam_params[k] == p->opacity) rode |= 1u << k;
+    if (rode && step_adam(u, rode, stream, 2)) return 1;
     if (gp_blend_backward(&ba, p->g_xyz_t, p->g_q_t, p->g_delta, nullptr, p->g_xyz, p->g_rotation, alloc, alloc_ctx, stream)) return 1;
     alloc(alloc_ctx, GP_BUF_TEMP_DONE, 0);
-    const uint32_t all = u->adam_count >= 32 ? 0xFFFFFFFFu : ((1u << u->adam_count) - 1u);
-    const uint32_t early = (u->hook || u->adam_count <= 0) ? 0u : (u->adam_early_mask & all);
+    if ((finalize_rides || rode) && gp_blend_rider_flush((hipStream_t)stream)) return 1;
+    const uint32_t early = (u->hook || u->adam_count <= 0) ? 0u : (u->adam_early_mask & all & ~rode);
     if (early && step_adam(u, early, stream, true)) return 1;
     gp_mlp_grads mg = p->g_mlp;
     const bool add_in_place = reg && gp_mlp_backward_splits(&p->mlp, K);
     if (add_in_place) gp_mlp_backward_accumulate_dfeature_once();
     const int rc_mlp = gp_mlp_backward(&p->mlp, &mi, p->acts, p->g_delta, &mg, (reg && !add_in_place) ? p->g_feature_tmp : p->g_keypoint_features,
                                        p->g_keypoints, alloc, alloc_ctx, stream);
-    if (rc_mlp) { gp_adam_rider_slot()->armed = false; return 1; }
+    if (rc_mlp) return 1;
     if (gp_adam_rider_flush((hipStream_t)stream)) return 1;
     if (reg && !add_in_place) {
         hipLaunchKernelGGL(gp_step_accumulate_kernel, dim3(gp_blocks((size_t)nfeat, 256)), dim3(256), 0, (hipStream_t)stream,
@@ -135,6 +172,6 @@
     }
     if (u->hook) u->hook(u->hook_ctx, GP_STEP_AFTER_BACKWARD);
 
-    if (u->adam_count > 0 && step_adam(u, all & ~early, stream)) return 1;
+    if (u->adam_count > 0 && step_adam(u, all & ~early & ~rode, stream)) return 1;
     return 0;
 }
diff --git a/gaussianprediction_amd/csrc/loss_adam_kernels.h b/gaussianprediction_amd/csrc/loss_adam_kernels.h
--- a/gaussianprediction_amd/csrc/loss_adam_kernels.h
+++ b/gaussianprediction_amd/csrc/loss_adam_kernels.h
@@ -79,3 +79,106 @@
                       const int64_t* numels, const float* lrs, const int64_t* steps, float beta1, float beta2, float eps, int zero_grad,
                       uint32_t keep_grad_mask, const uint32_t* skip_flag);
 int gp_adam_rider_flush(hipStream_t s);
+
+__device__ __forceinline__ float block_sum_256(float v, float* s_red) {
+#pragma unroll
+    for (int d = 32; d >= 1; d >>= 1) v += __shfl_xor(v, d);
+    const int lane = threadIdx.x & 63, wave = threadIdx.x >> 6;
+    if (lane == 0) s_red[wave] = v;
+    __syncthreads();
+    return s_red[0] + s_red[1] + s_red[2] + s_red[3];
+}
+__device__ __forceinline__ void loss_slot_totals(const double* __restrict__ sums, int nslots, double* s_red , double& s0, double& s1) {
+    const int tid = threadIdx.x;
+    double a = 0.0, b = 0.0;
+    const double2* s2 = reinterpret_cast<const double2*>(sums);
+    for (int k0 = tid; k0 < nslots; k0 += 256 * 8) {
+        double2 v[8];
+#pragma unroll
+        for (int u = 0; u < 8; ++u) { const int k = k0 + 256 * u; v[u] = s2[k < nslots ? k : nslots - 1]; }
+#pragma unroll
+        for (int u = 0; u < 8; ++u) if (k0 + 256 * u < nslots) { a += v[u].x; b += v[u].y; }
+    }
+#pragma unroll
+    for (int d = 32; d >= 1; d >>= 1) {
+        a += __shfl_xor(a, d);
+        b += __shfl_xor(b, d);
+    }
+    if ((tid & 63) == 0) { s_red[2 * (tid >> 6)] = a; s_red[2 * (tid >> 6) + 1] = b; }
+    __syncthreads();
+    s0 = (s_red[0] + s_red[2]) + (s_red[4] + s_red[6]);
+    s1 = (s_red[1] + s_red[3]) + (s_red[5] + s_red[7]);
+}
+struct LossFinalizeDev {
+    const double* sums;
+    int nslots;
+    double n;
+    float lambda;
+    const float* x;
+    long nx;
+    float scale_over_n;
+    float* loss;
+};
+__device__ __forceinline__ void loss_finalize_body(const LossFinalizeDev& f, float* s_red , double* s_tot ) {
+    float tot = 0.f;
+    if (f.x) {
+        const float* __restrict__ x = f.x;
+        const long nx = f.nx;
+        float acc = 0.f;
+        if ((nx & 3) == 0 && (((uintptr_t)x) & 15) == 0) {
+            const float4* x4 = (const float4*)x;
+            const long n4 = nx >> 2;
+            for (long i0 = threadIdx.x; i0 < n4; i0 += 256 * 8) {
+                float4 v[8];
+#pragma unroll
+                for (int u = 0; u < 8; ++u) { const long i = i0 + 256 * u; v[u] = x4[i < n4 ? i : n4 - 1]; }
+#pragma unroll
+                for (int u = 0; u < 8; ++u)
+                    if (i0 + 256 * u < n4) acc += (fabsf(v[u].x) + fabsf(v[u].y)) + (fabsf(v[u].z) + fabsf(v[u].w));
+            }
+        } else {
+            for (long i = threadIdx.x; i < nx; i += 256) acc += fabsf(x[i]);
+        }
+        tot = block_sum_256(acc, s_red);
+    }
+    double s0, s1;
+    loss_slot_totals(f.sums, f.nslots, s_tot, s0, s1);
+    if (threadIdx.x == 0) {
+        const float l = (float)((1.0 - (double)f.lambda) * s0 / f.n + (double)f.lambda * (1.0 - s1 / f.n));
+        f.loss[0] = f.x ? l + tot * f.scale_over_n : l;
+    }
+}
+
+struct BlendRideDev {
+    AdamTable t;
+    float b1, b2, eps;
+    int zero_grad;
+    const uint32_t* skip_flag;
+    unsigned adam_chunks;
+    unsigned fin_blocks;
+    LossFinalizeDev fin;
+};
+struct GpBlendRider {
+    GpAdamRider adam;
+    LossFinalizeDev fin;
+    bool fin_armed;
+};
+GpBlendRider* gp_blend_rider_slot();
+int gp_blend_rider_arm_adam(int count, float* const* params, float* const* grads, float* const* exp_avgs, float* const* exp_avg_sqs,
+                            const int64_t* numels, const float* lrs, const int64_t* steps, float beta1, float beta2, float eps,
+                            int zero_grad, uint32_t keep_grad_mask, const uint32_t* skip_flag);
+int gp_blend_rider_arm_finalize(const double* sums, int32_t channels, int32_t H, int32_t W, float lambda_dssim, const float* x, int64_t n,
+                                float scale, float* loss);
+int gp_blend_rider_flush(hipStream_t s);
+void gp_blend_rider_disarm();
+
+struct GpLossPrologue {
+    const int2* ranges;
+    const int32_t* tile_work;
+    int T;
+    uint32_t* order;
+    float* acc;
+    size_t acc_floats;
+    bool armed;
+};
+GpLossPrologue* gp_loss_prologue_slot();
diff --git a/gaussianprediction_amd/csrc/loss_adam_kernels.hip b/gaussianprediction_amd/csrc/loss_adam_kernels.hip
--- a/gaussianprediction_amd/csrc/loss_adam_kernels.hip
+++ b/gaussianprediction_amd/csrc/loss_adam_kernels.hip
@@ -1,6 +1,8 @@
 #include "gp_common.h"
 #include "loss_adam_kernels.h"
-
+#include "raster_kernels.h"
+
+#define GP_LOSS_REG_MAX 65536
 #define LT 32
 #define LH 5
 #define LE (LT + 2 * LH)
@@ -8,15 +10,6 @@
 #define LHP (LT + 1)
 
 struct Win11 { float w[11]; };
-
-__device__ __forceinline__ float block_sum_256(float v, float* s_red) {
-#pragma unroll
-    for (int d = 32; d >= 1; d >>= 1) v += __shfl_xor(v, d);
-    const int lane = threadIdx.x & 63, wave = threadIdx.x >> 6;
-    if (lane == 0) s_red[wave] = v;
-    __syncthreads();
-    return s_red[0] + s_red[1] + s_red[2] + s_red[3];
-}
 
 __global__ __launch_bounds__(256) void gp_l1_ssim_fwd_kernel(const float* __restrict__ img, const float* __restrict__ gt,
                                                             int H, int W, Win11 win, double* __restrict__ sums,
@@ -218,7 +211,7 @@
                                                               Win11 win, float lambda, const float* __restrict__ upstream,
                                                               double* __restrict__ sums, float* __restrict__ dimg,
                                                               const float* __restrict__ reg_x, long reg_n, float reg_scale_over_n,
-                                                              float* __restrict__ reg_g) {
+                                                              float* __restrict__ reg_g, GpLossPrologue pro) {
     typedef float f2 __attribute__((ext_vector_type(2)));
     __shared__ f2 s_ab[LF][LFP];
     __shared__ f2 s_h[LF][LP];
@@ -229,8 +222,23 @@
     float (*s_g2)[LHP] = (float (*)[LHP])((float*)&s_h[0][0] + 2 * LE * LHP);
     static_assert(3 * LE * LP <= 2 * LF * LFP && 3 * LE * LHP <= 2 * LF * LP, "aliased planes must fit");
     const int tid = threadIdx.x;
-    const int tx0 = blockIdx.x * LT, ty0 = blockIdx.y * LT, ch = blockIdx.z;
-    if (reg_g && blockIdx.x == 0 && blockIdx.y == 0 && blockIdx.z == 0) {
+    const unsigned first = pro.order ? 1u : 0u;
+    if (first && blockIdx.x == 0) {
+        gp_tile_order_body256(pro.ranges, pro.tile_work, pro.T, pro.order, (uint32_t*)&s_h[0][0], (uint32_t*)&s_h[0][0] + 128,
+                              (uint8_t*)&s_ab[0][0], (int)sizeof(s_ab));
+        return;
+    }
+    const unsigned lb = blockIdx.x - first;
+    const unsigned ngx = (unsigned)(W + LT - 1) / LT, ngy = (unsigned)(H + LT - 1) / LT;
+    const unsigned ch = lb / (ngx * ngy), lrem = lb - ch * (ngx * ngy), lby = lrem / ngx, lbx = lrem - lby * ngx;
+    const int tx0 = (int)lbx * LT, ty0 = (int)lby * LT;
+    if (pro.acc) {
+        const size_t n4 = pro.acc_floats >> 2, stride = (size_t)(gridDim.x - first) * 256;
+        float4* a4 = reinterpret_cast<float4*>(pro.acc);
+        for (size_t i = (size_t)lb * 256 + tid; i < n4; i += stride) a4[i] = make_float4(0.f, 0.f, 0.f, 0.f);
+        if (lb == 0 && (unsigned)tid < (unsigned)(pro.acc_floats & 3)) pro.acc[(n4 << 2) + tid] = 0.f;
+    }
+    if (reg_g && lb == 0) {
         const float c = (upstream ? upstream[0] : 1.f) * reg_scale_over_n;
         for (long i = tid; i < reg_n; i += 256) { const float v = reg_x[i]; reg_g[i] = v > 0.f ? c : (v < 0.f ? -c : 0.f); }
     }
@@ -378,9 +386,8 @@
     __syncthreads();
     const float ss_tot = block_sum_256(ss, s_red);
     if (tid == 0) {
-        const unsigned slot = blockIdx.x + gridDim.x * (blockIdx.y + gridDim.y * blockIdx.z);
-        sums[2 * slot] = (double)l1_tot;
-        sums[2 * slot + 1] = (double)ss_tot;
+        sums[2 * lb] = (double)l1_tot;
+        sums[2 * lb + 1] = (double)ss_tot;
     }
 }
 
@@ -418,60 +425,15 @@
     adam_chunk_body<256>(t, blockIdx.x, threadIdx.x, b1, b2, eps, zero_grad, skip_flag);
 }
 
-__device__ __forceinline__ void loss_slot_totals(const double* __restrict__ sums, int nslots, double* s_red , double& s0, double& s1) {
-    const int tid = threadIdx.x;
-    double a = 0.0, b = 0.0;
-    const double2* s2 = reinterpret_cast<const double2*>(sums);
-    for (int k0 = tid; k0 < nslots; k0 += 256 * 8) {
-        double2 v[8];
-#pragma unroll
-        for (int u = 0; u < 8; ++u) { const int k = k0 + 256 * u; v[u] = s2[k < nslots ? k : nslots - 1]; }
-#pragma unroll
-        for (int u = 0; u < 8; ++u) if (k0 + 256 * u < nslots) { a += v[u].x; b += v[u].y; }
-    }
-#pragma unroll
-    for (int d = 32; d >= 1; d >>= 1) {
-        a += __shfl_xor(a, d);
-        b += __shfl_xor(b, d);
-    }
-    if ((tid & 63) == 0) { s_red[2 * (tid >> 6)] = a; s_red[2 * (tid >> 6) + 1] = b; }
-    __syncthreads();
-    s0 = (s_red[0] + s_red[2]) + (s_red[4] + s_red[6]);
-    s1 = (s_red[1] + s_red[3]) + (s_red[5] + s_red[7]);
-}
-
 __global__ __launch_bounds__(256) void gp_loss_finalize_kernel(const double* __restrict__ sums, int nslots, double n, float lambda, float* __restrict__ loss) {
-    __shared__ double s_tot[8];
-    double s0, s1;
-    loss_slot_totals(sums, nslots, s_tot, s0, s1);
-    if (threadIdx.x == 0) loss[0] = (float)((1.0 - (double)lambda) * s0 / n + (double)lambda * (1.0 - s1 / n));
-}
-
-__global__ __launch_bounds__(256) void gp_loss_finalize_reg_kernel(const double* __restrict__ sums, int nslots, double n, float lambda,
-                                                                  const float* __restrict__ x, long nx, float scale_over_n,
-                                                                  float* __restrict__ loss) {
     __shared__ float s_red[4];
     __shared__ double s_tot[8];
-    float acc = 0.f;
-    if ((nx & 3) == 0 && (((uintptr_t)x) & 15) == 0) {
-        const float4* x4 = (const float4*)x;
-        const long n4 = nx >> 2;
-        for (long i0 = threadIdx.x; i0 < n4; i0 += 256 * 8) {
-            float4 v[8];
-#pragma unroll
-            for (int u = 0; u < 8; ++u) { const long i = i0 + 256 * u; v[u] = x4[i < n4 ? i : n4 - 1]; }
-#pragma unroll
-            for (int u = 0; u < 8; ++u)
-                if (i0 + 256 * u < n4) acc += (fabsf(v[u].x) + fabsf(v[u].y)) + (fabsf(v[u].z) + fabsf(v[u].w));
-        }
-    } else {
-        for (long i = threadIdx.x; i < nx; i += 256) acc += fabsf(x[i]);
-    }
-    const float tot = block_sum_256(acc, s_red);
-    double s0, s1;
-    loss_slot_totals(sums, nslots, s_tot, s0, s1);
-    if (threadIdx.x == 0)
-        loss[0] = (float)((1.0 - (double)lambda) * s0 / n + (double)lambda * (1.0 - s1 / n)) + tot * scale_over_n;
+    loss_finalize_body(LossFinalizeDev{sums, nslots, n, lambda, nullptr, 0L, 0.f, loss}, s_red, s_tot);
+}
+__global__ __launch_bounds__(256) void gp_loss_finalize_reg_kernel(LossFinalizeDev f) {
+    __shared__ float s_red[4];
+    __shared__ double s_tot[8];
+    loss_finalize_body(f, s_red, s_tot);
 }
 
 __global__ __launch_bounds__(256) void gp_l1_mean_fwd_kernel(const float* __restrict__ x, long n, float scale_over_n,
@@ -536,25 +498,28 @@
                                      const float* upstream, double* sums, float* dimg, const float* x, int64_t n, float scale, float* gx,
                                      gp_stream_t stream_) {
     hipStream_t s = (hipStream_t)stream_;
+    GpLossPrologue pro = *gp_loss_prologue_slot();
+    gp_loss_prologue_slot()->armed = false;
+    if (!pro.armed) memset(&pro, 0, sizeof(pro));
     if (!img || !gt || !sums || !dimg) GP_FAIL("null argument");
     if (channels != 3 || H <= 0 || W <= 0) GP_FAIL("expects a [3,H,W] image (got C=%d H=%d W=%d)", channels, H, W);
     if ((x != nullptr) != (gx != nullptr)) GP_FAIL("regulariser input and gradient must be given together");
     if (x && (n <= 0 || n > 65536)) GP_FAIL("regulariser input must have 1..65536 elements");
     GpProfScope _p("l1_ssim_fused", s);
-    hipLaunchKernelGGL(gp_l1_ssim_fused_kernel, dim3((W + LT - 1) / LT, (H + LT - 1) / LT, 3), dim3(256), 0, s, img, gt, H, W, make_window(),
-                       lambda_dssim, upstream, sums, dimg, x, x ? (long)n : 0L, x ? scale / (float)n : 0.f, gx);
-    GP_LAUNCH_CHECK();
-    return 0;
-}
-
-#define GP_LOSS_REG_MAX 65536
+    const unsigned tiles = (unsigned)((W + LT - 1) / LT) * (unsigned)((H + LT - 1) / LT) * 3u;
+    hipLaunchKernelGGL(gp_l1_ssim_fused_kernel, dim3(tiles + (pro.order ? 1u : 0u)), dim3(256), 0, s, img, gt, H, W, make_window(),
+                       lambda_dssim, upstream, sums, dimg, x, x ? (long)n : 0L, x ? scale / (float)n : 0.f, gx, pro);
+    GP_LAUNCH_CHECK();
+    return 0;
+}
+
 extern "C" int gp_loss_l1_ssim_finalize_reg(const double* sums, int32_t channels, int32_t H, int32_t W, float lambda_dssim,
                                             const float* x, int64_t n, float scale, float* loss, gp_stream_t stream_) {
     if (!sums || !loss || !x) GP_FAIL("null argument");
     if (((uintptr_t)sums & 15) != 0) GP_FAIL("sums must be 16-byte aligned");
     if (n <= 0 || n > GP_LOSS_REG_MAX) GP_FAIL("regulariser input must have 1..%d elements (use gp_l1_mean_forward beyond)", GP_LOSS_REG_MAX);
-    hipLaunchKernelGGL(gp_loss_finalize_reg_kernel, dim3(1), dim3(256), 0, (hipStream_t)stream_, sums, (int)GP_LOSS_SUM_SLOTS(H, W), (double)channels * H * W, lambda_dssim,
-                       x, (long)n, scale / (float)n, loss);
+    LossFinalizeDev f = {sums, (int)GP_LOSS_SUM_SLOTS(H, W), (double)channels * H * W, lambda_dssim, x, (long)n, scale / (float)n, loss};
+    hipLaunchKernelGGL(gp_loss_finalize_reg_kernel, dim3(1), dim3(256), 0, (hipStream_t)stream_, f);
     GP_LAUNCH_CHECK();
     return 0;
 }
@@ -657,6 +622,59 @@
     return 0;
 }
 
+GpBlendRider* gp_blend_rider_slot() {
+    static thread_local GpBlendRider slot = {};
+    return &slot;
+}
+void gp_blend_rider_disarm() {
+    GpBlendRider* r = gp_blend_rider_slot();
+    r->adam.armed = false;
+    r->fin_armed = false;
+}
+int gp_blend_rider_arm_adam(int count, float* const* params, float* const* grads, float* const* exp_avgs, float* const* exp_avg_sqs,
+                            const int64_t* numels, const float* lrs, const int64_t* steps, float beta1, float beta2, float eps,
+                            int zero_grad, uint32_t keep_grad_mask, const uint32_t* skip_flag) {
+    GpAdamRider* r = &gp_blend_rider_slot()->adam;
+    r->armed = false;
+    long chunks = 0;
+    if (adam_build_table(r->t, chunks, count, params, grads, exp_avgs, exp_avg_sqs, numels, lrs, steps, beta1, beta2, keep_grad_mask)) return 1;
+    r->b1 = beta1; r->b2 = beta2; r->eps = eps; r->zero_grad = zero_grad; r->skip_flag = skip_flag; r->chunks = (unsigned)chunks;
+    r->armed = chunks > 0;
+    return 0;
+}
+int gp_blend_rider_arm_finalize(const double* sums, int32_t channels, int32_t H, int32_t W, float lambda_dssim, const float* x, int64_t n,
+                                float scale, float* loss) {
+    GpBlendRider* r = gp_blend_rider_slot();
+    r->fin_armed = false;
+    if (!sums || !loss) GP_FAIL("null argument");
+    if (((uintptr_t)sums & 15) != 0) GP_FAIL("sums must be 16-byte aligned");
+    if (x && (n <= 0 || n > GP_LOSS_REG_MAX)) GP_FAIL("regulariser input must have 1..%d elements", GP_LOSS_REG_MAX);
+    r->fin = LossFinalizeDev{sums, (int)GP_LOSS_SUM_SLOTS(H, W), (double)channels * H * W, lambda_dssim, x, x ? (long)n : 0L,
+                             x ? scale / (float)n : 0.f, loss};
+    r->fin_armed = true;
+    return 0;
+}
+int gp_blend_rider_flush(hipStream_t s) {
+    GpBlendRider* r = gp_blend_rider_slot();
+    const bool fin = r->fin_armed, adam = r->adam.armed;
+    gp_blend_rider_disarm();
+    if (fin) {
+        hipLaunchKernelGGL(gp_loss_finalize_reg_kernel, dim3(1), dim3(256), 0, s, r->fin);
+        GP_LAUNCH_CHECK();
+    }
+    if (adam) {
+        GpProfScope _p("adam", s);
+        hipLaunchKernelGGL(gp_adam_multi_kernel, dim3(r->adam.chunks), dim3(256), 0, s, r->adam.t, r->adam.b1, r->adam.b2, r->adam.eps,
+                           r->adam.zero_grad, r->adam.skip_flag);
+        GP_LAUNCH_CHECK();
+    }
+    return 0;
+}
+GpLossPrologue* gp_loss_prologue_slot() {
+    static thread_local GpLossPrologue slot = {};
+    return &slot;
+}
+
 extern "C" int gp_adam_step_multi(int32_t count, float* const* params, float* const* grads, float* const* exp_avgs,
                                   float* const* exp_avg_sqs, const int64_t* numels, const float* lrs, float beta1, float beta2,
                                   float eps, int64_t step, int32_t zero_grad, uint32_t keep_grad_mask, const uint32_t* skip_flag,
diff --git a/gaussianprediction_amd/csrc/raster_kernels.h b/gaussianprediction_amd/csrc/raster_kernels.h
--- a/gaussianprediction_amd/csrc/raster_kernels.h
+++ b/gaussianprediction_amd/csrc/raster_kernels.h
@@ -85,6 +85,43 @@
     const int v = lg * 4 + sub;
     return 126 - (v < 126 ? v : 126);
 }
+__device__ __forceinline__ void gp_tile_order_body256(const int2* __restrict__ ranges, const int32_t* __restrict__ work_hint, int T,
+                                                      uint32_t* __restrict__ order, uint32_t* s_cnt, uint32_t* s_base, uint8_t* s_bk,
+                                                      int bk_cap) {
+    constexpr int PER = 16;
+    const int tid = threadIdx.x;
+    const bool keep = T <= bk_cap;
+    auto bucket_of = [&](int t) { const int2 r = ranges[t]; int w = r.y - r.x; if (work_hint) w = min(w, work_hint[t]); return gp_tile_bucket(w); };
+    if (tid < 128) s_cnt[tid] = 0;
+    __syncthreads();
+    for (int t0 = 0; t0 < T; t0 += 256 * PER) {
+        int2 rg[PER];
+        int wh[PER];
+#pragma unroll
+        for (int r = 0; r < PER; ++r) {
+            const int t = t0 + r * 256 + tid;
+            rg[r] = ranges[t < T ? t : T - 1];
+            wh[r] = work_hint ? work_hint[t < T ? t : T - 1] : 0x7fffffff;
+        }
+#pragma unroll
+        for (int r = 0; r < PER; ++r) {
+            const int t = t0 + r * 256 + tid;
+            if (t >= T) continue;
+            const int b = gp_tile_bucket(min(rg[r].y - rg[r].x, wh[r]));
+            if (keep) s_bk[t] = (uint8_t)b;
+            atomicAdd(&s_cnt[b], 1u);
+        }
+    }
+    __syncthreads();
+    if (tid < 128) {
+        uint32_t run = 0;
+#pragma unroll 16
+        for (int b = 0; b < 128; ++b) { const uint32_t c = s_cnt[b]; run += b < tid ? c : 0u; }
+        s_base[tid] = run;
+    }
+    __syncthreads();
+    for (int t = tid; t < T; t += 256) order[atomicAdd(&s_base[keep ? (int)s_bk[t] : bucket_of(t)], 1u)] = (uint32_t)t;
+}
 int gp_pair_counters_read(unsigned long long* out4);
 int gp_bwd_set_ablate(int v);
 __global__ __launch_bounds__(256) void gp_composite_fwd_count_kernel(RasterDims d, const int2* __restrict__ ranges,
```
